# onofreiandrea/quantum_simulations

Hardware: AMD Instinct MI355X
Metric: gate-applications/sec (random 1q+CX circuit, complex128 statevector) (higher is better)
Workload: dtype f64

## Files before the change

include/qsim_hip.h:

```cpp
#ifndef QSIM_HIP_H
#define QSIM_HIP_H

#include <stdint.h>

#ifdef __cplusplus
extern "C" {
#endif

#define QSIM_OK            0
#define QSIM_ERR_INVALID  (-1)
#define QSIM_ERR_NONLOCAL (-2)
#define QSIM_ERR_HIP      (-3)
#define QSIM_ERR_NOMEM    (-4)

typedef struct qsim_chunk qsim_chunk;

const char* qsim_last_error(void);
int qsim_version(void);
int qsim_device_count(int* count);

int qsim_create(int device, int n_local_qubits, qsim_chunk** out);
int qsim_create_view(qsim_chunk* parent, uint64_t offset_amps, int n_local_qubits,
                     qsim_chunk** out);
int qsim_wrap(int device, void* device_ptr, int n_local_qubits, void* stream,
              qsim_chunk** out);
int qsim_destroy(qsim_chunk* c);
int qsim_n_local_qubits(const qsim_chunk* c);
void* qsim_device_ptr(const qsim_chunk* c);

int qsim_init_zero(qsim_chunk* c, int set_amp0);
int qsim_init_random(qsim_chunk* c, uint64_t seed);
int qsim_upload(qsim_chunk* c, const double* re_im, uint64_t offset_amps, uint64_t count);
int qsim_download(qsim_chunk* c, double* re_im, uint64_t offset_amps, uint64_t count);
int qsim_download_c64(qsim_chunk* c, float* re_im, uint64_t offset_amps, uint64_t count);
int qsim_upload_c64(qsim_chunk* c, const float* re_im, uint64_t offset_amps, uint64_t count);
int qsim_copy(qsim_chunk* dst, const qsim_chunk* src);
int qsim_copy_variant(qsim_chunk* dst, const qsim_chunk* src, int variant);

int qsim_apply_1q(qsim_chunk* c, int qubit, const double U[8]);
int qsim_apply_2q(qsim_chunk* c, int qa, int qb, const double U[32]);
int qsim_apply_fused_k(qsim_chunk* c, int k, const int32_t* qubits, const double* M);
int qsim_apply_ops(qsim_chunk* c, int n_ops, const int32_t* nq, const int32_t* qubits,
                   const double* mats);
int qsim_apply_ops_unfused(qsim_chunk* c, int n_ops, const int32_t* nq, const int32_t* qubits,
                           const double* mats);
int qsim_last_pass_count(const qsim_chunk* c);
int qsim_plan_cache_clear(void);
int qsim_apply_ops_tiled(qsim_chunk* c, int n_ops, const int32_t* nq, const int32_t* qubits, const double* mats,
                         int n_tiles, const uint64_t* tile_masks);
int qsim_apply_ops_placed(qsim_chunk* c, int n_ops, const int32_t* nq, const int32_t* qubits, const double* mats,
                          int n_tiles, const uint64_t* tile_masks, const int32_t* earliest_pass);

typedef struct qsim_cycle qsim_cycle;
typedef struct {
  int32_t n_ops; const int32_t* nq; const int32_t* qubits; const double* mats;
  int32_t n_tiles; const uint64_t* tile_masks;
  const int32_t* earliest_pass;
} qsim_cycle_list;
int qsim_cycle_create(int n_local_qubits, const qsim_cycle_list* head, const qsim_cycle_list* steady, const qsim_cycle_list* tail,
                      int32_t* n_passes, qsim_cycle** out);
int qsim_cycle_destroy(qsim_cycle* cycle);
int qsim_apply_cycle(qsim_chunk* c, const qsim_cycle* cycle);

typedef struct {
  uint32_t struct_size;
  const qsim_chunk* src; int32_t src_m; int32_t src_bits[3];
  qsim_chunk* dst; int32_t dst_m; int32_t dst_bits[3];
  qsim_chunk* dst_own; int32_t own_pattern;
  int32_t dst_parts;
  int32_t src_parts;
  int32_t n_tiles;
  const uint64_t* tile_masks;
} qsim_ops_io;
int qsim_apply_ops_io(qsim_chunk* c, int n_ops, const int32_t* nq, const int32_t* qubits,
                      const double* mats, const qsim_ops_io* io, int* n_passes);
int qsim_apply_ops_io_own_slab(const qsim_chunk* c, int32_t* in_chunk);
int qsim_apply_ops_io_load(qsim_chunk* c, int part);
int qsim_apply_ops_io_source_parts(const qsim_chunk* c, int32_t* n_parts, uint64_t* piece_amps, int32_t* n_launches);
int qsim_apply_ops_io_parts(const qsim_chunk* c, int32_t* n_parts, uint64_t* piece_amps, int32_t* n_launches);
int qsim_apply_ops_io_part(qsim_chunk* c, int part);
int qsim_split_piece_count(int n_local_qubits, int m, int dst_parts);
int qsim_tiles_per_workgroup(int n_local_qubits, int tile_bits, int n_fixed_bits);
#define QSIM_PASS_IMAGE_BYTES 4096
int qsim_plan_ops(int n_local_qubits, int n_ops, const int32_t* nq, const int32_t* qubits, const double* mats,
                  void* out, uint64_t out_capacity_bytes, int32_t* n_passes);
int qsim_plan_ops_tiled(int n_local_qubits, int n_ops, const int32_t* nq, const int32_t* qubits, const double* mats,
                        int n_tiles, const uint64_t* tile_masks, void* out, uint64_t out_capacity_bytes, int32_t* n_passes);

int qsim_plan_peek_pass(int n_local_qubits, int n_total_qubits, int n_ops, const int32_t* nq, const int32_t* qubits,
                        const double* mats, const uint8_t* done, uint64_t avoid_mask, uint64_t hint_mask, uint64_t* tile_mask,
                        uint64_t* need_mask, int32_t* n_members, int32_t* members);

int qsim_plan_search(int n_local_qubits, int n_ops, const int32_t* nq, const int32_t* qubits, const double* mats, int beam,
                     uint64_t* out_masks, int out_capacity, int32_t* n_passes);

#define QSIM_PLAN_HISTOGRAM_BINS 64
#define QSIM_TRIPLES_UNBOUNDED 1
#define QSIM_TRIPLES_NEED_BITS 2
int qsim_plan_search_triples(int n_local_qubits, int n_ops, const int32_t* nq, const int32_t* qubits, const double* mats,
                             int n_triples, const int32_t* triples, int beam, int n_threads, int flags, int32_t* best_passes,
                             int32_t* n_found, int32_t* found_index, int32_t* found_triples, uint64_t* found_masks,
                             uint64_t mask_capacity, int32_t* histogram);
int qsim_plan_search_cycle(int n_local_qubits, int n_ops, const int32_t* nq, const int32_t* qubits, const double* mats,
                           int n_triples, const int32_t* triples, const int32_t* plain_passes, int beam, int n_threads,
                           int32_t* n_found, int32_t* found_index, int32_t* found_triples, int32_t* found_passes,
                           uint8_t* found_tail, uint64_t* found_masks, uint64_t mask_capacity);

int qsim_rewrite_ops(int n_qubits, int n_ops, const int32_t* nq, const int32_t* qubits, const double* mats, int32_t* out_nq,
                     int32_t* out_qubits, double* out_mats, int out_capacity, int32_t* n_out, int32_t* need_tile);

int qsim_lower_pass_images(void* images, int n_images, int32_t* n_rewritten);

enum { QSIM_ENGINE_COST_FIXED_US = 0, QSIM_ENGINE_COST_GROUP, QSIM_ENGINE_COST_DENSE1, QSIM_ENGINE_COST_REAL1,
       QSIM_ENGINE_COST_HAD1, QSIM_ENGINE_COST_SWAP1, QSIM_ENGINE_COST_ASWAP1, QSIM_ENGINE_COST_ANTI1, QSIM_ENGINE_COST_PHASE,
       QSIM_ENGINE_COST_PHASE_NEG, QSIM_ENGINE_COST_PHASE_I, QSIM_ENGINE_COST_DIAGR, QSIM_ENGINE_COST_DENSE2,
       QSIM_ENGINE_COST_PRED_LANE, QSIM_ENGINE_COST_PRED_OUTER, QSIM_ENGINE_COST_REG_CTRL, QSIM_ENGINE_COST_DIRECT_END,
       QSIM_ENGINE_COST_FIT_QUBITS, QSIM_ENGINE_COST_UNIT1, QSIM_ENGINE_COST_COUNT };
int qsim_plan_balance(int n_local_qubits, int n_ops, const int32_t* nq, const int32_t* qubits, const double* mats,
                      int n_tiles, const uint64_t* tile_masks, const double* pass_memory_us, const double* engine_costs,
                      int n_engine_costs, int32_t* earliest_pass, double* engine_us_before, double* engine_us_after);
int qsim_plan_ops_placed(int n_local_qubits, int n_ops, const int32_t* nq, const int32_t* qubits, const double* mats,
                         int n_tiles, const uint64_t* tile_masks, const int32_t* earliest_pass, void* out,
                         uint64_t out_capacity_bytes, int32_t* n_passes);
int qsim_rewrite_ops_priced(int n_qubits, int n_ops, const int32_t* nq, const int32_t* qubits, const double* mats,
                            int32_t* out_nq, int32_t* out_qubits, double* out_mats, int out_capacity, int32_t* n_out,
                            int32_t* need_tile, const double* engine_costs, int n_engine_costs);

int qsim_plan_count_layouts(int n_local_qubits, int n_ops, const int32_t* nq, const int32_t* qubits, const double* mats,
                            int n_layouts, const int32_t* layouts, int32_t* n_passes, int n_threads);

int qsim_choose_layout(int n_local_qubits, int n_tiles, const uint64_t* tile_masks, int top_bit, const double* bit_cost,
                       const double* pair_cost, const double* triple_cost , uint64_t seed,
                       int sweeps, int32_t* out_l2p, double* cost_identity, double* cost_chosen);

int qsim_apply_1q_pair(qsim_chunk* c0, qsim_chunk* c1, const double U[8]);
int qsim_apply_2q_pair_qa_local(qsim_chunk* c0, qsim_chunk* c1, int qa, const double U[32]);
int qsim_apply_2q_pair_qb_local(qsim_chunk* c0, qsim_chunk* c1, int qb, const double U[32]);
int qsim_apply_2q_quad(qsim_chunk* c00, qsim_chunk* c01, qsim_chunk* c10, qsim_chunk* c11,
                       const double U[32]);

int qsim_pack_half(const qsim_chunk* src, int bit, int value, qsim_chunk* buf);
int qsim_unpack_half(qsim_chunk* dst, int bit, int value, const qsim_chunk* buf);
int qsim_pack_bits(const qsim_chunk* src, int m, const int32_t* bits, int pattern,
                   qsim_chunk* buf, uint64_t buf_offset_amps);
int qsim_unpack_bits(qsim_chunk* dst, int m, const int32_t* bits, int pattern,
                     const qsim_chunk* buf, uint64_t buf_offset_amps);
int qsim_pack_all(const qsim_chunk* src, int m, const int32_t* bits, qsim_chunk* buf, int skip_pattern,
                  int piece, int n_pieces);
int qsim_unpack_all(qsim_chunk* dst, int m, const int32_t* bits, const qsim_chunk* buf, int skip_pattern,
                    int piece, int n_pieces);

int qsim_swap_global_local(qsim_chunk* const* chunks, int n_chunks, const int32_t* global_bits,
                           const int32_t* local_bits, int m);

#define QSIM_COMM_ID_BYTES 128
typedef struct qsim_comm qsim_comm;
int qsim_comm_get_unique_id(uint8_t id[QSIM_COMM_ID_BYTES]);
int qsim_comm_init(int device, int rank, int world, const uint8_t id[QSIM_COMM_ID_BYTES], qsim_comm** out);
int qsim_comm_destroy(qsim_comm* comm);
int qsim_comm_rank(const qsim_comm* comm);
int qsim_comm_world(const qsim_comm* comm);
int qsim_comm_exchange(qsim_comm* comm, int n_peers, const int32_t* peers, const qsim_chunk* send,
                       const uint64_t* send_off, qsim_chunk* recv, const uint64_t* recv_off, uint64_t count_amps);
int qsim_comm_exchange_bg(qsim_comm* comm, int n_peers, const int32_t* peers, const qsim_chunk* send,
                          const uint64_t* send_off, qsim_chunk* recv, const uint64_t* recv_off, uint64_t count_amps,
                          uint32_t* ticket);
int qsim_comm_join(qsim_comm* comm, qsim_chunk* c);
int qsim_comm_wait(qsim_comm* comm, qsim_chunk* c, uint32_t ticket);
int qsim_comm_relayout(qsim_comm* comm, qsim_chunk* state, qsim_chunk* buf0, qsim_chunk* buf1, int m,
                       const int32_t* local_bits, const int32_t* global_bits, int n_pieces);
int qsim_comm_relayout_plan(int rank, int world, int n_local_qubits, int m, const int32_t* local_bits,
                            const int32_t* global_bits, int n_pieces, int32_t* out_n_pieces, int32_t* out_n_peers,
                            int32_t* out_own_pattern, int32_t* out_peers, uint64_t* out_slab_offsets,
                            uint64_t* out_piece_amps);
int qsim_comm_relayout_loopback(qsim_comm* comm, qsim_chunk* state, qsim_chunk* buf0, qsim_chunk* buf1, int m,
                                const int32_t* local_bits, const int32_t* global_bits, int n_pieces, int as_rank,
                                int as_world);
int qsim_apply_1q_pair_remote(qsim_comm* comm, qsim_chunk* shard, qsim_chunk* buf, int partner_rank, int my_side,
                              const double U[8]);
int qsim_apply_2q_pair_qa_local_remote(qsim_comm* comm, qsim_chunk* shard, qsim_chunk* buf, int partner_rank,
                                       int my_side, int qa, const double U[32]);
int qsim_apply_2q_pair_qb_local_remote(qsim_comm* comm, qsim_chunk* shard, qsim_chunk* buf, int partner_rank,
                                       int my_side, int qb, const double U[32]);

int qsim_apply_2q_quad_remote(qsim_comm* comm, qsim_chunk* shard, qsim_chunk* buf, const int32_t ranks[4], int my_index,
                              const double U[32]);
typedef struct { int32_t n_ops; const int32_t* nq; const int32_t* qubits; const double* mats; } qsim_op_list;
int qsim_comm_relayout_fused(qsim_comm* comm, qsim_chunk* shard, qsim_chunk* send, qsim_chunk* recv,
                             const qsim_op_list* before, const qsim_op_list* after, int m, const int32_t* local_bits,
                             const int32_t* global_bits, int n_pieces, int as_rank, int as_world, int* n_passes);

int qsim_count_nonzero(qsim_chunk* c, double eps, uint64_t* count);
int qsim_export_nonzero(qsim_chunk* c, double eps, uint64_t capacity, uint64_t* out_idx, double* out_re_im,
                        uint64_t* n_rows);
int qsim_sync(qsim_chunk* c);
int qsim_norm2(qsim_chunk* c, double* out);
int qsim_probabilities(qsim_chunk* c, int r, const int32_t* qubits, double* out);
int qsim_reduced_density_matrix(qsim_chunk* c, int r, const int32_t* qubits, double* out);
int qsim_reduced_density_matrix_wide(qsim_chunk* c, int r, const int32_t* qubits, double* out);
int qsim_expectation_pauli(qsim_chunk* c, int n_terms, const uint64_t* x_masks, const uint64_t* z_masks, double* out,
                           int* n_passes);
int qsim_plan_expectation(int n_local_qubits, int n_terms, const uint64_t* x_masks, int32_t* pass_of_term,
                          uint64_t* tile_masks, int* n_passes);
int qsim_apply_pauli_rotations(qsim_chunk* c, int n, const uint64_t* x_masks, const uint64_t* z_masks,
                               const double* thetas, int* n_passes);
int qsim_apply_diagonal_phase(qsim_chunk* c, int n_terms, const uint64_t* z_masks, const double* coeffs, double gamma);
int qsim_diagonal_moments(qsim_chunk* c, int n_terms, const uint64_t* z_masks, const double* coeffs, double out[3]);
int qsim_apply_diagonal_sum(qsim_chunk* dst, const qsim_chunk* src, int n_terms, const uint64_t* z_masks, const double* coeffs,
                            int accumulate);
int qsim_overlap_diagonal(qsim_chunk* ket, const qsim_chunk* bra, int n_terms, const uint64_t* z_masks, const double* coeffs,
                          double out[4]);
int qsim_expectation_z_terms(qsim_chunk* c, int n_terms, const uint64_t* z_masks, double* out, int* n_passes);
int qsim_plan_pauli_rotations(int n_local_qubits, int n, const uint64_t* x_masks, int32_t* pass_of,
                              uint64_t* tile_masks, int* n_passes);
int qsim_apply_pauli_sum(qsim_chunk* dst, const qsim_chunk* src, int n_terms, const uint64_t* x_masks,
                         const uint64_t* z_masks, const double* coeffs, int* n_passes);
int qsim_overlap_pauli(qsim_chunk* ket, const qsim_chunk* bra, int n_terms, const uint64_t* x_masks,
                       const uint64_t* z_masks, double* out_re_im, int* n_passes);
int qsim_lincomb(qsim_chunk* dst, const double dst_coeff[2], int n_src, const qsim_chunk* const* srcs,
                 const double* coeffs_re_im, int n_bras, const qsim_chunk* const* bras, double* dots_re_im,
                 double* norm2);
int qsim_sample(qsim_chunk* c, uint64_t n_shots, const double* randnums, uint64_t* out_indices, double* total, int* n_passes);
int qsim_sample_locate(uint64_t n_blocks, const double* block_cdf, uint64_t n_shots, const double* randnums,
                       uint64_t* out_block, double* out_local);
int qsim_sample_block_bits(void);
int qsim_max_abs_err_closed_form(qsim_chunk* c, int kind, int n_total_qubits,
                                 uint64_t base_index, double* out);
int qsim_max_abs_err_closed_form_perm(qsim_chunk* c, int kind, int n_total_qubits,
                                      uint64_t base_index, const int32_t* log_to_phys,
                                      double* out);
int qsim_fingerprint(qsim_chunk* c, int n_total_qubits, uint64_t base_index, const int32_t* log_to_phys, uint64_t seed,
                     uint64_t sel_mask, uint64_t sel_value, double out[2]);
int qsim_time_begin(qsim_chunk* c);
int qsim_time_end(qsim_chunk* c, float* elapsed_ms);


typedef struct {
  char kernel[48];
  uint64_t launches;
  double total_ms;
  double algorithmic_bytes;
  double hbm_bytes;
  uint64_t streaming_launches;
} qsim_profile_entry;
int qsim_profile_begin(qsim_chunk* c);
int qsim_profile_end(qsim_chunk* c, int max_entries, int* n_entries, qsim_profile_entry* out);

#ifdef __cplusplus
}
#endif
#endif
```

quantum_simulations_amd/_lib.py:

```python
from __future__ import annotations

import ctypes as C
import os
from pathlib import Path

LIB_NAME = "libqsim_hip.so"
LIB_PATH = Path(os.environ.get("QSIM_LIBRARY") or (Path(__file__).resolve().parent / LIB_NAME))

QSIM_OK = 0
QSIM_ERR_INVALID = -1
QSIM_ERR_NONLOCAL = -2
QSIM_ERR_HIP = -3
QSIM_ERR_NOMEM = -4


class QsimLibraryMissing(RuntimeError):
    pass


class QsimHipError(RuntimeError):
    pass


_P = C.c_void_p
_D = C.POINTER(C.c_double)
_I32 = C.POINTER(C.c_int32)

SIGNATURES = {
    "qsim_last_error": (C.c_char_p, []),
    "qsim_version": (C.c_int, []),
    "qsim_device_count": (C.c_int, [C.POINTER(C.c_int)]),
    "qsim_create": (C.c_int, [C.c_int, C.c_int, C.POINTER(_P)]),
    "qsim_create_view": (C.c_int, [_P, C.c_uint64, C.c_int, C.POINTER(_P)]),
    "qsim_wrap": (C.c_int, [C.c_int, _P, C.c_int, _P, C.POINTER(_P)]),
    "qsim_destroy": (C.c_int, [_P]),
    "qsim_n_local_qubits": (C.c_int, [_P]),
    "qsim_device_ptr": (_P, [_P]),
    "qsim_init_zero": (C.c_int, [_P, C.c_int]),
    "qsim_init_random": (C.c_int, [_P, C.c_uint64]),
    "qsim_upload": (C.c_int, [_P, _P, C.c_uint64, C.c_uint64]),
    "qsim_download": (C.c_int, [_P, _P, C.c_uint64, C.c_uint64]),
    "qsim_download_c64": (C.c_int, [_P, _P, C.c_uint64, C.c_uint64]),
    "qsim_upload_c64": (C.c_int, [_P, _P, C.c_uint64, C.c_uint64]),
    "qsim_copy": (C.c_int, [_P, _P]),
    "qsim_copy_variant": (C.c_int, [_P, _P, C.c_int]),
    "qsim_apply_1q": (C.c_int, [_P, C.c_int, _P]),
    "qsim_apply_2q": (C.c_int, [_P, C.c_int, C.c_int, _P]),
    "qsim_apply_fused_k": (C.c_int, [_P, C.c_int, _P, _P]),
    "qsim_apply_ops": (C.c_int, [_P, C.c_int, _P, _P, _P]),
    "qsim_apply_ops_unfused": (C.c_int, [_P, C.c_int, _P, _P, _P]),
    "qsim_plan_ops": (C.c_int, [C.c_int, C.c_int, _P, _P, _P, _P, C.c_uint64, _P]),
    "qsim_plan_ops_tiled": (C.c_int, [C.c_int, C.c_int, _P, _P, _P, C.c_int, _P, _P, C.c_uint64, _P]),
    "qsim_lower_pass_images": (C.c_int, [_P, C.c_int, C.POINTER(C.c_int32)]),
    "qsim_plan_search": (C.c_int, [C.c_int, C.c_int, _P, _P, _P, C.c_int, _P, C.c_int, _P]),
    "qsim_plan_search_triples": (C.c_int, [C.c_int, C.c_int, _P, _P, _P, C.c_int, _P, C.c_int, C.c_int, C.c_int, _P, _P, _P, _P, _P,
                                           C.c_uint64, _P]),
    "qsim_plan_search_cycle": (C.c_int, [C.c_int, C.c_int, _P, _P, _P, C.c_int, _P, _P, C.c_int, C.c_int, _P, _P, _P, _P, _P, _P,
                                         C.c_uint64]),
    "qsim_cycle_create": (C.c_int, [C.c_int, _P, _P, _P, _P, C.POINTER(_P)]),
    "qsim_cycle_destroy": (C.c_int, [_P]),
    "qsim_apply_cycle": (C.c_int, [_P, _P]),
    "qsim_rewrite_ops": (C.c_int, [C.c_int, C.c_int, _P, _P, _P, _P, _P, _P, C.c_int, _P, _P]),
    "qsim_rewrite_ops_priced": (C.c_int, [C.c_int, C.c_int, _P, _P, _P, _P, _P, _P, C.c_int, _P, _P, _P, C.c_int]),
    "qsim_apply_ops_tiled": (C.c_int, [_P, C.c_int, _P, _P, _P, C.c_int, _P]),
    "qsim_apply_ops_placed": (C.c_int, [_P, C.c_int, _P, _P, _P, C.c_int, _P, _P]),
    "qsim_plan_ops_placed": (C.c_int, [C.c_int, C.c_int, _P, _P, _P, C.c_int, _P, _P, _P, C.c_uint64, _P]),
    "qsim_plan_balance": (C.c_int, [C.c_int, C.c_int, _P, _P, _P, C.c_int, _P, _P, _P, C.c_int, _P, _P, _P]),
    "qsim_choose_layout": (C.c_int, [C.c_int, C.c_int, _P, C.c_int, _P, _P, _P, C.c_uint64, C.c_int, _P, C.POINTER(C.c_double), C.POINTER(C.c_double)]),
    "qsim_plan_count_layouts": (C.c_int, [C.c_int, C.c_int, _P, _P, _P, C.c_int, _P, _P, C.c_int]),
    "qsim_plan_peek_pass": (C.c_int, [C.c_int, C.c_int, C.c_int, _P, _P, _P, _P, C.c_uint64, C.c_uint64, C.POINTER(C.c_uint64),
                                      C.POINTER(C.c_uint64), C.POINTER(C.c_int32), _P]),
    "qsim_last_pass_count": (C.c_int, [_P]),
    "qsim_plan_cache_clear": (C.c_int, []),
    "qsim_apply_ops_io": (C.c_int, [_P, C.c_int, _P, _P, _P, _P, C.POINTER(C.c_int)]),
    "qsim_apply_ops_io_part": (C.c_int, [_P, C.c_int]),
    "qsim_apply_ops_io_load": (C.c_int, [_P, C.c_int]),
    "qsim_apply_ops_io_source_parts": (C.c_int, [_P, _P, _P, _P]),
    "qsim_apply_ops_io_parts": (C.c_int, [_P, _P, _P, _P]),
    "qsim_apply_ops_io_own_slab": (C.c_int, [_P, _P]),
    "qsim_split_piece_count": (C.c_int, [C.c_int, C.c_int, C.c_int]),
    "qsim_tiles_per_workgroup": (C.c_int, [C.c_int, C.c_int, C.c_int]),
    "qsim_apply_1q_pair": (C.c_int, [_P, _P, _P]),
    "qsim_apply_2q_pair_qa_local": (C.c_int, [_P, _P, C.c_int, _P]),
    "qsim_apply_2q_pair_qb_local": (C.c_int, [_P, _P, C.c_int, _P]),
    "qsim_apply_2q_quad": (C.c_int, [_P, _P, _P, _P, _P]),
    "qsim_pack_half": (C.c_int, [_P, C.c_int, C.c_int, _P]),
    "qsim_unpack_half": (C.c_int, [_P, C.c_int, C.c_int, _P]),
    "qsim_pack_bits": (C.c_int, [_P, C.c_int, _P, C.c_int, _P, C.c_uint64]),
    "qsim_unpack_bits": (C.c_int, [_P, C.c_int, _P, C.c_int, _P, C.c_uint64]),
    "qsim_pack_all": (C.c_int, [_P, C.c_int, _P, _P, C.c_int, C.c_int, C.c_int]),
    "qsim_unpack_all": (C.c_int, [_P, C.c_int, _P, _P, C.c_int, C.c_int, C.c_int]),
    "qsim_swap_global_local": (C.c_int, [_P, C.c_int, _P, _P, C.c_int]),
    "qsim_comm_get_unique_id": (C.c_int, [_P]),
    "qsim_comm_init": (C.c_int, [C.c_int, C.c_int, C.c_int, _P, C.POINTER(_P)]),
    "qsim_comm_destroy": (C.c_int, [_P]),
    "qsim_comm_rank": (C.c_int, [_P]),
    "qsim_comm_world": (C.c_int, [_P]),
    "qsim_comm_exchange": (C.c_int, [_P, C.c_int, _P, _P, _P, _P, _P, C.c_uint64]),
    "qsim_comm_exchange_bg": (C.c_int, [_P, C.c_int, _P, _P, _P, _P, _P, C.c_uint64, C.POINTER(C.c_uint32)]),
    "qsim_comm_wait": (C.c_int, [_P, _P, C.c_uint32]),
    "qsim_comm_join": (C.c_int, [_P, _P]),
    "qsim_comm_relayout": (C.c_int, [_P, _P, _P, _P, C.c_int, _P, _P, C.c_int]),
    "qsim_comm_relayout_plan": (C.c_int, [C.c_int, C.c_int, C.c_int, C.c_int, _P, _P, C.c_int, _P, _P, _P, _P, _P, _P]),
    "qsim_comm_relayout_loopback": (C.c_int, [_P, _P, _P, _P, C.c_int, _P, _P, C.c_int, C.c_int, C.c_int]),
    "qsim_apply_1q_pair_remote": (C.c_int, [_P, _P, _P, C.c_int, C.c_int, _P]),
    "qsim_apply_2q_pair_qa_local_remote": (C.c_int, [_P, _P, _P, C.c_int, C.c_int, C.c_int, _P]),
    "qsim_apply_2q_pair_qb_local_remote": (C.c_int, [_P, _P, _P, C.c_int, C.c_int, C.c_int, _P]),
    "qsim_apply_2q_quad_remote": (C.c_int, [_P, _P, _P, _P, C.c_int, _P]),
    "qsim_comm_relayout_fused": (C.c_int, [_P, _P, _P, _P, _P, _P, C.c_int, _P, _P, C.c_int, C.c_int, C.c_int, C.POINTER(C.c_int)]),
    "qsim_count_nonzero": (C.c_int, [_P, C.c_double, C.POINTER(C.c_uint64)]),
    "qsim_export_nonzero": (C.c_int, [_P, C.c_double, C.c_uint64, _P, _P, C.POINTER(C.c_uint64)]),
    "qsim_sync": (C.c_int, [_P]),
    "qsim_norm2": (C.c_int, [_P, C.POINTER(C.c_double)]),
    "qsim_probabilities": (C.c_int, [_P, C.c_int, _P, _P]),
    "qsim_reduced_density_matrix": (C.c_int, [_P, C.c_int, _P, _P]),
    "qsim_reduced_density_matrix_wide": (C.c_int, [_P, C.c_int, _P, _P]),
    "qsim_expectation_pauli": (C.c_int, [_P, C.c_int, _P, _P, _P, C.POINTER(C.c_int)]),
    "qsim_plan_expectation": (C.c_int, [C.c_int, C.c_int, _P, _P, _P, C.POINTER(C.c_int)]),
    "qsim_apply_pauli_rotations": (C.c_int, [_P, C.c_int, _P, _P, _P, C.POINTER(C.c_int)]),
    "qsim_plan_pauli_rotations": (C.c_int, [C.c_int, C.c_int, _P, _P, _P, C.POINTER(C.c_int)]),
    "qsim_apply_diagonal_phase": (C.c_int, [_P, C.c_int, _P, _P, C.c_double]),
    "qsim_diagonal_moments": (C.c_int, [_P, C.c_int, _P, _P, _P]),
    "qsim_apply_diagonal_sum": (C.c_int, [_P, _P, C.c_int, _P, _P, C.c_int]),
    "qsim_overlap_diagonal": (C.c_int, [_P, _P, C.c_int, _P, _P, _P]),
    "qsim_expectation_z_terms": (C.c_int, [_P, C.c_int, _P, _P, C.POINTER(C.c_int)]),
    "qsim_apply_pauli_sum": (C.c_int, [_P, _P, C.c_int, _P, _P, _P, C.POINTER(C.c_int)]),
    "qsim_overlap_pauli": (C.c_int, [_P, _P, C.c_int, _P, _P, _P, C.POINTER(C.c_int)]),
    "qsim_lincomb": (C.c_int, [_P, _P, C.c_int, _P, _P, C.c_int, _P, _P, _P]),
    "qsim_sample": (C.c_int, [_P, C.c_uint64, _P, _P, C.POINTER(C.c_double), C.POINTER(C.c_int)]),
    "qsim_sample_locate": (C.c_int, [C.c_uint64, _P, C.c_uint64, _P, _P, _P]),
    "qsim_sample_block_bits": (C.c_int, []),
    "qsim_max_abs_err_closed_form": (C.c_int, [_P, C.c_int, C.c_int, C.c_uint64,
                                               C.POINTER(C.c_double)]),
    "qsim_max_abs_err_closed_form_perm": (C.c_int, [_P, C.c_int, C.c_int, C.c_uint64, _P,
                                                    C.POINTER(C.c_double)]),
    "qsim_fingerprint": (C.c_int, [_P, C.c_int, C.c_uint64, _P, C.c_uint64, C.c_uint64, C.c_uint64, _P]),
    "qsim_time_begin": (C.c_int, [_P]),
    "qsim_time_end": (C.c_int, [_P, C.POINTER(C.c_float)]),
    "qsim_profile_begin": (C.c_int, [_P]),
    "qsim_profile_end": (C.c_int, [_P, C.c_int, C.POINTER(C.c_int), _P]),
}


class OpsIo(C.Structure):
    _fields_ = [("struct_size", C.c_uint32),
                ("src", C.c_void_p), ("src_m", C.c_int32), ("src_bits", C.c_int32 * 3),
                ("dst", C.c_void_p), ("dst_m", C.c_int32), ("dst_bits", C.c_int32 * 3),
                ("dst_own", C.c_void_p), ("own_pattern", C.c_int32), ("dst_parts", C.c_int32), ("src_parts", C.c_int32),
                ("n_tiles", C.c_int32), ("tile_masks", C.c_void_p)]

    def __init__(self, *args, **kw):
        super().__init__(*args, **kw)
        self.struct_size = C.sizeof(OpsIo)


class OpList(C.Structure):
    _fields_ = [("n_ops", C.c_int32), ("nq", C.c_void_p), ("qubits", C.c_void_p), ("mats", C.c_void_p)]


class CycleList(C.Structure):
    _fields_ = [("n_ops", C.c_int32), ("nq", C.c_void_p), ("qubits", C.c_void_p), ("mats", C.c_void_p),
                ("n_tiles", C.c_int32), ("tile_masks", C.c_void_p), ("earliest_pass", C.c_void_p)]


class ProfileEntry(C.Structure):
    _fields_ = [("kernel", C.c_char * 48), ("launches", C.c_uint64),
                ("total_ms", C.c_double), ("algorithmic_bytes", C.c_double),
                ("hbm_bytes", C.c_double), ("streaming_launches", C.c_uint64)]

_lib = None


def source_hash() -> str:
    import hashlib
    h = hashlib.sha256()
    csrc = Path(__file__).resolve().parent / "csrc"
    for path in sorted(list(csrc.glob("*.h")) + list(csrc.glob("*.hip")) + list(csrc.glob("*.py")) + [csrc / "Makefile"]):
        h.update(path.name.encode())
        h.update(path.read_bytes())
    return h.hexdigest()[:16]


def load() -> C.CDLL:
    global _lib
    if _lib is not None:
        return _lib
    if not LIB_PATH.exists():
        raise QsimLibraryMissing(
            f"{LIB_PATH} not found: the HIP extension is not built. Run "
            "`python -c 'import __graft_entry__ as g; g.build()'` (needs hipcc). "
            "This engine has no CPU fallback.")
    lib = C.CDLL(str(LIB_PATH))
    for name, (restype, argtypes) in SIGNATURES.items():
        fn = getattr(lib, name)
        fn.restype = restype
        fn.argtypes = argtypes
    _lib = lib
    return lib


def ptr(a):
    return None if a is None else a.ctypes.data_as(C.c_void_p)


def check(rc: int) -> None:
    if rc == QSIM_OK:
        return
    msg = (load().qsim_last_error() or b"").decode("utf-8", "replace")
    if rc == QSIM_ERR_NONLOCAL:
        raise NotImplementedError(msg)
    if rc == QSIM_ERR_INVALID:
        raise ValueError(msg)
    if rc == QSIM_ERR_NOMEM:
        raise MemoryError(msg)
    raise QsimHipError(msg)
```

quantum_simulations_amd/csrc/abi_gates.h:

```cpp

enum QubitReport { kQubitOfChunk, kQubitOfPlan, kQubitOfState };

static int check_op_list(int n_ops, const int32_t* nq, const int32_t* qubits, const double* mats, int qubit_limit, QubitReport how) {
  if (n_ops < 0 || (n_ops && (!nq || !qubits || !mats))) return fail(QSIM_ERR_INVALID, "bad op list");
  for (int i = 0; i < n_ops; ++i) {
    if (nq[i] != 1 && nq[i] != 2) return fail(QSIM_ERR_INVALID, "op %d: arity %d", i, nq[i]);
    for (int j = 0; j < nq[i]; ++j) {
      const int q = qubits[2 * i + j];
      if (q >= 0 && q < qubit_limit) continue;
      if (how == kQubitOfState) return fail(QSIM_ERR_INVALID, "op %d: qubit %d out of range", i, q);
      if (how == kQubitOfChunk && q < 0) return fail(QSIM_ERR_INVALID, "qubit %d is negative", q);
      return fail(QSIM_ERR_NONLOCAL, "qubit %d >= log2(chunk_size)=%d: non-local gate requires layout/collect step", q, qubit_limit);
    }
    if (nq[i] == 2 && qubits[2 * i] == qubits[2 * i + 1]) return fail(QSIM_ERR_INVALID, "op %d: repeated qubit", i);
  }
  return QSIM_OK;
}

static void classify_ops(int n_ops, const int32_t* nq, const int32_t* qubits, const double* mats, std::vector<FusedOp>* ops,
                         std::vector<int32_t>* origin = nullptr) {
  ops->reserve((size_t)n_ops);
  for (int i = 0; i < n_ops; ++i) {
    FusedOp o;
    if (!classify_op(nq[i], qubits + 2 * i, mats + 32 * (size_t)i, &o)) continue;
    ops->push_back(o);
    if (origin) origin->push_back(i);
  }
}

static int validate_ops(qsim_chunk* c, int n_ops, const int32_t* nq, const int32_t* qubits, const double* mats) {
  int rc = check_chunk(c, "qsim_apply_ops");
  if (rc) return rc;
  return check_op_list(n_ops, nq, qubits, mats, c->k, kQubitOfChunk);
}

extern "C" {
int qsim_apply_1q(qsim_chunk* c, int qubit, const double U[8]) {
  int rc = check_chunk(c, "qsim_apply_1q");
  if (rc || (rc = check_local_qubit(c, qubit))) return rc;
  if (!U) return fail(QSIM_ERR_INVALID, "U is null");
  HIP_TRY(hipSetDevice(c->device));
  Group g = {{c, nullptr, nullptr, nullptr}, 1, c->k};
  return gate_1q(g, qubit, U, c->stream);
}

int qsim_apply_2q(qsim_chunk* c, int qa, int qb, const double U[32]) {
  int rc = check_chunk(c, "qsim_apply_2q");
  if (rc || (rc = check_local_qubit(c, qa)) || (rc = check_local_qubit(c, qb))) return rc;
  if (qa == qb) return fail(QSIM_ERR_INVALID, "apply_2q needs two distinct qubits, got %d twice", qa);
  if (!U) return fail(QSIM_ERR_INVALID, "U is null");
  HIP_TRY(hipSetDevice(c->device));
  Group g = {{c, nullptr, nullptr, nullptr}, 1, c->k};
  return gate_2q(g, qa, qb, U, c->stream);
}

int qsim_apply_ops_unfused(qsim_chunk* c, int n_ops, const int32_t* nq, const int32_t* qubits, const double* mats) {
  int rc = validate_ops(c, n_ops, nq, qubits, mats);
  if (rc) return rc;
  for (int i = 0; i < n_ops; ++i) {
    rc = nq[i] == 1 ? qsim_apply_1q(c, qubits[2 * i], mats + 32 * (size_t)i)
                    : qsim_apply_2q(c, qubits[2 * i], qubits[2 * i + 1], mats + 32 * (size_t)i);
    if (rc) return rc;
  }
  return QSIM_OK;
}

static int apply_ops_fused(qsim_chunk* c, int n_ops, const int32_t* nq, const int32_t* qubits, const double* mats,
                           int n_tiles, const uint64_t* tile_masks, const char* what, const int32_t* earliest_pass = nullptr) {
  int rc = validate_ops(c, n_ops, nq, qubits, mats);
  if (rc) return rc;
  if (n_tiles < 0 || (n_tiles && !tile_masks)) return fail(QSIM_ERR_INVALID, "%s: bad tile list", what);
  if ((rc = require_no_parts(c, what))) return rc;
  if (n_ops < 2 || c->k < kTileMinChunk || c->k > kTileMaxQubits) {
    c->last_passes = n_ops;
    return qsim_apply_ops_unfused(c, n_ops, nq, qubits, mats);
  }
  HIP_TRY(hipSetDevice(c->device));
  std::vector<FusedOp> ops;
  std::vector<int32_t> origin, placed;
  classify_ops(n_ops, nq, qubits, mats, &ops, &origin);
  int passes = 0;
  TileHint hint = {tile_masks, n_tiles};
  if (earliest_pass && n_tiles) {
    for (int32_t i : origin) placed.push_back(earliest_pass[i]);
    hint.earliest = placed.data();
  }
  rc = run_fused(c, ops, RawOps{n_ops, nq, qubits, mats}, n_tiles ? &hint : nullptr, nullptr, &passes,
                 [&](TileArgs& a, int T, double alg_bytes, bool) { return dispatch_planned(c, a, T, alg_bytes); });
  c->last_passes = passes;
  return rc;
}

int qsim_apply_ops(qsim_chunk* c, int n_ops, const int32_t* nq, const int32_t* qubits, const double* mats) {
  return apply_ops_fused(c, n_ops, nq, qubits, mats, 0, nullptr, "qsim_apply_ops");
}
int qsim_apply_ops_tiled(qsim_chunk* c, int n_ops, const int32_t* nq, const int32_t* qubits, const double* mats,
                         int n_tiles, const uint64_t* tile_masks) {
  return apply_ops_fused(c, n_ops, nq, qubits, mats, n_tiles, tile_masks, "qsim_apply_ops_tiled");
}
int qsim_apply_ops_placed(qsim_chunk* c, int n_ops, const int32_t* nq, const int32_t* qubits, const double* mats,
                          int n_tiles, const uint64_t* tile_masks, const int32_t* earliest_pass) {
  return apply_ops_fused(c, n_ops, nq, qubits, mats, n_tiles, tile_masks, "qsim_apply_ops_placed", earliest_pass);
}

}

struct qsim_cycle {
  int k;
  u64 id;
  PassList head, steady, tail;
};
static std::atomic<u64> g_cycle_ids{0};

static int cycle_passes(int k, const qsim_cycle_list* l, const char* part, PassList* out) {
  if (!l || l->n_ops < 1 || l->n_tiles < 0 || (l->n_tiles && !l->tile_masks))
    return fail(QSIM_ERR_INVALID, "qsim_cycle_create: bad %s list", part);
  int rc = check_op_list(l->n_ops, l->nq, l->qubits, l->mats, k, kQubitOfPlan);
  if (rc) return rc;
  std::vector<FusedOp> ops;
  std::vector<int32_t> origin, placed;
  classify_ops(l->n_ops, l->nq, l->qubits, l->mats, &ops, &origin);
  if (ops.empty()) return fail(QSIM_ERR_INVALID, "qsim_cycle_create: the %s list holds identities only", part);
  TileHint hint = {l->tile_masks, l->n_tiles};
  if (l->earliest_pass && l->n_tiles) {
    for (int32_t i : origin) placed.push_back(l->earliest_pass[i]);
    hint.earliest = placed.data();
  }
  auto made = std::make_shared<std::vector<CachedPass>>();
  int passes = 0;
  rc = plan_fused(k, ops, &passes, [&](TileArgs& a, int T, double alg_bytes, bool, bool) {
    lower_unit_real(&a);
    made->push_back(CachedPass{a, T, alg_bytes});
    return (int)QSIM_OK;
  }, l->n_tiles ? &hint : nullptr);
  *out = made;
  return rc;
}

extern "C" {
int qsim_cycle_create(int n_local_qubits, const qsim_cycle_list* head, const qsim_cycle_list* steady, const qsim_cycle_list* tail,
                      int32_t* n_passes, qsim_cycle** out) {
  if (!out) return fail(QSIM_ERR_INVALID, "qsim_cycle_create: out is null");
  if (n_local_qubits < kTileMinChunk || n_local_qubits > kTileMaxQubits)
    return fail(QSIM_ERR_INVALID, "qsim_cycle_create: fused passes need %d..%d local qubits", kTileMinChunk, kTileMaxQubits);
  std::unique_ptr<qsim_cycle> cy(new qsim_cycle());
  cy->k = n_local_qubits;
  cy->id = ++g_cycle_ids;
  int rc = cycle_passes(n_local_qubits, head, "head", &cy->head);
  if (rc || (rc = cycle_passes(n_local_qubits, steady, "steady", &cy->steady)) || (rc = cycle_passes(n_local_qubits, tail, "tail", &cy->tail)))
    return rc;
  if (n_passes) { n_passes[0] = (int32_t)cy->head->size(); n_passes[1] = (int32_t)cy->steady->size(); n_passes[2] = (int32_t)cy->tail->size(); }
  *out = cy.release();
  return QSIM_OK;
}

int qsim_cycle_destroy(qsim_cycle* cycle) {
  delete cycle;
  return QSIM_OK;
}

int qsim_apply_cycle(qsim_chunk* c, const qsim_cycle* cycle) {
  int rc = check_chunk_unsettled(c, "qsim_apply_cycle");
  if (rc) return rc;
  if (!cycle) return fail(QSIM_ERR_INVALID, "qsim_apply_cycle: null cycle");
  if (cycle->k != c->k) return fail(QSIM_ERR_INVALID, "qsim_apply_cycle: a cycle for %d qubits on a chunk of %d", cycle->k, c->k);
  if (!c->owns_memory || c->parent)
    return fail(QSIM_ERR_INVALID, "qsim_apply_cycle: the chunk must own its memory (views and wrapped pointers cannot defer a tail)");
  if ((rc = require_no_parts(c, "qsim_apply_cycle"))) return rc;
  const bool steady = c->deferred && c->deferred->passes && c->deferred->id == cycle->id;
  if (!steady && (rc = settle(c))) return rc;
  if (!c->deferred) c->deferred = new DeferredTail();
  c->deferred->passes.reset();
  const std::vector<CachedPass>& run = steady ? *cycle->steady : *cycle->head;
  if ((rc = launch_passes(c, run))) return rc;
  c->deferred->id = cycle->id;
  c->deferred->passes = cycle->tail;
  c->last_passes = (int)run.size();
  return QSIM_OK;
}

int qsim_apply_fused_k(qsim_chunk* c, int k, const int32_t* qubits, const double* M) {
  int rc = check_chunk(c, "qsim_apply_fused_k");
  if (rc) return rc;
  if (!qubits || !M) return fail(QSIM_ERR_INVALID, "qsim_apply_fused_k: null argument");
  if (k < 1 || k > 6) return fail(QSIM_ERR_INVALID, "qsim_apply_fused_k: 1 <= k <= 6 qubits expected, got %d", k);
  if ((rc = require_no_parts(c, "qsim_apply_fused_k"))) return rc;
  for (int i = 0; i < k; ++i) {
    if ((rc = check_local_qubit(c, qubits[i]))) return rc;
    for (int j = 0; j < i; ++j) if (qubits[j] == qubits[i]) return fail(QSIM_ERR_INVALID, "qsim_apply_fused_k: repeated qubit %d", qubits[i]);
  }
  if (k == 1) return qsim_apply_1q(c, qubits[0], M);
  if (k == 2) return qsim_apply_2q(c, qubits[1], qubits[0], M);
  return apply_dense_block(c, k, qubits, M);
}

int qsim_last_pass_count(const qsim_chunk* c) { return c ? c->last_passes : -1; }

int qsim_apply_1q_pair(qsim_chunk* c0, qsim_chunk* c1, const double U[8]) {
  qsim_chunk* cs[2] = {c0, c1};
  int rc = check_group(cs, 2, "qsim_apply_1q_pair");
  if (rc) return rc;
  if (!U) return fail(QSIM_ERR_INVALID, "U is null");
  HIP_TRY(hipSetDevice(c0->device));
  Group g = {{c0, c1, nullptr, nullptr}, 2, c0->k};
  return gate_1q(g, c0->k, U, c0->stream);
}

static int apply_2q_pair(qsim_chunk* c0, qsim_chunk* c1, int q_local, bool qa_is_local, const double U[32], const char* what) {
  qsim_chunk* cs[2] = {c0, c1};
  int rc = check_group(cs, 2, what);
  if (rc || (rc = check_local_qubit(c0, q_local))) return rc;
  if (!U) return fail(QSIM_ERR_INVALID, "U is null");
  HIP_TRY(hipSetDevice(c0->device));
  Group g = {{c0, c1, nullptr, nullptr}, 2, c0->k};
  return qa_is_local ? gate_2q(g, q_local, c0->k, U, c0->stream) : gate_2q(g, c0->k, q_local, U, c0->stream);
}
int qsim_apply_2q_pair_qa_local(qsim_chunk* c0, qsim_chunk* c1, int qa, const double U[32]) {
  return apply_2q_pair(c0, c1, qa, true, U, "qsim_apply_2q_pair_qa_local");
}
int qsim_apply_2q_pair_qb_local(qsim_chunk* c0, qsim_chunk* c1, int qb, const double U[32]) {
  return apply_2q_pair(c0, c1, qb, false, U, "qsim_apply_2q_pair_qb_local");
}

int qsim_apply_2q_quad(qsim_chunk* c00, qsim_chunk* c01, qsim_chunk* c10, qsim_chunk* c11, const double U[32]) {
  qsim_chunk* cs[4] = {c00, c01, c10, c11};
  int rc = check_group(cs, 4, "qsim_apply_2q_quad");
  if (rc) return rc;
  if (!U) return fail(QSIM_ERR_INVALID, "U is null");
  HIP_TRY(hipSetDevice(c00->device));
  Group g = {{c00, c01, c10, c11}, 4, c00->k};
  return gate_2q(g, c00->k + 1, c00->k, U, c00->stream);
}
}
```

quantum_simulations_amd/csrc/abi_plan.h:

```cpp
extern "C" {
int qsim_plan_cache_clear(void) {
  std::lock_guard<std::mutex> lock(g_plan_cache_mu);
  g_plan_cache.clear();
  return QSIM_OK;
}

static_assert(sizeof(TileArgs) == QSIM_PASS_IMAGE_BYTES, "pass image = the kernel-argument block of k_tile");

}
static int plan_ops_images(const char* what, int n_local_qubits, int n_ops, const int32_t* nq, const int32_t* qubits,
                           const double* mats, int n_tiles, const uint64_t* tile_masks, const int32_t* earliest_pass, void* out,
                           uint64_t out_capacity_bytes, int32_t* n_passes) {
  if (n_tiles < 0 || (n_tiles && !tile_masks)) return fail(QSIM_ERR_INVALID, "%s: bad tile list", what);
  if (!n_passes) return fail(QSIM_ERR_INVALID, "%s: n_passes is null", what);
  if (n_local_qubits < kTileMinChunk || n_local_qubits > kTileMaxQubits)
    return fail(QSIM_ERR_INVALID, "%s: fused passes need %d..%d local qubits", what, kTileMinChunk, kTileMaxQubits);
  int rc = check_op_list(n_ops, nq, qubits, mats, n_local_qubits, kQubitOfPlan);
  if (rc) return rc;
  std::vector<FusedOp> ops;
  std::vector<int32_t> origin, placed;
  classify_ops(n_ops, nq, qubits, mats, &ops, &origin);
  int passes = 0;
  char* dst = (char*)out;
  uint64_t used = 0;
  TileHint hint = {tile_masks, n_tiles};
  if (earliest_pass && n_tiles) {
    for (int32_t i : origin) placed.push_back(earliest_pass[i]);
    hint.earliest = placed.data();
  }
  rc = plan_fused(n_local_qubits, ops, &passes, [&](TileArgs& a, int T, double, bool, bool) {
    if (dst) {
      if (used + sizeof(TileArgs) > out_capacity_bytes) return fail(QSIM_ERR_INVALID, "%s: output buffer too small", what);
      std::memcpy(dst + used, &a, sizeof a);
    }
    used += sizeof(TileArgs);
    return (int)QSIM_OK;
  }, n_tiles ? &hint : nullptr);
  *n_passes = passes;
  return rc;
}
extern "C" {
int qsim_plan_ops(int n_local_qubits, int n_ops, const int32_t* nq, const int32_t* qubits, const double* mats,
                  void* out, uint64_t out_capacity_bytes, int32_t* n_passes) {
  return plan_ops_images("qsim_plan_ops", n_local_qubits, n_ops, nq, qubits, mats, 0, nullptr, nullptr, out, out_capacity_bytes, n_passes);
}
int qsim_plan_ops_tiled(int n_local_qubits, int n_ops, const int32_t* nq, const int32_t* qubits, const double* mats,
                        int n_tiles, const uint64_t* tile_masks, void* out, uint64_t out_capacity_bytes, int32_t* n_passes) {
  return plan_ops_images("qsim_plan_ops_tiled", n_local_qubits, n_ops, nq, qubits, mats, n_tiles, tile_masks, nullptr, out,
                         out_capacity_bytes, n_passes);
}
int qsim_plan_ops_placed(int n_local_qubits, int n_ops, const int32_t* nq, const int32_t* qubits, const double* mats,
                         int n_tiles, const uint64_t* tile_masks, const int32_t* earliest_pass, void* out,
                         uint64_t out_capacity_bytes, int32_t* n_passes) {
  return plan_ops_images("qsim_plan_ops_placed", n_local_qubits, n_ops, nq, qubits, mats, n_tiles, tile_masks, earliest_pass, out,
                         out_capacity_bytes, n_passes);
}

int qsim_lower_pass_images(void* images, int n_images, int32_t* n_rewritten) {
  if (n_images < 0 || (n_images && !images)) return fail(QSIM_ERR_INVALID, "qsim_lower_pass_images: bad arguments");
  int total = 0;
  for (int i = 0; i < n_images; ++i) {
    TileArgs a;
    std::memcpy(&a, (char*)images + (size_t)i * sizeof a, sizeof a);
    total += lower_unit_real(&a);
    std::memcpy((char*)images + (size_t)i * sizeof a, &a, sizeof a);
  }
  if (n_rewritten) *n_rewritten = total;
  return QSIM_OK;
}

int qsim_plan_search(int n_local_qubits, int n_ops, const int32_t* nq, const int32_t* qubits, const double* mats, int beam,
                     uint64_t* out_masks, int out_capacity, int32_t* n_passes) {
  if (!n_passes || out_capacity < 0) return fail(QSIM_ERR_INVALID, "qsim_plan_search: bad arguments");
  if (n_local_qubits < kTileMinChunk || n_local_qubits > kTileMaxQubits)
    return fail(QSIM_ERR_INVALID, "qsim_plan_search: fused passes need %d..%d local qubits", kTileMinChunk, kTileMaxQubits);
  int rc = check_op_list(n_ops, nq, qubits, mats, n_local_qubits, kQubitOfPlan);
  if (rc) return rc;
#ifdef QSIM_PROBES
  if (beam <= 0) if (const char* e = getenv("QSIM_PLAN_BEAM")) beam = atoi(e);
#endif
  ListSearch ts;
  ts.beam = beam;
  ts.bounded = false;
  rc = plan_search_triples(n_local_qubits, n_ops, nq, qubits, mats, {LineTriple{{0, 1, 2}}}, &ts);
  if (rc) return rc;
  const std::vector<u64>& masks = ts.masks[0];
  *n_passes = ts.best;
  if (out_masks) {
    if ((int)masks.size() > out_capacity) return fail(QSIM_ERR_INVALID, "qsim_plan_search: output buffer too small");
    for (size_t p = 0; p < masks.size(); ++p) out_masks[p] = masks[p];
  }
  return QSIM_OK;
}

int qsim_plan_search_triples(int n_local_qubits, int n_ops, const int32_t* nq, const int32_t* qubits, const double* mats,
                             int n_triples, const int32_t* triples, int beam, int n_threads, int flags, int32_t* best_passes,
                             int32_t* n_found, int32_t* found_index, int32_t* found_triples, uint64_t* found_masks,
                             uint64_t mask_capacity, int32_t* histogram) {
  if (!best_passes || !n_found || !found_index || !found_triples || n_triples < 0 || (n_triples && !triples) || (mask_capacity && !found_masks))
    return fail(QSIM_ERR_INVALID, "qsim_plan_search_triples: bad arguments");
  if (n_local_qubits < kTileMinChunk || n_local_qubits > kTileMaxQubits)
    return fail(QSIM_ERR_INVALID, "qsim_plan_search_triples: fused passes need %d..%d local qubits", kTileMinChunk, kTileMaxQubits);
  int rc = check_op_list(n_ops, nq, qubits, mats, n_local_qubits, kQubitOfPlan);
  if (rc) return rc;
  std::vector<LineTriple> list;
  for (int t = 0; t < n_triples; ++t) {
    const int32_t* q = triples + 3 * (size_t)t;
    for (int b = 0; b < 3; ++b)
      if (q[b] < 0 || q[b] >= n_local_qubits || (b && q[b] == q[0]) || (b == 2 && q[2] == q[1]))
        return fail(QSIM_ERR_INVALID, "qsim_plan_search_triples: triple %d is not three qubits of the %d", t, n_local_qubits);
    list.push_back(LineTriple{{q[0], q[1], q[2]}});
  }
  if (!n_triples)
    for (int a = 0; a < n_local_qubits; ++a)
      for (int b = a + 1; b < n_local_qubits; ++b)
        for (int c = b + 1; c < n_local_qubits; ++c) list.push_back(LineTriple{{a, b, c}});
  ListSearch ts;
  ts.beam = beam;
  ts.n_threads = n_threads;
  ts.bounded = !(flags & QSIM_TRIPLES_UNBOUNDED);
  ts.need_bits = (flags & QSIM_TRIPLES_NEED_BITS) != 0;
  rc = plan_search_triples(n_local_qubits, n_ops, nq, qubits, mats, list, &ts);
  if (rc) return rc;
  std::vector<int32_t> found;
  for (size_t t = 0; t < list.size(); ++t) if (ts.passes[t] == ts.best) found.push_back((int32_t)t);
  std::stable_sort(found.begin(), found.end(), [&](int32_t x, int32_t y) {
    return std::lexicographical_compare(list[(size_t)x].q, list[(size_t)x].q + 3, list[(size_t)y].q, list[(size_t)y].q + 3);
  });
  *best_passes = ts.best;
  *n_found = (int32_t)found.size();
  if (histogram) {
    for (int b = 0; b < QSIM_PLAN_HISTOGRAM_BINS; ++b) histogram[b] = 0;
    for (int32_t p : ts.passes) ++histogram[p < 0 ? QSIM_PLAN_HISTOGRAM_BINS - 1 : std::min((int)p, QSIM_PLAN_HISTOGRAM_BINS - 2)];
  }
  if ((uint64_t)found.size() * (uint64_t)ts.best > mask_capacity)
    return fail(QSIM_ERR_INVALID, "qsim_plan_search_triples: output buffer too small (%d triples of %d masks)", (int)found.size(), ts.best);
  for (size_t f = 0; f < found.size(); ++f) {
    const size_t t = (size_t)found[f];
    found_index[f] = found[f];
    for (int b = 0; b < 3; ++b) found_triples[3 * f + b] = list[t].q[b];
    for (int p = 0; p < ts.best; ++p) found_masks[f * (size_t)ts.best + p] = ts.masks[t][(size_t)p];
  }
  return QSIM_OK;
}

int qsim_plan_search_cycle(int n_local_qubits, int n_ops, const int32_t* nq, const int32_t* qubits, const double* mats,
                           int n_triples, const int32_t* triples, const int32_t* plain_passes, int beam, int n_threads,
                           int32_t* n_found, int32_t* found_index, int32_t* found_triples, int32_t* found_passes,
                           uint8_t* found_tail, uint64_t* found_masks, uint64_t mask_capacity) {
  if (!n_found || !found_index || !found_triples || !found_passes || !found_tail || n_triples < 1 || !triples || (mask_capacity && !found_masks))
    return fail(QSIM_ERR_INVALID, "qsim_plan_search_cycle: bad arguments");
  if (n_local_qubits < kTileMinChunk || n_local_qubits > kTileMaxQubits)
    return fail(QSIM_ERR_INVALID, "qsim_plan_search_cycle: fused passes need %d..%d local qubits", kTileMinChunk, kTileMaxQubits);
  int rc = check_op_list(n_ops, nq, qubits, mats, n_local_qubits, kQubitOfPlan);
  if (rc) return rc;
  std::vector<LineTriple> list;
  for (int t = 0; t < n_triples; ++t) {
    const int32_t* q = triples + 3 * (size_t)t;
    for (int b = 0; b < 3; ++b)
      if (q[b] < 0 || q[b] >= n_local_qubits || (b && q[b] == q[0]) || (b == 2 && q[2] == q[1]))
        return fail(QSIM_ERR_INVALID, "qsim_plan_search_cycle: triple %d is not three qubits of the %d", t, n_local_qubits);
    list.push_back(LineTriple{{q[0], q[1], q[2]}});
  }
  std::vector<CyclePlan> cycles;
  if ((rc = plan_search_cycle(n_local_qubits, n_ops, nq, qubits, mats, list, plain_passes, beam, n_threads, &cycles))) return rc;
  int fewest = 1 << 30;
  for (const CyclePlan& c : cycles) if (c.found) fewest = std::min(fewest, (int)c.passes[1]);
  int found = 0;
  uint64_t used = 0;
  for (const CyclePlan& c : cycles) if (c.found && c.passes[1] == fewest) { ++found; used += c.masks[0].size() + c.masks[1].size() + c.masks[2].size(); }
  *n_found = found;
  if (used > mask_capacity) return fail(QSIM_ERR_INVALID, "qsim_plan_search_cycle: output buffer too small (%llu masks)", (u64)used);
  size_t f = 0;
  for (size_t t = 0; t < cycles.size(); ++t) {
    const CyclePlan& c = cycles[t];
    if (!c.found || c.passes[1] != fewest) continue;
    found_index[f] = (int32_t)t;
    for (int b = 0; b < 3; ++b) found_triples[3 * f + b] = list[t].q[b];
    found_passes[4 * f] = c.plain;
    for (int w = 0; w < 3; ++w) {
      found_passes[4 * f + 1 + w] = c.passes[w];
      for (u64 m : c.masks[w]) *found_masks++ = m;
    }
    std::memcpy(found_tail + f * (size_t)n_ops, c.tail.data(), (size_t)n_ops);
    ++f;
  }
  return QSIM_OK;
}

int qsim_plan_balance(int n_local_qubits, int n_ops, const int32_t* nq, const int32_t* qubits, const double* mats,
                      int n_tiles, const uint64_t* tile_masks, const double* pass_memory_us, const double* engine_costs,
                      int n_engine_costs, int32_t* earliest_pass, double* engine_us_before, double* engine_us_after) {
  if (n_tiles < 1 || !tile_masks || !pass_memory_us) return fail(QSIM_ERR_INVALID, "qsim_plan_balance: bad arguments");
  if (n_local_qubits < kTileMinChunk || n_local_qubits > kTileMaxQubits)
    return fail(QSIM_ERR_INVALID, "qsim_plan_balance: fused passes need %d..%d local qubits", kTileMinChunk, kTileMaxQubits);
  EngineCosts ec;
  if (!engine_costs_from(engine_costs, n_engine_costs, &ec))
    return fail(QSIM_ERR_INVALID, "qsim_plan_balance: the cost table needs %d entries", (int)QSIM_ENGINE_COST_COUNT);
  int rc = check_op_list(n_ops, nq, qubits, mats, n_local_qubits, kQubitOfPlan);
  if (rc) return rc;
  std::vector<FusedOp> ops;
  std::vector<int32_t> origin;
  classify_ops(n_ops, nq, qubits, mats, &ops, &origin);
  const std::vector<u64> masks(tile_masks, tile_masks + n_tiles);
  std::vector<int32_t> placed;
  std::vector<double> before, after;
  rc = plan_balance(n_local_qubits, ops, masks, pass_memory_us, ec, earliest_pass != nullptr, &placed, &before, &after);
  if (rc) return rc;
  for (int i = 0; earliest_pass && i < n_ops; ++i) earliest_pass[i] = 0;
  for (size_t j = 0; earliest_pass && j < origin.size(); ++j) earliest_pass[origin[j]] = placed[j];
  for (int p = 0; p < n_tiles; ++p) {
    if (engine_us_before) engine_us_before[p] = before[(size_t)p];
    if (engine_us_after) engine_us_after[p] = after[(size_t)p];
  }
  return QSIM_OK;
}

int qsim_rewrite_ops(int n_qubits, int n_ops, const int32_t* nq, const int32_t* qubits, const double* mats, int32_t* out_nq,
                     int32_t* out_qubits, double* out_mats, int out_capacity, int32_t* n_out, int32_t* need_tile) {
  return qsim_rewrite_ops_priced(n_qubits, n_ops, nq, qubits, mats, out_nq, out_qubits, out_mats, out_capacity, n_out, need_tile, nullptr, 0);
}

int qsim_rewrite_ops_priced(int n_qubits, int n_ops, const int32_t* nq, const int32_t* qubits, const double* mats,
                            int32_t* out_nq, int32_t* out_qubits, double* out_mats, int out_capacity, int32_t* n_out,
                            int32_t* need_tile, const double* engine_costs, int n_engine_costs) {
  if (!n_out || out_capacity < 0 || (out_capacity && (!out_nq || !out_qubits || !out_mats)))
    return fail(QSIM_ERR_INVALID, "qsim_rewrite_ops: bad arguments");
  if (n_qubits < 1 || n_qubits > 63) return fail(QSIM_ERR_INVALID, "qsim_rewrite_ops: bad qubit count %d", n_qubits);
  int rc = check_op_list(n_ops, nq, qubits, mats, n_qubits, kQubitOfState);
  if (rc) return rc;
  std::vector<RwOp> ops;
  int need_in = 0, need_out = 0;
  EngineCosts ec;
  const bool priced = engine_costs_from(engine_costs, n_engine_costs, &ec);
  if (engine_costs && !priced) return fail(QSIM_ERR_INVALID, "qsim_rewrite_ops_priced: the cost table has %d entries, not %d", n_engine_costs, (int)QSIM_ENGINE_COST_COUNT);
  rewrite_op_list(n_qubits, n_ops, nq, qubits, mats, &ops, &need_in, priced ? &ec : nullptr);
  *n_out = (int32_t)ops.size();
  if (ops.size() > (size_t)out_capacity) return fail(QSIM_ERR_INVALID, "qsim_rewrite_ops: output buffer too small (%d ops)", (int)ops.size());
  for (size_t i = 0; i < ops.size(); ++i) {
    out_nq[i] = ops[i].nq;
    out_qubits[2 * i] = ops[i].q[0];
    out_qubits[2 * i + 1] = ops[i].nq == 2 ? ops[i].q[1] : 0;
    std::memcpy(out_mats + 32 * i, ops[i].U, sizeof ops[i].U);
    need_out += rw_needs_tile(ops[i]);
  }
  if (need_tile) { need_tile[0] = need_in; need_tile[1] = need_out; }
  return QSIM_OK;
}

int qsim_plan_peek_pass(int n_local_qubits, int n_total_qubits, int n_ops, const int32_t* nq, const int32_t* qubits,
                        const double* mats, const uint8_t* done, uint64_t avoid_mask, uint64_t hint_mask, uint64_t* tile_mask,
                        uint64_t* need_mask, int32_t* n_members, int32_t* members) {
  if (!done || !tile_mask || !n_members || !members) return fail(QSIM_ERR_INVALID, "qsim_plan_peek_pass: null argument");
  if (n_local_qubits < kTileMinChunk || n_local_qubits > kTileMaxQubits)
    return fail(QSIM_ERR_INVALID, "qsim_plan_peek_pass: fused passes need %d..%d local qubits", kTileMinChunk, kTileMaxQubits);
  if (n_total_qubits < n_local_qubits || n_total_qubits > 63) return fail(QSIM_ERR_INVALID, "qsim_plan_peek_pass: bad total qubit count %d", n_total_qubits);
  int rc = check_op_list(n_ops, nq, qubits, mats, n_total_qubits, kQubitOfState);
  if (rc) return rc;
  std::vector<FusedOp> ops;
  std::vector<int32_t> origin;
  classify_ops(n_ops, nq, qubits, mats, &ops, &origin);
  std::vector<uint8_t> done_ops;
  for (int32_t i : origin) done_ops.push_back(done[i]);
  std::vector<size_t> held;
  PeekPlan peek;
  peek.n_total = n_total_qubits;
  peek.done = done_ops.data();
  peek.avoid = avoid_mask;
  peek.tile_mask = peek.need_mask = 0;
  peek.members = &held;
  int passes = 0;
  const TileHint hint = {&hint_mask, 1};
  rc = plan_fused(n_local_qubits, ops, &passes, [](TileArgs&, int, double, bool, bool) { return (int)QSIM_OK; },
                  hint_mask ? &hint : nullptr, &peek);
  if (rc) return rc;
  *tile_mask = peek.tile_mask;
  if (need_mask) *need_mask = peek.need_mask;
  *n_members = (int32_t)held.size();
  for (size_t j = 0; j < held.size(); ++j) members[j] = origin[held[j]];
  return QSIM_OK;
}

int qsim_plan_count_layouts(int n_local_qubits, int n_ops, const int32_t* nq, const int32_t* qubits, const double* mats,
                            int n_layouts, const int32_t* layouts, int32_t* n_passes, int n_threads) {
  if (!n_passes || n_layouts < 0 || (n_layouts && !layouts)) return fail(QSIM_ERR_INVALID, "qsim_plan_count_layouts: bad arguments");
  if (n_local_qubits < kTileMinChunk || n_local_qubits > kTileMaxQubits)
    return fail(QSIM_ERR_INVALID, "qsim_plan_count_layouts: fused passes need %d..%d local qubits", kTileMinChunk, kTileMaxQubits);
  const int bad_ops = check_op_list(n_ops, nq, qubits, mats, n_local_qubits, kQubitOfPlan);
  if (bad_ops) return bad_ops;
  for (int l = 0; l < n_layouts; ++l) {
    u64 seen = 0;
    for (int q = 0; q < n_local_qubits; ++q) {
      const int b = layouts[(size_t)l * n_local_qubits + q];
      if (b < 0 || b >= n_local_qubits || ((seen >> b) & 1)) return fail(QSIM_ERR_INVALID, "qsim_plan_count_layouts: layout %d is not a permutation", l);
      seen |= 1ull << b;
    }
  }
  (void)tuning();
  std::atomic<int> next{0}, bad{0};
  auto work = [&]() {
    std::vector<FusedOp> ops;
    for (;;) {
      const int l = next.fetch_add(1);
      if (l >= n_layouts) return;
      const int32_t* lay = layouts + (size_t)l * n_local_qubits;
      ops.clear();
      for (int i = 0; i < n_ops; ++i) {
        const int32_t q[2] = {lay[qubits[2 * i]], nq[i] == 2 ? lay[qubits[2 * i + 1]] : -1};
        FusedOp o;
        if (classify_op(nq[i], q, mats + 32 * (size_t)i, &o)) ops.push_back(o);
      }
      int passes = 0;
      const int rc = plan_fused(n_local_qubits, ops, &passes, [](TileArgs&, int, double, bool, bool) { return (int)QSIM_OK; });
      if (rc) bad.store(1);
      n_passes[l] = rc ? -1 : passes;
    }
  };
  const int nt = std::max(1, std::min(n_threads > 0 ? n_threads : 1, std::min(n_layouts, 64)));
  std::vector<std::thread> pool;
  for (int t = 1; t < nt; ++t) pool.emplace_back(work);
  work();
  for (std::thread& t : pool) t.join();
  if (bad.load()) return fail(QSIM_ERR_INVALID, "qsim_plan_count_layouts: a layout could not be planned");
  return QSIM_OK;
}

int qsim_choose_layout(int n_local_qubits, int n_tiles, const uint64_t* tile_masks, int top_bit, const double* bit_cost,
                       const double* pair_cost, const double* triple_cost, uint64_t seed, int sweeps, int32_t* out_l2p,
                       double* cost_identity, double* cost_chosen) {
  const int n = n_local_qubits, low = kTileLow;
  if (n < low + 2 || n > 62 || n_tiles < 0 || (n_tiles && !tile_masks) || !bit_cost || !pair_cost || !out_l2p || top_bit < low || top_bit > 62 || sweeps < 1)
    return fail(QSIM_ERR_INVALID, "qsim_choose_layout: bad arguments");
  const int nb = top_bit - low + 1;
  std::vector<std::vector<int>> tiles((size_t)n_tiles);
  std::vector<std::vector<int>> member((size_t)n);
  for (int t = 0; t < n_tiles; ++t)
    for (int q = low; q < n; ++q)
      if ((tile_masks[t] >> q) & 1) { tiles[(size_t)t].push_back(q); member[(size_t)q].push_back(t); }
  std::vector<double> sym((size_t)nb * nb, 0.0);
  for (int a = 0; a < nb; ++a)
    for (int b = a + 1; b < nb; ++b) sym[(size_t)a * nb + b] = sym[(size_t)b * nb + a] = pair_cost[(size_t)a * nb + b];
  std::vector<int> l2p((size_t)n);
  for (int q = 0; q < n; ++q) l2p[(size_t)q] = q;
  auto cost_of = [&](int t) {
    int idx[64], m = 0;
    for (int q : tiles[(size_t)t]) idx[m++] = std::min(l2p[(size_t)q], top_bit) - low;
    double c = 0;
    for (int i = 0; i < m; ++i) {
      c += bit_cost[idx[i]];
      for (int j = i + 1; j < m; ++j) c += sym[(size_t)idx[i] * nb + idx[j]];
    }
    if (triple_cost) {
      std::sort(idx, idx + m);
      for (int i = 0; i < m; ++i)
        for (int j = i + 1; j < m; ++j) {
          if (idx[j] == idx[i]) continue;
          const double* row = triple_cost + ((size_t)idx[i] * nb + idx[j]) * nb;
          for (int l = j + 1; l < m; ++l) if (idx[l] != idx[j]) c += row[idx[l]];
        }
    }
    return c;
  };
  std::vector<double> costs((size_t)n_tiles);
  double cur = 0;
  for (int t = 0; t < n_tiles; ++t) cur += (costs[(size_t)t] = cost_of(t));
  const double identity = cur;
  double best = cur;
// ... 46 lines not shown
```

quantum_simulations_amd/csrc/tile_groups.h:

```cpp

template <class Fn>
static void for_each_triple(unsigned mask, Fn&& fn) {
  for (unsigned a = mask; a; a &= a - 1)
    for (unsigned b = a & (a - 1); b; b &= b - 1)
      for (unsigned c = b & (b - 1); c; c &= c - 1) fn((a & -a) | (b & -b) | (c & -c));
}

struct PhaseRuns {
  struct Acc { uint16_t blk; u64 outer; double2 phi[3]; unsigned touched; };
  std::vector<Acc> open;

  static int run_bytes(unsigned touched) { const int n = __builtin_popcount(touched); return desc_bytes(n == 1 ? 2 : (n == 2 ? 6 : 14)); }
  int reserve() const {
    int bytes = 0;
    for (const Acc& acc : open) bytes += run_bytes(acc.touched);
    return bytes;
  }
  void add(uint16_t blk, u64 outer, int r, double2 phase) {
    size_t i = 0;
    while (i < open.size() && !(open[i].blk == blk && open[i].outer == outer)) ++i;
    if (i == open.size()) {
      Acc acc;
      acc.blk = blk; acc.outer = outer; acc.touched = 0;
      for (int e = 0; e < 3; ++e) acc.phi[e] = make_double2(1.0, 0.0);
// ... 229 lines not shown
        bool touched_later = false;
        for (size_t q = p + 1; q < ng && !touched_later; ++q) touched_later = !gone[q] && (op_qmask(op_at(q)) & tbit);
        if (cv.kind == TG_SWAP1 && tuning().tile_sink_swaps && !touched_later) continue;
        for (size_t q = p; q-- > 0;) {
          if (gone[q] || !(op_qmask(op_at(q)) & tbit)) continue;
          if (is_plain_1q(op_at(q)) && !paired[q]) { partner = (long)q; u_first = true; }
          break;
        }
      }
      if (partner < 0) continue;
      const FusedOp& u = op_at((size_t)partner);
      Half& half = first_half[(size_t)partner];
      half.op = cv;
      if (u_first) mul2x2(cv.m, u.m, half.op.m); else mul2x2(u.m, cv.m, half.op.m);
      set_1q_kind(&half.op);
      half.stands_for = p;
      paired[(size_t)partner] = 1;
      gone[p] = 1;
    }
    for (size_t q = 0; q < ng; ++q) {
      if (gone[q]) continue;
      const FusedOp& u = op_at(q);
      if (!paired[q]) { seq.push_back(Item{u, grp[q], 0}); continue; }
      const FusedOp& a = first_half[q].op;
      FusedOp b = u;
      b.control = a.control;
      b.control_zero = true;
      b.nq = 2;
      b.qubits[1] = a.control;
      seq.push_back(Item{a, grp[first_half[q].stands_for], desc_bytes(op_shape(b).nd)});
      seq.push_back(Item{b, grp[q], 0});
    }
    return seq;
  }

  TileDesc describe(const FusedOp& o, const OpShape& shape, u64 touched_later, unsigned* reg_mask) {
    TileDesc d;
    std::memset(&d, 0, sizeof d);
    int ctrl_reg = -1;
    *reg_mask = 0;
    auto require_one = [&](int qubit) {
      const int p = tile_pos(qubit);
      if (p < 0) { d.outer_mask |= 1ull << qubit; return; }
      const int r = reg_pos(p);
      if (r >= 0) { *reg_mask |= 1u << r; ctrl_reg = r; }
      else d.blk_mask |= (uint16_t)(1u << p);
    };
    auto put = [&](int at, double2 v) { d.m[2 * at] = v.x; d.m[2 * at + 1] = v.y; };
    if (o.kind == TG_PHASE) {
      for (int t = 0; t < o.nbits; ++t) require_one(o.bits[t]);
      d.opcode = (uint8_t)(shape.family + *reg_mask);
      if (shape.nd) { put(0, o.m[0]); d.nd = 2; }
    } else if (o.kind == TG_DENSE2) {
      d.opcode = (uint8_t)(OPC_DENSE2 + 3 * reg_pos(tile_pos(o.target[0])) + reg_pos(tile_pos(o.target[1])));
      for (int e = 0; e < 16; ++e) put(e, o.m[e]);
      d.nd = 32;
    } else {
      const int J = reg_pos(tile_pos(o.target[0]));
      if (o.control >= 0 && o.control_zero) { d.outer_mask |= 1ull << o.control; d.outer_zero = true; }
      else if (o.control >= 0) require_one(o.control);
      d.opcode = (uint8_t)(shape.family + opc_1q_variant(J, ctrl_reg));
      if (shape.family == OPC_SWAP1 && tuning().tile_sink_swaps &&
          !(touched_later & (1ull << o.target[0])) && !(ctrl_reg >= 0 && (touched_later & (1ull << o.control))))
        d.opcode = (uint8_t)(OPC_ASWAP1 + opc_1q_variant(J, ctrl_reg));
      if (shape.family == OPC_HAD1) {
        pass_scale *= o.m[0].x;
      } else if (shape.family == OPC_REAL1) {
        d.m[0] = o.m[0].x; d.m[1] = o.m[1].x; d.m[2] = o.m[2].x; d.m[3] = o.m[3].x; d.nd = 4;
      } else if (shape.family == OPC_ANTI1) {
        put(0, o.m[1]); put(1, o.m[2]); d.nd = 4;
      } else if (shape.family == OPC_DENSE1) {
        for (int e = 0; e < 4; ++e) put(e, o.m[e]);
        d.nd = 8;
      }
    }
    return d;
  }

  bool write_group(const std::vector<size_t>& grp, unsigned claimed) {
    std::vector<int> S;
    for (unsigned m = claimed; m; m &= m - 1) S.push_back(__builtin_ctz(m));
    for (int b = T - 1; (int)S.size() < kGroupBits && b >= 0; --b)
      if (std::find(S.begin(), S.end(), b) == S.end()) S.push_back(b);
    std::sort(S.begin(), S.end());
    TileGroup tg;
    for (int j = 0; j < 3; ++j) tg.s[j] = regs[j] = S[j];
    tg.qmask = 0;
    used += kGroupRecordBytes;
    PhaseRuns runs;
    const std::vector<Item> seq = mux_pairs(grp);
    std::vector<u64> later(seq.size() + 1, 0);
    for (size_t i = seq.size(); i-- > 0;) later[i] = later[i + 1] | op_qmask(seq[i].op);
    bool cut = false;
    size_t gi = 0;
    for (const Item& item : seq) {
      const u64 touched_later = later[++gi];
      const FusedOp& o = item.op;
      const OpShape shape = op_shape(o);
      {
        const bool mergeable = merge_on && o.kind == TG_PHASE;
        if (used + runs.reserve() + (mergeable ? desc_bytes(14) : desc_bytes(shape.nd)) + item.with_next > kTileRecordBudget) { cut = true; break; }
      }
      done[item.mi] = 1;
      (*emitted)[item.mi] = 1;
      --left;
      tg.qmask |= op_qmask(o);
      unsigned reg_mask = 0;
      const TileDesc d = describe(o, shape, touched_later, &reg_mask);
      if (o.kind == TG_PHASE && merge_on && __builtin_popcount(reg_mask) == 1) {
        runs.add(d.blk_mask, d.outer_mask, __builtin_ctz(reg_mask), o.m[0]);
        continue;
      }
      if (o.kind != TG_PHASE) {
        unsigned tmask = 0;
        for (int t = 0; t < o.ntargets; ++t) tmask |= 1u << reg_pos(tile_pos(o.target[t]));
        for (size_t i = runs.open.size(); i-- > 0;) if (runs.open[i].touched & tmask) used += runs.flush(i, &tg.gates);
      }
      used += desc_bytes(d);
      tg.gates.push_back(d);
    }
    while (!runs.open.empty()) used += runs.flush(0, &tg.gates);
    if (!tg.gates.empty()) out->push_back(tg);
    else used -= kGroupRecordBytes;
    return cut;
  }

  void move_last_forward() {
    if (!(tuning().tile_direct && T == kTileBitsMax && out->size() > 1 && out->back().s[0] < low)) return;
    size_t at = out->size() - 1;
    while (at > 0 && !((*out)[at].qmask & (*out)[at - 1].qmask)) { std::swap((*out)[at], (*out)[at - 1]); --at; }
    if (out->back().s[0] < low)
      while (at + 1 < out->size()) { std::swap((*out)[at], (*out)[at + 1]); ++at; }
  }
  void apply_scale() {
    if (!(pass_scale != 1.0 && !out->empty())) return;
    TileDesc* host = nullptr;
    for (TileGroup& g : *out)
      for (TileDesc& d : g.gates) {
        if (factor_host_doubles(d.opcode) && !d.blk_mask && !d.outer_mask && !host) host = &d;
      }
    if (host) {
      for (int e = 0; e < host->nd; ++e) host->m[e] *= pass_scale;
    } else {
      TileDesc d;
      std::memset(&d, 0, sizeof d);
      d.opcode = OPC_SCALE;
      d.m[0] = pass_scale;
      d.nd = 1;
      out->back().gates.push_back(d);
    }
  }
};

static int lower_unit_real(TileArgs* a) {
  if (!tuning().tile_unit || !tuning().tile_special) return 0;
  unsigned char* const base = reinterpret_cast<unsigned char*>(a);
  auto get32 = [&](int at) { uint32_t v; std::memcpy(&v, base + at, 4); return v; };
  auto put32 = [&](int at, uint32_t v) { std::memcpy(base + at, &v, 4); };
  std::vector<int> unit;
  int host = -1, host_next = 0;
  for (int off = kTileStreamOff;;) {
    const int entry = (int)(get32(off) / 4), next = (int)get32(off + 4);
    if (entry == OPC_END || entry == OPC_END_DIRECT) break;
    if (next <= off || next + kEndRecordBytes > kTileArgBytes) return 0;
    if (factor_host_doubles(entry)) {
      double m[4];
      for (int e = 0; e < 4; ++e) std::memcpy(&m[e], base + record_double_at(off, next, 4, e), 8);
      if (entry >= OPC_REAL1 && entry < OPC_REAL1 + 3 && unit_real_of(m)) unit.push_back(off);
      else if (host < 0) { host = off; host_next = next; }
    }
    off = next;
  }
  if (host < 0) {
    if (unit.size() < 2) return 0;
    host = unit.back();
    host_next = (int)get32(host + 4);
    unit.pop_back();
  }
  double factor = 1.0;
  for (int off : unit) {
    double m[4];
    const int next = (int)get32(off + 4);
    for (int e = 0; e < 4; ++e) std::memcpy(&m[e], base + record_double_at(off, next, 4, e), 8);
    UnitReal u;
    unit_real_of(m, &u);
    factor *= u.s;
    const uint32_t J = get32(off) / 4 - OPC_REAL1;
    const uint32_t entry = OPC_UNIT1 + 4 * J + 2 * (u.form_a ? 1u : 0u) + (u.neg ? 1u : 0u);
    put32(off, 4 * entry);
    put32(off + 12, (4 * entry) << 16);
    const double out[4] = {u.p, u.q, u.s, 0.0};
    for (int e = 0; e < 4; ++e) std::memcpy(base + record_double_at(off, next, 4, e), &out[e], 8);
  }
  if (unit.empty()) return 0;
  const int host_nd = factor_host_doubles((int)(get32(host) / 4));
  for (int e = 0; e < host_nd; ++e) {
    double v;
    unsigned char* at = base + record_double_at(host, host_next, host_nd, e);
    std::memcpy(&v, at, 8);
    v *= factor;
    std::memcpy(at, &v, 8);
  }
  return (int)unit.size();
}
```

quantum_simulations_amd/csrc/tile_launch.h:

```cpp
static int tile_order_for(const TileArgs&, int) {
#ifdef QSIM_PROBES
  if (tuning().tile_order >= 0) return tuning().tile_order;
#endif
  return 0;
}

static uint8_t slab_position(const TileSlab& t, int b) {
  for (int j = 0; j < 3; ++j) if (t.bit[j] == b) return (uint8_t)(t.top + j);
  for (int i = 0; i < 4; ++i) if ((t.field[i] >> b) & 1) return (uint8_t)(b - i);
  return (uint8_t)b;
}

static void probe_out_of_place(TileArgs* args, const qsim_chunk* c) {
#ifdef QSIM_PROBES
  if (getenv("QSIM_DEBUG_OUT_OF_PLACE")) {
    static double2* other = nullptr;
    static size_t other_bytes = 0;
    const size_t need = sizeof(double2) << c->k;
    if (other_bytes < need) { if (other) (void)hipFree(other); (void)hipMalloc((void**)&other, need); other_bytes = need; }
    args->amp_out = other;
  }
#endif
}
static void probe_stamps_arm(TileArgs* args, u64 ntiles, hipStream_t stream) {
// ... 53 lines not shown
  } else {
  const int per_wg = tiles_per_workgroup(c->k, T, a.nfix);
  if (per_wg < 0) return per_wg;
  const u64 ntiles = 1ull << (c->k - T - a.nfix);
  TileArgs args = a;
  args.ntiles = (uint32_t)ntiles;
  args.order = (uint8_t)((a.order & ~kTileOrderMask) | (tile_order_for(a, T) & kTileOrderMask));
  args.nbits = (uint8_t)c->k;
  if (!args.amp_out) args.amp_out = args.amp;
  for (int i = 0; i < T - kTileLow; ++i) {
    if (args.perm & kTilePermIn) args.lay_in[i] = slab_position(args.slab_in, args.lay_in[i]);
    if (args.perm & kTilePermOut) args.lay_out[i] = slab_position(args.slab_out, args.lay_out[i]);
  }
  probe_out_of_place(&args, c);
  probe_stamps_arm(&args, ntiles, stream);
  bool wide = false;
  for (int i = 0; i < kTileThreadBits - kTileLow && i < T - kTileLow; ++i) wide = wide || args.lay_in[i] >= 28 || args.lay_out[i] >= 28;
  bool nt = c->span_bytes > tuning().mall_bytes;
  if (tuning().force_nt >= 0) nt = tuning().force_nt != 0;
  constexpr int TPW = QSIM_TILES_PER_WG;
  const bool two = per_wg > 1;
  const unsigned grid = (unsigned)(two ? ntiles / TPW : ntiles);
  const bool part = T == kTileBitsMax && args.nfix != 0;
  {
    ProfileScope prof(kClsTile, alg_bytes, stream, nt, 32.0 * (double)(ntiles << T));
    if constexpr (T == kTileBitsMax) {
      if (part && two) launch_k_tile<T, TPW, true>(nt, wide, grid, stream, args);
      else if (part) launch_k_tile<T, 1, true>(nt, wide, grid, stream, args);
    }
    if (!part && two) launch_k_tile<T, TPW, false>(nt, wide, grid, stream, args);
    else if (!part) launch_k_tile<T, 1, false>(nt, wide, grid, stream, args);
  }
  HIP_TRY(hipGetLastError());
  if (!part) probe_stamps_dump(args, a.nrec, ntiles, stream);
  return QSIM_OK;
  }
}

static int launch_tile_any(const TileArgs& a, int T, const qsim_chunk* c, hipStream_t stream, double alg_bytes) {
  switch (T) {
    case 8: return launch_tile<8>(a, c, stream, alg_bytes);
    case 9: return launch_tile<9>(a, c, stream, alg_bytes);
    case 10: return launch_tile<10>(a, c, stream, alg_bytes);
    case 11: return launch_tile<11>(a, c, stream, alg_bytes);
    case 12: return launch_tile<12>(a, c, stream, alg_bytes);
  }
  return fail(QSIM_ERR_INVALID, "internal: tile size %d", T);
}

struct SlabLayout {
  int m = 0;
  int bits[3] = {0, 0, 0};
};
static void slab_descriptor(int k, const SlabLayout& L, TileSlab* t) {
  int sorted[3] = {64, 64, 64};
  for (int j = 0; j < L.m; ++j) sorted[j] = L.bits[j];
  std::sort(sorted, sorted + L.m);
  auto below = [](int b) -> u64 { return b >= 64 ? ~0ull : ((1ull << b) - 1); };
  t->field[0] = below(sorted[0]);
  for (int i = 1; i < 4; ++i) {
    const int lo = sorted[i - 1], hi = i < 3 ? sorted[i] : 64;
    t->field[i] = lo >= 64 ? 0 : (below(hi) & ~below(lo + 1));
  }
  for (int j = 0; j < 3; ++j) t->bit[j] = (uint8_t)(j < L.m ? L.bits[j] : 63);
  t->top = (uint8_t)(k - L.m);
  std::memset(t->pad, 0, sizeof t->pad);
}
struct FusedIo {
  const qsim_chunk* src = nullptr;
  SlabLayout in;
  qsim_chunk* dst = nullptr;
  SlabLayout out;
  qsim_chunk* dst_own = nullptr;
  int own_pattern = -1;
  bool parts = false;
  bool fused_in = false, fused_out = false;
  bool own_in_chunk = false;
};

static void prepare_planned(qsim_chunk* c, TileArgs& a, int T, bool first, bool last, FusedIo* io) {
  a.amp = c->amp;
  a.amp_out = c->amp;
  a.amp_out_own = nullptr;
  a.perm = 0;
  if (io && first && io->src) {
    a.amp = io->src->amp;
    a.perm |= kTilePermIn;
    slab_descriptor(c->k, io->in, &a.slab_in);
    io->fused_in = true;
  }
  if (io && last && io->dst) {
    bool clash = false;
    for (int j = 0; j < T - kTileLow; ++j)
      for (int i = 0; i < io->out.m; ++i) clash = clash || a.h[j] == io->out.bits[i];
    if (!clash || io->own_pattern < 0) {
      a.amp_out = io->dst->amp;
      a.perm |= kTilePermOut;
      slab_descriptor(c->k, io->out, &a.slab_out);
      if (io->own_pattern >= 0) {
        a.perm |= kTileOwnOut;
        a.amp_out_own = io->dst_own->amp;
        if (first && io->src && io->dst_own->amp == io->src->amp) {
          a.amp_out_own = c->amp;
          io->own_in_chunk = true;
        }
        a.own_mask = a.own_value = 0;
        for (int i = 0; i < io->out.m; ++i) {
          a.own_mask |= 1ull << io->out.bits[i];
          if ((io->own_pattern >> i) & 1) a.own_value |= 1ull << io->out.bits[i];
        }
      }
      io->fused_out = true;
    }
  }
}

static bool stays_for_parts(const FusedIo& io, int T, bool last) {
  return last && io.dst && io.parts && io.fused_out && T == kTileBitsMax;
}

static int dispatch_planned(qsim_chunk* c, TileArgs& a, int T, double alg_bytes) {
  if (tuning().debug_stats < 2) return launch_tile_any(a, T, c, c->stream, alg_bytes);
  hipEvent_t e0, e1;
  (void)hipEventCreate(&e0); (void)hipEventCreate(&e1);
  (void)hipEventRecord(e0, c->stream);
  const int rc = launch_tile_any(a, T, c, c->stream, alg_bytes);
  (void)hipEventRecord(e1, c->stream);
  (void)hipEventSynchronize(e1);
  float ms = 0;
  (void)hipEventElapsedTime(&ms, e0, e1);
  std::fprintf(stderr, "[qsim] timed pass: %.3f ms, %d records, high bits", ms, a.nrec);
  for (int j = 0; j < T - kTileLow; ++j) std::fprintf(stderr, " %d", a.h[j]);
  std::fprintf(stderr, "\n");
  (void)hipEventDestroy(e0); (void)hipEventDestroy(e1);
  return rc;
}

struct CachedPass { TileArgs a; int T; double alg_bytes; };
struct CachedPlan {
  int k = 0;
  u64 hash = 0;
  std::vector<unsigned char> key;
  std::vector<CachedPass> passes;
};
constexpr size_t kPlanCacheEntries = 8;
constexpr size_t kPlanCacheMaxKeyBytes = 4u << 20;
static std::list<CachedPlan> g_plan_cache;
static std::mutex g_plan_cache_mu;

struct RawOps { int n; const int32_t* nq; const int32_t* qubits; const double* mats; };

template <class Sink>
static int run_fused(qsim_chunk* c, const std::vector<FusedOp>& ops, const RawOps& raw, const TileHint* hint, FusedIo* io,
                     int* n_passes, Sink&& sink) {
  std::vector<unsigned char> key;
  u64 hash = 0;
  const size_t n_ops = (size_t)raw.n;
  const size_t hint_bytes = hint ? sizeof(uint64_t) * (size_t)hint->n : 0;
  const size_t placed_bytes = hint && hint->earliest ? sizeof(int32_t) * ops.size() : 0;
  const int32_t hint_tag[2] = {hint ? hint->n : -1, placed_bytes != 0};
  const size_t key_bytes = n_ops * (sizeof(int32_t) * 3 + sizeof(double) * 32) + sizeof hint_tag + hint_bytes + placed_bytes;
  const bool cacheable = raw.nq && raw.qubits && raw.mats && raw.n > 0 && key_bytes <= kPlanCacheMaxKeyBytes && tuning().debug_stats == 0 &&
                         tuning().debug_skip_gates == 0;
  if (cacheable) {
    key.resize(key_bytes);
    unsigned char* w = key.data();
    std::memcpy(w, raw.nq, sizeof(int32_t) * n_ops); w += sizeof(int32_t) * n_ops;
    std::memcpy(w, raw.qubits, sizeof(int32_t) * 2 * n_ops); w += sizeof(int32_t) * 2 * n_ops;
    std::memcpy(w, raw.mats, sizeof(double) * 32 * n_ops); w += sizeof(double) * 32 * n_ops;
    std::memcpy(w, hint_tag, sizeof hint_tag); w += sizeof hint_tag;
    if (hint_bytes) std::memcpy(w, hint->masks, hint_bytes);
    if (placed_bytes) std::memcpy(w + hint_bytes, hint->earliest, placed_bytes);
    hash = fnv1a(key.data(), key.size(), 1469598103934665603ull ^ (u64)c->k);
    std::vector<CachedPass> hit;
    {
      std::lock_guard<std::mutex> lock(g_plan_cache_mu);
      for (auto it = g_plan_cache.begin(); it != g_plan_cache.end(); ++it)
        if (it->hash == hash && it->k == c->k && it->key == key) {
          g_plan_cache.splice(g_plan_cache.begin(), g_plan_cache, it);
          hit = g_plan_cache.front().passes;
          break;
        }
    }
    if (!hit.empty()) {
      for (size_t p = 0; p < hit.size(); ++p) {
        const bool last = p + 1 == hit.size();
        prepare_planned(c, hit[p].a, hit[p].T, p == 0, last, io);
        const int rc = sink(hit[p].a, hit[p].T, hit[p].alg_bytes, last);
        if (rc) return rc;
      }
      *n_passes = (int)hit.size();
      return QSIM_OK;
    }
  }
  std::vector<CachedPass> made;
  const int rc = plan_fused(c->k, ops, n_passes, [&](TileArgs& a, int T, double alg_bytes, bool first, bool last) {
    lower_unit_real(&a);
    if (cacheable) made.push_back(CachedPass{a, T, alg_bytes});
    prepare_planned(c, a, T, first, last, io);
    return sink(a, T, alg_bytes, last);
  }, hint);
  if (rc == QSIM_OK && cacheable && !made.empty()) {
    std::lock_guard<std::mutex> lock(g_plan_cache_mu);
    g_plan_cache.emplace_front();
    CachedPlan& e = g_plan_cache.front();
    e.k = c->k; e.hash = hash; e.key.swap(key); e.passes.swap(made);
    while (g_plan_cache.size() > kPlanCacheEntries) g_plan_cache.pop_back();
  }
  return rc;
}
```

quantum_simulations_amd/csrc/tile_planner.h:

```cpp
constexpr int kTileMinChunk = kTileThreadBits > 8 ? kTileThreadBits : 8;

struct TileHint { const uint64_t* masks; int n; const int32_t* earliest = nullptr; };
struct PeekPlan {
  int n_total;
  const uint8_t* done;
  uint64_t avoid;
  uint64_t tile_mask;
  uint64_t need_mask;
  std::vector<size_t>* members;
};

struct PassBuilder {
  const Tuning& tune;
  const std::vector<FusedOp>& ops;
  const int k, T, low, cap;
  const size_t n_ops;
  std::vector<char> done;
  std::vector<u64> qm, need;
  std::vector<u64> tm;
  std::vector<u64> xm;
  u64 all_qubits, rank_bits;
  bool lookahead;
  const int32_t* earliest = nullptr;
  int pass_no = 0;
// ... 26 lines not shown
    lookahead = tune.plan_lookahead >= 0 ? tune.plan_lookahead != 0 : k >= 24;
    remaining = n_ops;
    scan_window = tune.plan_scan_window;
    tie_break = tune.plan_conflict_cost < 0;
    jit_state = 0x9E3779B97F4A7C15ull * (u64)(tune.plan_jitter + 1);
    for (int b = low; b < low + tune.plan_force_low && b < k && __builtin_popcountll(forced_static) < cap; ++b) forced_static |= 1ull << b;
    anchor = tune.plan_anchor;
  }

  struct Blocked {
    const PassBuilder& pb;
    u64 bt = 0, bd = 0, bx = 0;
    bool admits(size_t i) const { return !(pb.qm[i] & bt) && !(pb.tm[i] & bd) && !((pb.qm[i] & ~pb.xm[i]) & bx); }
    bool add(size_t i) {
      bt |= pb.tm[i] & ~pb.xm[i];
      bx |= pb.xm[i];
      bd |= pb.qm[i] & ~pb.tm[i];
      return bt == pb.all_qubits;
    }
  };

  void begin_pass() {
    while (first < n_ops && done[first]) ++first;
    scan_window = remaining > 4 * (size_t)tune.plan_scan_window ? std::max(1, tune.plan_scan_window * 2 / 3) : tune.plan_scan_window;
  }

  int holds(u64 tile_mask, std::vector<size_t>* out) const {
    Blocked blocked{*this};
    int count = 0, seen = 0;
    for (size_t i = first; i < n_ops && count < tune.max_gates_per_pass; ++i) {
      if (done[i]) continue;
      if (++seen > scan_window) break;
      if (!blocked.admits(i) || (need[i] & ~tile_mask) || (earliest && earliest[i] > pass_no)) {
        if (blocked.add(i)) break;
        continue;
      }
      ++count;
      if (out) out->push_back(i);
    }
    return count;
  }
  static int conflicts(u64 mask) {
    int c = 0;
    for (int b = 13; b <= 16; ++b) c += 2 * (int)(((mask >> b) & (mask >> (b + 7)) & 1));
    for (int b = 18; b <= 19; ++b) c += (int)(((mask >> b) & (mask >> (b + 8)) & 1));
    return c;
  }
  int penalty(u64 mask) const { return tune.plan_conflict_cost > 0 ? tune.plan_conflict_cost * conflicts(mask) / 2 : 0; }
  unsigned jitter() { jit_state ^= jit_state << 13; jit_state ^= jit_state >> 7; jit_state ^= jit_state << 17; return (unsigned)(jit_state >> 33); }
  int keyed(int count, u64 mask) {
    if (tune.plan_jitter > 0) return (count - (int)(jitter() % 8 == 0) - (int)(jitter() % 16 == 0)) * 64 + (int)(jitter() % 64);
    return tie_break ? count * 64 - conflicts(mask) : count;
  }
  static u64 mask_of(const std::vector<int>& bits, size_t n) { u64 m = 0; for (size_t i = 0; i < n && i < bits.size(); ++i) m |= 1ull << bits[i]; return m; }

  bool grow_memo_on = false;
  std::vector<std::pair<u64, u64>> grow_memo;
  u64 grow(u64 mask) {
    const bool memo = grow_memo_on && tune.plan_jitter <= 0;
    const size_t known = grow_memo.size();
    std::vector<u64> path;
    while (__builtin_popcountll(mask) < cap) {
      if (memo) {
        size_t at = 0;
        while (at < known && grow_memo[at].first != mask) ++at;
        if (at < known) { mask = grow_memo[at].second; break; }
        path.push_back(mask);
      }
      int pick = -1, pick_count = -(1 << 20);
      for (int b = low; b < k; ++b) {
        if ((mask >> b) & 1) continue;
        const int c = keyed(holds(mask | (1ull << b), nullptr) - penalty(mask | (1ull << b)), mask | (1ull << b));
        if (c > pick_count) { pick_count = c; pick = b; }
      }
      if (pick < 0) break;
      mask |= 1ull << pick;
    }
    for (u64 through : path) grow_memo.push_back({through, mask});
    return mask;
  }

  u64 first_come(u64 forced, std::vector<int>* claimed) const {
    const int n_forced = __builtin_popcountll(forced);
    Blocked blocked{*this};
    u64 mask = forced;
    int count = 0, seen = 0;
    for (size_t i = first; i < n_ops && count < tune.max_gates_per_pass; ++i) {
      if (done[i]) continue;
      if (++seen > scan_window) break;
      bool ok = blocked.admits(i);
      const u64 extra = need[i] & ~mask;
      if (ok && (n_forced + (int)claimed->size() + __builtin_popcountll(extra) > cap || (extra & rank_bits))) ok = false;
      if (!ok) { if (blocked.add(i)) break; continue; }
      for (u64 e = extra; e; e &= e - 1) claimed->push_back(__builtin_ctzll(e));
      mask |= extra;
      ++count;
    }
    return mask;
  }

  void candidates(std::vector<u64>* out, size_t max_seed, size_t seed_step, u64 prev, bool always = false) {
    u64 forced = forced_static;
    if (anchor > 0 && prev) {
      for (int picked = 0; picked < anchor && picked < cap; ++picked) {
        int pick = -1, pick_count = -(1 << 20);
        for (int b = low; b < k; ++b) {
          if (!((prev >> b) & 1) || ((forced >> b) & 1)) continue;
          const int c = holds(forced | (1ull << b), nullptr);
          if (c > pick_count) { pick_count = c; pick = b; }
        }
        if (pick < 0) break;
        forced |= 1ull << pick;
      }
    }
    std::vector<int> claimed;
    first_come(forced, &claimed);
    out->clear();
    out->push_back(forced | mask_of(claimed, claimed.size()));
    if (!((lookahead || always) && k - low > cap) || holds(out->front(), nullptr) >= kSaturated) return;
    for (size_t seed = 0; seed <= max_seed && seed <= claimed.size(); seed += seed_step)
      out->push_back(grow(forced | mask_of(claimed, seed)));
  }

  std::vector<int> filled(std::vector<int> high) const {
    for (int b = low; (int)high.size() < cap && b < k; ++b)
      if (std::find(high.begin(), high.end(), b) == high.end()) high.push_back(b);
    std::sort(high.begin(), high.end());
    return high;
  }
  std::vector<int> bits_of(u64 mask) const {
    std::vector<int> high;
    for (int b = low; b < k; ++b) if ((mask >> b) & 1) high.push_back(b);
    return high;
  }

  void emit(const std::vector<size_t>& members, const std::vector<int>& high, std::vector<TileGroup>* groups, std::vector<char>* emitted) const {
    emitted->assign(members.size(), 0);
    GroupEmitter::emit(ops, members, high, T, groups, emitted);
    if (lookahead && tune.tile_direct && tune.tile_last_search && T == kTileBitsMax) {
      auto trips = [&](const std::vector<TileGroup>& g) {
        return g.empty() ? 1 << 20 : (int)g.size() + (g.front().s[0] < kTileLow) + (g.back().s[0] < kTileLow);
      };
      auto count = [](const std::vector<char>& e) { size_t c = 0; for (char x : e) c += x != 0; return c; };
      std::vector<char> emitted2(members.size(), 0);
      std::vector<TileGroup> groups2;
      GroupEmitter::emit(ops, members, high, T, &groups2, &emitted2, true);
      if (count(emitted2) > count(*emitted) || (count(emitted2) == count(*emitted) && trips(groups2) < trips(*groups))) {
        groups->swap(groups2);
        emitted->swap(emitted2);
      }
    }
  }

  u64 choose_tile(const TileHint* hint, int pass, u64 prev_mask, bool depth2) {
    if (hint && pass < hint->n) {
      const u64 m = hint->masks[pass] & all_qubits & ~((1ull << low) - 1);
      if (m && __builtin_popcountll(m) <= cap && holds(m, nullptr) > 0) return m;
    }
    candidates(&cands, 6, 2, prev_mask);
    u64 best_mask = cands[0];
    int best_score = -(1 << 20);
    for (size_t ci = 0; ci < cands.size(); ++ci) {
      trial.clear();
      int score = std::min(holds(cands[ci], &trial), kSaturated) - penalty(cands[ci]);
      if (depth2 && cands.size() > 1 && trial.size() < remaining) {
        const size_t first_saved = first;
        for (size_t i : trial) done[i] = 1;
        while (first < n_ops && done[first]) ++first;
        candidates(&cands2, 4, 4, cands[ci]);
        int next_best = 0;
        for (u64 m2 : cands2) next_best = std::max(next_best, std::min(holds(m2, nullptr), kSaturated) - penalty(m2));
        for (size_t i : trial) done[i] = 0;
        first = first_saved;
        score += next_best;
      } else if (depth2 && trial.size() >= remaining) {
        score += 2 * kSaturated;
      }
      score = keyed(score, cands[ci]);
      if (score > best_score) { best_score = score; best_mask = cands[ci]; }
    }
    return best_mask;
  }

  u64 keep_needed(const std::vector<size_t>& members, u64 avoid, std::vector<int>* high) const {
    u64 needed = 0;
    for (size_t i : members) needed |= need[i];
    std::vector<int> kept;
    for (int b : *high) if ((needed >> b) & 1) kept.push_back(b);
    for (int b = low; (int)kept.size() < cap && b < k; ++b)
      if (!((avoid >> b) & 1) && std::find(kept.begin(), kept.end(), b) == kept.end()) kept.push_back(b);
    *high = kept;
    return needed;
  }
  double account(const std::vector<size_t>& members, const std::vector<char>& emitted, size_t* n_emitted) {
    double alg_bytes = 0;
    *n_emitted = 0;
    for (size_t mi = 0; mi < members.size(); ++mi)
      if (emitted[mi]) {
        const FusedOp& o = ops[members[mi]];
        const int halvings = o.kind == TG_PHASE ? o.nbits : (o.control >= 0 ? 1 : o.halvings);
        alg_bytes += 32.0 * (double)((1ull << k) >> halvings) + 32.0 * (double)(1ull << k) * o.absorbed;
        done[members[mi]] = 1; --remaining; ++*n_emitted;
      }
    return alg_bytes;
  }
};

#ifdef QSIM_PROBES
static std::vector<int> probe_int_list(const char* name) {
  std::vector<int> bits;
  if (const char* e = getenv(name))
    for (const char* p = e; *p;) { bits.push_back(atoi(p)); while (*p && *p != ',') ++p; if (*p) ++p; }
  return bits;
}
#endif
static void probe_tile_bits(int k, int low, int cap, std::vector<int>* high_io) {
#ifdef QSIM_PROBES
  std::vector<int>& high = *high_io;
  const int mode = tuning().debug_skip_gates;
  if (mode == 2) for (int j = 0; j < cap; ++j) high[j] = low + j;
  if (mode == 3) for (int j = 0; j < cap; ++j) high[j] = k - cap + j;
  if (mode == 4) {
    const std::vector<int> bits = probe_int_list("QSIM_DEBUG_TILE_BITS");
    if ((int)bits.size() == cap) { high = bits; std::sort(high.begin(), high.end()); }
  }
#endif
}
static void probe_strip_gates(std::vector<TileGroup>* groups) {
#ifdef QSIM_PROBES
  if (tuning().debug_skip_gates) {
    groups->resize(1);
    (*groups)[0].gates.clear();
  }
#endif
}
static void probe_remap_tile(int T, int cap, TileArgs* a) {
#ifdef QSIM_PROBES
  std::vector<int> bits = probe_int_list("QSIM_DEBUG_REMAP_TILE");
  if ((int)bits.size() == cap && T == kTileBitsMax) {
    std::sort(bits.begin(), bits.end());
    uint8_t map[64];
    for (int b = 0; b < 64; ++b) map[b] = (uint8_t)b;
    for (int j = 0; j < cap; ++j) map[a->h[j]] = (uint8_t)bits[(size_t)j];
    for (int j = 0; j < cap; ++j) { a->lay_in[j] = map[a->lay_in[j]]; a->lay_out[j] = map[a->lay_out[j]]; }
    for (int j = 0; j < cap; ++j) a->h[j] = (uint8_t)bits[(size_t)j];
  }
#endif
}

template <class Sink>
static int plan_fused(int k, const std::vector<FusedOp>& ops_in, int* n_passes, Sink&& sink, const TileHint* hint = nullptr,
                      PeekPlan* peek = nullptr) {
  const Tuning& tune = tuning();
  const std::vector<FusedOp> ops = planned_ops(ops_in);
  PassBuilder pb(k, ops, peek ? peek->n_total : k);
  const int T = pb.T;
  *n_passes = 0;
  if (peek) {
    pb.remaining = 0;
    for (size_t i = 0; i < pb.n_ops; ++i) { pb.done[i] = peek->done[i] != 0; pb.remaining += !pb.done[i]; }
    peek->tile_mask = peek->need_mask = 0;
    peek->members->clear();
  }
  const bool depth2 = tune.plan_lookahead >= 0 ? tune.plan_lookahead >= 2 : k >= 26;
  u64 prev_mask = 0;
  while (pb.remaining) {
    pb.begin_pass();
    pb.pass_no = *n_passes;
    pb.earliest = (hint && hint->earliest && *n_passes < hint->n && !tune.tile_commute_fuse) ? hint->earliest : nullptr;
    u64 best_mask = pb.choose_tile(hint, *n_passes, prev_mask, depth2);
    std::vector<size_t> members;
    pb.holds(best_mask, &members);
    if (members.empty() && pb.earliest) {
      pb.earliest = nullptr;
      best_mask = pb.choose_tile(hint, *n_passes, prev_mask, depth2);
      pb.holds(best_mask, &members);
    }
    std::vector<int> high = pb.bits_of(best_mask);
    if (peek) {
      if (members.empty()) { *n_passes = 0; return QSIM_OK; }
      peek->need_mask = pb.keep_needed(members, peek->avoid, &high);
    }
    if (members.empty()) return fail(QSIM_ERR_INVALID, "internal: fused planner made no progress");
    high = pb.filled(high);
    prev_mask = PassBuilder::mask_of(high, high.size());
    probe_tile_bits(k, pb.low, pb.cap, &high);
    TileArgs a;
    std::memset(&a, 0, sizeof a);
    a.T = T;
    for (size_t j = 0; j < high.size(); ++j) a.h[j] = (uint8_t)high[j];
    std::vector<char> emitted;
    std::vector<TileGroup> groups;
    pb.emit(members, high, &groups, &emitted);
    size_t n_emitted = 0;
    const double alg_bytes = pb.account(members, emitted, &n_emitted);
    if (!n_emitted) return fail(QSIM_ERR_INVALID, "internal: fused planner emitted nothing");
    if (peek) {
      for (int b : high) peek->tile_mask |= 1ull << b;
      for (size_t mi = 0; mi < members.size(); ++mi) if (emitted[mi]) peek->members->push_back(members[mi]);
      *n_passes = 1;
      return QSIM_OK;
    }
    probe_strip_gates(&groups);
    int rc = serialize_pass(groups, &a);
    if (rc) return rc;
    probe_remap_tile(T, pb.cap, &a);
    if (tune.debug_stats) {
      size_t descs = 0;
      for (const TileGroup& g : groups) descs += g.gates.size();
      std::fprintf(stderr, "[qsim] pass %d: %zu gates, %zu groups, %zu descriptors\n", *n_passes, n_emitted, groups.size(), descs);
    }
    rc = sink(a, T, alg_bytes, *n_passes == 0, pb.remaining == 0);
    if (rc) return rc;
    ++*n_passes;
  }
  return QSIM_OK;
}
```

quantum_simulations_amd/csrc/tile_search.h:

```cpp
struct SearchNode { int parent; u64 mask; };
struct SearchState {
  std::vector<char> done;
  size_t remaining;
  int parent;
  u64 mask;
  long rank;
  int conflicts;
  u64 hash;
};

constexpr int kSearchBeamDefault = 8;
constexpr size_t kSearchPairSeeds = 10;
constexpr int kSearchBeamMax = 4096;

struct SearchBound {
  const std::atomic<int>* best;
  bool need_bits;
  bool cut;
};

static int planned_tiles(int k, const std::vector<FusedOp>& ops, const TileHint* hint, std::vector<u64>* masks, int* n_passes) {
  masks->clear();
  return plan_fused(k, ops, n_passes, [&](TileArgs& a, int T, double, bool, bool) {
    u64 m = 0;
// ... 182 lines not shown
      for (int seen = best.load(); passes < seen && !best.compare_exchange_weak(seen, passes);) {}
    }
  };
  const int nt = (int)std::max<size_t>(1, std::min<size_t>((size_t)std::max(1, ts->n_threads), std::min<size_t>(n, 64)));
  std::vector<std::thread> pool;
  for (int t = 1; t < nt; ++t) pool.emplace_back(work);
  work();
  for (std::thread& t : pool) t.join();
  if (bad.load()) return fail(QSIM_ERR_INVALID, "internal: an op list of a pass search could not be planned");
  ts->best = best.load();
  for (size_t t = 0; t < n && ts->bounded; ++t)
    if (ts->passes[t] != ts->best) {
      ts->masks[t].clear();
      ts->passes[t] = -1;
    }
  return QSIM_OK;
}

static void triple_ops(int k, const LineTriple& t, int n_ops, const int32_t* nq, const int32_t* qubits, const double* mats,
                       std::vector<FusedOp>* ops, std::vector<int32_t>* origin = nullptr) {
  std::vector<int32_t> lay((size_t)k);
  triple_layout(k, t, lay.data());
  for (int i = 0; i < n_ops; ++i) {
    const int32_t q[2] = {lay[qubits[2 * i]], nq[i] == 2 ? lay[qubits[2 * i + 1]] : -1};
    FusedOp o;
    if (!classify_op(nq[i], q, mats + 32 * (size_t)i, &o)) continue;
    ops->push_back(o);
    if (origin) origin->push_back(i);
  }
}

static int plan_search_triples(int k, int n_ops, const int32_t* nq, const int32_t* qubits, const double* mats,
                               const std::vector<LineTriple>& triples, ListSearch* ts) {
  const bool bounded = ts->bounded;
  const int rc = plan_search_lists(k, triples.size(), [&](size_t t, std::vector<FusedOp>* ops) {
    triple_ops(k, triples[t], n_ops, nq, qubits, mats, ops);
  }, ts);
  for (size_t t = 0; t < triples.size() && !rc && !bounded; ++t) if (ts->passes[t] != ts->best) ts->masks[t].clear();
  return rc;
}

struct CyclePlan {
  bool found = false;
  int32_t plain = 0;
  int32_t passes[3] = {0, 0, 0};
  std::vector<uint8_t> tail;
  std::vector<u64> masks[3];
};

static bool replay_pass_of(int k, const std::vector<FusedOp>& ops, const std::vector<u64>& masks, std::vector<int32_t>* pass_of) {
  pass_of->assign(ops.size(), -1);
  PassBuilder pb(k, ops, k);
  std::vector<size_t> members;
  std::vector<char> emitted;
  std::vector<TileGroup> groups;
  for (size_t p = 0; p < masks.size() && pb.remaining; ++p) {
    pb.begin_pass();
    pb.pass_no = (int)p;
    members.clear();
    pb.holds(masks[p], &members);
    if (members.empty()) return false;
    pb.emit(members, pb.filled(pb.bits_of(masks[p])), &groups, &emitted);
    for (size_t mi = 0; mi < members.size(); ++mi) if (emitted[mi]) (*pass_of)[members[mi]] = (int32_t)p;
    size_t n_emitted = 0;
    pb.account(members, emitted, &n_emitted);
    if (!n_emitted) return false;
  }
  return pb.remaining == 0;
}

static int plan_search_cycle(int k, int n_ops, const int32_t* nq, const int32_t* qubits, const double* mats,
                             const std::vector<LineTriple>& triples, const int32_t* plain_passes, int beam, int n_threads,
                             std::vector<CyclePlan>* out) {
  const size_t n = triples.size();
  out->assign(n, CyclePlan());
  std::vector<std::vector<FusedOp>> L(n);
  std::vector<std::vector<int32_t>> origin(n);
  for (size_t t = 0; t < n; ++t) triple_ops(k, triples[t], n_ops, nq, qubits, mats, &L[t], &origin[t]);
  ListSearch ls;
  ls.beam = beam;
  ls.n_threads = n_threads;
  int rc = plan_search_lists(k, n, [&](size_t t, std::vector<FusedOp>* ops) {
    *ops = L[t];
    ops->insert(ops->end(), L[t].begin(), L[t].end());
  }, &ls);
  if (rc) return rc;
  std::vector<size_t> cyc;
  std::vector<std::vector<FusedOp>> part[3];
  std::vector<int32_t> pass_of;
  for (size_t t = 0; t < n; ++t) {
    if (ls.passes[t] < 0) continue;
    std::vector<FusedOp> twice = L[t];
    twice.insert(twice.end(), L[t].begin(), L[t].end());
    const std::vector<FusedOp> planned = planned_ops(twice);
    const size_t m = L[t].size();
    if (planned.size() != twice.size() || !replay_pass_of(k, planned, ls.masks[t], &pass_of)) continue;
    int32_t cut = 1 << 30;
    for (size_t i = m; i < 2 * m; ++i) cut = std::min(cut, pass_of[i]);
    std::vector<FusedOp> A, B;
    CyclePlan& c = (*out)[t];
    c.tail.assign((size_t)n_ops, 0);
    for (size_t i = 0; i < m; ++i) {
      (pass_of[i] < cut ? A : B).push_back(L[t][i]);
      c.tail[(size_t)origin[t][i]] = pass_of[i] >= cut;
    }
    if (A.empty() || B.empty()) continue;
    std::vector<FusedOp> BA = B;
    BA.insert(BA.end(), A.begin(), A.end());
    cyc.push_back(t);
    part[0].push_back(A); part[1].push_back(BA); part[2].push_back(B);
  }
  if (cyc.empty()) return QSIM_OK;
  ListSearch steady;
  steady.beam = beam;
  steady.n_threads = n_threads;
  rc = plan_search_lists(k, cyc.size(), [&](size_t j, std::vector<FusedOp>* ops) { *ops = part[1][j]; }, &steady);
  if (rc) return rc;
  std::vector<size_t> kept;
  for (size_t j = 0; j < cyc.size(); ++j) if (steady.passes[j] == steady.best) kept.push_back(j);
  ListSearch ends;
  ends.beam = beam;
  ends.n_threads = n_threads;
  ends.bounded = false;
  const size_t per = plain_passes ? 2 : 3;
  rc = plan_search_lists(k, per * kept.size(), [&](size_t j, std::vector<FusedOp>* ops) {
    const size_t which = j % per, at = kept[j / per];
    *ops = which == 0 ? part[0][at] : which == 1 ? part[2][at] : L[cyc[at]];
  }, &ends);
  if (rc) return rc;
  for (size_t i = 0; i < kept.size(); ++i) {
    const size_t t = cyc[kept[i]];
    CyclePlan& c = (*out)[t];
    c.plain = plain_passes ? plain_passes[t] : ends.passes[per * i + 2];
    c.passes[0] = ends.passes[per * i];
    c.passes[1] = steady.passes[kept[i]];
    c.passes[2] = ends.passes[per * i + 1];
    c.masks[0] = ends.masks[per * i];
    c.masks[1] = steady.masks[kept[i]];
    c.masks[2] = ends.masks[per * i + 1];
    bool ok = c.passes[1] < c.plain;
    for (int w = 0; w < 3 && ok; ++w) {
      std::vector<u64> replay;
      int replay_passes = 0;
      const std::vector<uint64_t> named(c.masks[w].begin(), c.masks[w].end());
      const TileHint hint = {named.data(), (int)named.size()};
      if ((rc = planned_tiles(k, part[w][kept[i]], &hint, &replay, &replay_passes))) return rc;
      ok = replay_passes == c.passes[w] && (int)named.size() == c.passes[w];
    }
    c.found = ok;
  }
  return QSIM_OK;
}

static int plan_balance(int k, const std::vector<FusedOp>& ops_in, const std::vector<u64>& masks, const double* mem_us,
                        const EngineCosts& ec, bool place, std::vector<int32_t>* earliest, std::vector<double>* eng_before,
                        std::vector<double>* eng_after) {
  const std::vector<FusedOp> ops = planned_ops(ops_in);
  const size_t n_pass = masks.size(), n_ops = ops.size();
  earliest->assign(ops_in.size(), 0);
  eng_before->assign(n_pass, 0.0);
  eng_after->assign(n_pass, 0.0);
  if (n_ops != ops_in.size() || !n_pass) return QSIM_OK;
  std::vector<size_t> members;
  std::vector<char> emitted;
  std::vector<TileGroup> groups;
  std::vector<int32_t> pass_of(n_ops, -1);
  PassBuilder rules(k, ops, k);
  auto replay = [&](const int32_t* place, std::vector<double>* eng) {
    PassBuilder pb(k, ops, k);
    for (size_t p = 0; p < n_pass && pb.remaining; ++p) {
      pb.begin_pass();
      pb.pass_no = (int)p;
      pb.earliest = place;
      members.clear();
      pb.holds(masks[p], &members);
      if (members.empty()) return false;
      pb.emit(members, pb.filled(pb.bits_of(masks[p])), &groups, &emitted);
      (*eng)[p] = ec.of_pass(groups, k);
      for (size_t mi = 0; mi < members.size(); ++mi) if (emitted[mi]) pass_of[members[mi]] = (int32_t)p;
      size_t n_emitted = 0;
      pb.account(members, emitted, &n_emitted);
      if (!n_emitted) return false;
    }
    return pb.remaining == 0;
  };
  if (!replay(nullptr, eng_before)) return QSIM_OK;
  *eng_after = *eng_before;
  if (!place) return QSIM_OK;
  const double scale = std::ldexp(1.0, k - (int)ec.v[QSIM_ENGINE_COST_FIT_QUBITS]);
  std::vector<double> slack(n_pass);
  for (size_t p = 0; p < n_pass; ++p) slack[p] = mem_us[p] - (*eng_before)[p];
  std::vector<int32_t> window(n_ops, -1);
  for (size_t i = 0; i < n_ops; ++i) {
    if (ops[i].ntargets) continue;
    window[i] = (int32_t)n_pass - 1;
    for (size_t j = i + 1; j < n_ops; ++j)
      if (rules.tm[j] & rules.qm[i]) window[i] = std::min(window[i], pass_of[j]);
  }
  std::vector<int32_t> placed(n_ops, 0);
  bool any = false;
  for (size_t p = 0; p + 1 < n_pass; ++p)
    for (size_t i = n_ops; i-- > 0 && slack[p] < 0;) {
      if (pass_of[i] != (int32_t)p || window[i] <= (int32_t)p) continue;
      const double us = ec.of_family(priced_family(ops[i])) * scale;
      size_t to = p;
      for (size_t q = p + 1; q <= (size_t)window[i]; ++q) if (to == p || slack[q] > slack[to]) to = q;
      if (slack[to] < us) continue;
      placed[i] = (int32_t)to;
      slack[to] -= us;
      slack[p] += us;
      any = true;
    }
  if (!any) return QSIM_OK;
  std::vector<double> check(n_pass, 0.0);
  if (!replay(placed.data(), &check)) return QSIM_OK;
  double before = 0, after = 0;
  for (size_t p = 0; p < n_pass; ++p) { before += std::max(mem_us[p], (*eng_before)[p]); after += std::max(mem_us[p], check[p]); }
  if (!(after < before)) return QSIM_OK;
  *earliest = placed;
  *eng_after = check;
  return QSIM_OK;
}
```

quantum_simulations_amd/kernel/device.py:

```python
from __future__ import annotations

import ctypes as C

import numpy as np

from quantum_simulations_amd import _lib


def _mat_ptr(U: np.ndarray, dim: int):
    m = np.ascontiguousarray(U, dtype=np.complex128)
    if m.shape != (dim, dim):
        raise ValueError(f"expected a {dim}x{dim} matrix, got shape {m.shape}")
    return m, _lib.ptr(m)


Z_TERMS_PER_CALL = 16384

_TERM_ARRAYS = {"x": (np.uint64, "x masks"), "z": (np.uint64, "z masks"), "coeffs": (np.float64, "coefficients"), "angles": (np.float64, "angles")}


def _term_arrays(call: str, **arrays) -> list:
    out = [np.ascontiguousarray(a, dtype=_TERM_ARRAYS[kind][0]).reshape(-1) for kind, a in arrays.items()]
    if len({a.size for a in out}) > 1:
        raise ValueError(f"{call}: " + ", ".join(f"{a.size} {_TERM_ARRAYS[kind][1]}" for kind, a in zip(arrays, out)))
    return out


def pack_ops(ops) -> tuple[np.ndarray, np.ndarray, np.ndarray]:
    n = len(ops)
    nq = np.zeros(n, dtype=np.int32)
    qs = np.zeros(2 * n, dtype=np.int32)
    mats = np.zeros((n, 16), dtype=np.complex128)
    for i, (qubits, U) in enumerate(ops):
        nq[i] = len(qubits)
        qs[2 * i: 2 * i + len(qubits)] = qubits
        flat = np.asarray(U, dtype=np.complex128).reshape(-1)
        if flat.size != (4 if len(qubits) == 1 else 16):
            raise ValueError(f"op {i}: matrix size {flat.size} does not fit {len(qubits)} qubit(s)")
        mats[i, : flat.size] = flat
    return nq, qs, mats


def as_packed(ops) -> tuple[np.ndarray, np.ndarray, np.ndarray]:
    if isinstance(ops, tuple) and len(ops) == 3 and isinstance(ops[0], np.ndarray):
        return ops
    return pack_ops(ops)


class DeviceChunk:

    def __init__(self, handle: int, k: int, device: int, keep=None):
        self._h = C.c_void_p(handle)
        self.k = k
        self.device = device
        self._keep = keep

    @classmethod
    def empty(cls, k: int, device: int = 0) -> "DeviceChunk":
        lib = _lib.load()
        h = C.c_void_p()
        _lib.check(lib.qsim_create(device, k, C.byref(h)))
        return cls(h.value, k, device)

    @classmethod
    def zero_state(cls, k: int, device: int = 0, set_amp0: bool = True) -> "DeviceChunk":
        c = cls.empty(k, device)
        c.init_zero(set_amp0)
        return c

    @classmethod
    def from_numpy(cls, arr: np.ndarray, device: int = 0) -> "DeviceChunk":
        n = arr.shape[0]
        if arr.ndim != 1 or n < 1 or n & (n - 1):
            raise ValueError("chunk must be a 1-D array with a power-of-two length")
        c = cls.empty(n.bit_length() - 1, device)
        c.upload(arr)
        return c

    @classmethod
    def wrap_pointer(cls, ptr: int, k: int, device: int, stream: int = 0, keep=None) -> "DeviceChunk":
        lib = _lib.load()
        h = C.c_void_p()
        _lib.check(lib.qsim_wrap(device, C.c_void_p(ptr), k, C.c_void_p(stream), C.byref(h)))
        return cls(h.value, k, device, keep=keep)

    def view(self, offset_amps: int, k: int) -> "DeviceChunk":
        lib = _lib.load()
        h = C.c_void_p()
        _lib.check(lib.qsim_create_view(self._h, offset_amps, k, C.byref(h)))
        return DeviceChunk(h.value, k, self.device, keep=self)

    def close(self) -> None:
        if self._h is not None and self._h.value:
            _lib.load().qsim_destroy(self._h)
            self._h = C.c_void_p()

    def __del__(self):
        try:
            self.close()
        except Exception:
            pass

    def __len__(self) -> int:
        return 1 << self.k

    @property
    def device_ptr(self) -> int:
        return _lib.load().qsim_device_ptr(self._h) or 0

    def init_zero(self, set_amp0: bool = True) -> None:
        _lib.check(_lib.load().qsim_init_zero(self._h, 1 if set_amp0 else 0))

    def init_random(self, seed: int) -> None:
        _lib.check(_lib.load().qsim_init_random(self._h, seed))

    def upload(self, arr: np.ndarray, offset: int = 0) -> None:
        host = np.ascontiguousarray(arr, dtype=np.complex128)
        _lib.check(_lib.load().qsim_upload(self._h, _lib.ptr(host), offset, host.size))

    def download(self, offset: int = 0, count: int | None = None) -> np.ndarray:
        count = len(self) - offset if count is None else count
        out = np.empty(count, dtype=np.complex128)
        _lib.check(_lib.load().qsim_download(self._h, _lib.ptr(out), offset, count))
        return out

    def download_c64(self, offset: int = 0, count: int | None = None) -> np.ndarray:
        count = len(self) - offset if count is None else count
        out = np.empty(count, dtype=np.complex64)
        _lib.check(_lib.load().qsim_download_c64(self._h, _lib.ptr(out), int(offset), int(count)))
        return out

    def upload_c64(self, arr: np.ndarray, offset: int = 0) -> None:
        a = np.ascontiguousarray(arr, dtype=np.complex64)
        _lib.check(_lib.load().qsim_upload_c64(self._h, _lib.ptr(a), int(offset), int(a.size)))

    def copy_from(self, other: "DeviceChunk", variant: int = 0) -> None:
        if variant:
            _lib.check(_lib.load().qsim_copy_variant(self._h, other._h, int(variant)))
        else:
            _lib.check(_lib.load().qsim_copy(self._h, other._h))

    def apply_1q(self, qubit: int, U: np.ndarray) -> None:
        m, p = _mat_ptr(U, 2)
        _lib.check(_lib.load().qsim_apply_1q(self._h, int(qubit), p))

    def apply_2q(self, qa: int, qb: int, U: np.ndarray) -> None:
        m, p = _mat_ptr(U, 4)
        _lib.check(_lib.load().qsim_apply_2q(self._h, int(qa), int(qb), p))

    def apply_fused_k(self, qubits, M: np.ndarray) -> None:
        q = np.asarray(qubits, dtype=np.int32)
        m = np.ascontiguousarray(M, dtype=np.complex128)
        if m.shape != (1 << len(q), 1 << len(q)):
            raise ValueError(f"a {len(q)}-qubit block needs a {1 << len(q)} x {1 << len(q)} matrix, got {m.shape}")
        _lib.check(_lib.load().qsim_apply_fused_k(self._h, len(q), _lib.ptr(q), _lib.ptr(m)))

    def apply_ops_tiled(self, ops, tile_masks) -> int:
        nq, qs, mats = as_packed(ops)
        tm = np.ascontiguousarray(tile_masks, dtype=np.uint64)
        lib = _lib.load()
        _lib.check(lib.qsim_apply_ops_tiled(self._h, len(nq), _lib.ptr(nq), _lib.ptr(qs), _lib.ptr(mats), len(tm), _lib.ptr(tm)))
        return lib.qsim_last_pass_count(self._h)

    def apply_ops_placed(self, ops, tile_masks, earliest) -> int:
        nq, qs, mats = as_packed(ops)
        tm = np.ascontiguousarray(tile_masks, dtype=np.uint64)
        place = np.ascontiguousarray(earliest, dtype=np.int32)
        if len(place) != len(nq):
            raise ValueError("one earliest pass per op expected")
        lib = _lib.load()
        _lib.check(lib.qsim_apply_ops_placed(self._h, len(nq), _lib.ptr(nq), _lib.ptr(qs), _lib.ptr(mats), len(tm), _lib.ptr(tm),
                                             _lib.ptr(place)))
        return lib.qsim_last_pass_count(self._h)

    def apply_cycle(self, cycle: "Cycle") -> int:
        lib = _lib.load()
        _lib.check(lib.qsim_apply_cycle(self._h, cycle._h))
        return lib.qsim_last_pass_count(self._h)

    def apply_ops(self, ops, fused: bool = True) -> int:
        if not len(ops):
            return 0
        nq, qs, mats = as_packed(ops)
        lib = _lib.load()
        fn = lib.qsim_apply_ops if fused else lib.qsim_apply_ops_unfused
        _lib.check(fn(self._h, len(nq), _lib.ptr(nq), _lib.ptr(qs), _lib.ptr(mats)))
        return lib.qsim_last_pass_count(self._h) if fused else len(nq)

    def apply_pauli_rotations(self, x_masks, z_masks, thetas) -> int:
        x, z, th = _term_arrays("apply_pauli_rotations", x=x_masks, z=z_masks, angles=thetas)
        passes = C.c_int(0)
        _lib.check(_lib.load().qsim_apply_pauli_rotations(self._h, int(x.size), _lib.ptr(x), _lib.ptr(z), _lib.ptr(th), C.byref(passes)))
        self.last_rotation_passes = passes.value
        return passes.value

    def apply_diagonal_phase(self, z_masks, coeffs, gamma) -> None:
        z, co = _term_arrays("apply_diagonal_phase", z=z_masks, coeffs=coeffs)
        _lib.check(_lib.load().qsim_apply_diagonal_phase(self._h, int(z.size), _lib.ptr(z), _lib.ptr(co), float(gamma)))

    def diagonal_moments(self, z_masks, coeffs) -> tuple:
        z, co = _term_arrays("diagonal_moments", z=z_masks, coeffs=coeffs)
        out = np.empty(3, dtype=np.float64)
        _lib.check(_lib.load().qsim_diagonal_moments(self._h, int(z.size), _lib.ptr(z), _lib.ptr(co), _lib.ptr(out)))
        return float(out[0]), float(out[1]), float(out[2])

    def apply_diagonal_sum(self, src: "DeviceChunk", z_masks, coeffs, accumulate: bool = False) -> None:
        z, co = _term_arrays("apply_diagonal_sum", z=z_masks, coeffs=coeffs)
        _lib.check(_lib.load().qsim_apply_diagonal_sum(self._h, src._h, int(z.size), _lib.ptr(z), _lib.ptr(co), 1 if accumulate else 0))

    def overlap_diagonal(self, bra: "DeviceChunk", z_masks, coeffs) -> tuple:
        z, co = _term_arrays("overlap_diagonal", z=z_masks, coeffs=coeffs)
        out = np.empty(4, dtype=np.float64)
        _lib.check(_lib.load().qsim_overlap_diagonal(self._h, bra._h, int(z.size), _lib.ptr(z), _lib.ptr(co), _lib.ptr(out)))
        return complex(out[0], out[1]), complex(out[2], out[3])

    def expectation_z_terms(self, z_masks) -> np.ndarray:
        (z,) = _term_arrays("expectation_z_terms", z=z_masks)
        out = np.empty(z.size, dtype=np.float64)
        self.last_z_terms_passes = 0
        for first in range(0, max(z.size, 1), Z_TERMS_PER_CALL):
            part, res = z[first:first + Z_TERMS_PER_CALL], out[first:first + Z_TERMS_PER_CALL]
            passes = C.c_int(0)
            _lib.check(_lib.load().qsim_expectation_z_terms(self._h, int(part.size), _lib.ptr(part), _lib.ptr(res), C.byref(passes)))
            self.last_z_terms_passes += passes.value
        return out

    def apply_pauli_sum(self, src: "DeviceChunk", x_masks, z_masks, coeffs) -> int:
        x, z, co = _term_arrays("apply_pauli_sum", x=x_masks, z=z_masks, coeffs=coeffs)
        passes = C.c_int(0)
        _lib.check(_lib.load().qsim_apply_pauli_sum(self._h, src._h, int(x.size), _lib.ptr(x), _lib.ptr(z), _lib.ptr(co), C.byref(passes)))
        self.last_pauli_sum_passes = passes.value
        return passes.value

    def overlap_pauli(self, bra: "DeviceChunk", x_masks, z_masks) -> np.ndarray:
        x, z = _term_arrays("overlap_pauli", x=x_masks, z=z_masks)
        out = np.empty(x.size, dtype=np.complex128)
        passes = C.c_int(0)
        _lib.check(_lib.load().qsim_overlap_pauli(self._h, bra._h, int(x.size), _lib.ptr(x), _lib.ptr(z), _lib.ptr(out), C.byref(passes)))
        self.last_overlap_passes = passes.value
        return out

    def overlap(self, bra: "DeviceChunk") -> complex:
        return complex(self.overlap_pauli(bra, [0], [0])[0])

    def lincomb(self, dst_coeff, srcs=(), coeffs=(), bras=(), want_norm2: bool = False) -> tuple:
        srcs, bras = list(srcs), list(bras)
        co = np.ascontiguousarray(coeffs, dtype=np.complex128).reshape(-1)
        if co.size != len(srcs):
            raise ValueError(f"lincomb: {len(srcs)} sources, {co.size} coefficients")
        dc = np.array([complex(dst_coeff)], dtype=np.complex128)
        src_h = (C.c_void_p * max(len(srcs), 1))(*[s._h.value for s in srcs])
        bra_h = (C.c_void_p * max(len(bras), 1))(*[b._h.value for b in bras])
        dots = np.empty(len(bras), dtype=np.complex128)
        norm2 = C.c_double(0.0)
        _lib.check(_lib.load().qsim_lincomb(self._h, _lib.ptr(dc), len(srcs), src_h, _lib.ptr(co), len(bras), bra_h, _lib.ptr(dots),
                                            C.byref(norm2) if want_norm2 else None))
        return dots, (norm2.value if want_norm2 else None)

    def dot(self, bra: "DeviceChunk") -> complex:
        return complex(self.lincomb(1.0, bras=[bra])[0][0])

    def apply_ops_io(self, ops, src=None, dst=None, parts: int = 0, src_parts: int = 0, tiles=None) -> int:
        nq, qs, mats = as_packed(ops)
        io = _lib.OpsIo()
        keep = []
        if tiles is not None and len(tiles):
            tm = np.ascontiguousarray(tiles, dtype=np.uint64)
            io.n_tiles, io.tile_masks = len(tm), tm.ctypes.data
            keep.append(tm)
        if src is not None:
            chunk, bits = src
            io.src, io.src_m = chunk._h, len(bits)
            for i, b in enumerate(bits):
                io.src_bits[i] = int(b)
            keep.append(chunk)
        io.own_pattern = -1
        if dst is not None:
            chunk, bits, own_chunk, own_pattern = dst
            io.dst, io.dst_m = chunk._h, len(bits)
            for i, b in enumerate(bits):
                io.dst_bits[i] = int(b)
            if own_chunk is not None and own_pattern >= 0:
                io.dst_own, io.own_pattern = own_chunk._h, int(own_pattern)
            keep += [chunk, own_chunk]
        io.dst_parts = int(parts) if dst is not None else 0
        io.src_parts = int(src_parts) if src is not None else 0
        passes = C.c_int()
        _lib.check(_lib.load().qsim_apply_ops_io(self._h, len(nq), _lib.ptr(nq), _lib.ptr(qs), _lib.ptr(mats), C.byref(io), C.byref(passes)))
        return passes.value

    def own_slab_in_chunk(self) -> bool:
        flag = C.c_int32()
        _lib.check(_lib.load().qsim_apply_ops_io_own_slab(self._h, C.byref(flag)))
        return bool(flag.value)

    def pending_parts(self) -> list:
        n_parts, amps_, launches = C.c_int32(), C.c_uint64(), C.c_int32()
        _lib.check(_lib.load().qsim_apply_ops_io_parts(self._h, C.byref(n_parts), C.byref(amps_), C.byref(launches)))
        self.last_split_launches = launches.value
        return [(j * int(amps_.value), int(amps_.value)) for j in range(n_parts.value)]

    def store_part(self, part: int) -> None:
        _lib.check(_lib.load().qsim_apply_ops_io_part(self._h, int(part)))

    def source_parts(self) -> tuple:
        n_parts, amps_, launches = C.c_int32(), C.c_uint64(), C.c_int32()
        _lib.check(_lib.load().qsim_apply_ops_io_source_parts(self._h, C.byref(n_parts), C.byref(amps_), C.byref(launches)))
        return n_parts.value, int(amps_.value), launches.value

    def load_part(self, part: int) -> None:
        _lib.check(_lib.load().qsim_apply_ops_io_load(self._h, int(part)))

    def sync(self) -> None:
        _lib.check(_lib.load().qsim_sync(self._h))

    def count_nonzero(self, eps: float = 1e-15) -> int:
        n = C.c_uint64()
        _lib.check(_lib.load().qsim_count_nonzero(self._h, float(eps), C.byref(n)))
        return int(n.value)

    def export_nonzero(self, eps: float = 1e-15, capacity: int | None = None):
        if capacity is None:
            capacity = self.count_nonzero(eps)
        idx = np.empty(capacity, dtype=np.uint64)
        amp = np.empty(capacity, dtype=np.complex128)
        n = C.c_uint64()
        _lib.check(_lib.load().qsim_export_nonzero(self._h, float(eps), int(capacity), _lib.ptr(idx), _lib.ptr(amp), C.byref(n)))
        if n.value > capacity:
            return None
        return idx[:n.value], amp[:n.value]

    def norm2(self) -> float:
        out = C.c_double()
        _lib.check(_lib.load().qsim_norm2(self._h, C.byref(out)))
        return out.value

    def probabilities(self, qubits) -> np.ndarray:
        q = np.ascontiguousarray(qubits, dtype=np.int32).reshape(-1)
        if not 1 <= len(q) <= 8:
            raise ValueError(f"probabilities: 1 to 8 qubits expected, got {len(q)}")
        out = np.empty(1 << len(q), dtype=np.float64)
        _lib.check(_lib.load().qsim_probabilities(self._h, len(q), _lib.ptr(q), _lib.ptr(out)))
        return out

    def reduced_density_matrix(self, qubits) -> np.ndarray:
        return self._density_call("reduced_density_matrix", 1, 6, "", qubits)

    def reduced_density_matrix_wide(self, qubits) -> np.ndarray:
        return self._density_call("reduced_density_matrix_wide", 7, 12, " (reduced_density_matrix serves 1 to 6)", qubits)

    def _density_call(self, name: str, lo: int, hi: int, hint: str, qubits) -> np.ndarray:
        q = np.ascontiguousarray(qubits, dtype=np.int32).reshape(-1)
        if not lo <= len(q) <= hi:
            raise ValueError(f"{name}: {lo} to {hi} qubits expected, got {len(q)}{hint}")
        out = np.empty((1 << len(q), 1 << len(q)), dtype=np.complex128)
        _lib.check(getattr(_lib.load(), "qsim_" + name)(self._h, len(q), _lib.ptr(q), _lib.ptr(out)))
        return out

    def expectation_pauli(self, x_masks, z_masks) -> np.ndarray:
        x, z = _term_arrays("expectation_pauli", x=x_masks, z=z_masks)
        out = np.empty(x.size, dtype=np.float64)
        passes = C.c_int(0)
        _lib.check(_lib.load().qsim_expectation_pauli(self._h, int(x.size), _lib.ptr(x), _lib.ptr(z), _lib.ptr(out), C.byref(passes)))
        self.last_expectation_passes = passes.value
        return out

    def expectation(self, obs, l2p=None) -> float:
        from quantum_simulations_amd.observable import as_pauli_sum
        obs = as_pauli_sum(obs, self.k if l2p is None else len(l2p))
        x, z = obs.masks(l2p)
        return obs.value(self.expectation_pauli(x, z))

    def sample(self, randnums) -> np.ndarray:
        r = np.ascontiguousarray(randnums, dtype=np.float64).reshape(-1)
        out = np.empty(r.size, dtype=np.uint64)
        total, passes = C.c_double(0.0), C.c_int(0)
        _lib.check(_lib.load().qsim_sample(self._h, int(r.size), _lib.ptr(r), _lib.ptr(out), C.byref(total), C.byref(passes)))
        self.last_sample_total, self.last_sample_passes = total.value, passes.value
        return out

    def max_abs_err_closed_form(self, kind: str, n_total: int, base_index: int = 0,
                                log_to_phys=None) -> float:
        out = C.c_double()
        code = {"ghz": 0, "ghz_qft": 1}[kind]
        perm = None if log_to_phys is None else np.asarray(log_to_phys, dtype=np.int32)
        _lib.check(_lib.load().qsim_max_abs_err_closed_form_perm(self._h, code, n_total, base_index, _lib.ptr(perm), C.byref(out)))
        return out.value

    def fingerprint(self, n_total: int, base_index: int = 0, log_to_phys=None, seed: int = 0,
                    sel_mask: int = 0, sel_value: int = 0) -> complex:
        out = (C.c_double * 2)()
        perm = None if log_to_phys is None else np.asarray(log_to_phys, dtype=np.int32)
        _lib.check(_lib.load().qsim_fingerprint(self._h, n_total, base_index, _lib.ptr(perm), seed, sel_mask, sel_value, out))
        return complex(out[0], out[1])

    def time_begin(self) -> None:
        _lib.check(_lib.load().qsim_time_begin(self._h))

    def time_end(self) -> float:
        ms = C.c_float()
        _lib.check(_lib.load().qsim_time_end(self._h, C.byref(ms)))
        return ms.value

    def profile_begin(self) -> None:
        _lib.check(_lib.load().qsim_profile_begin(self._h))

    def profile_end(self) -> list[dict]:
        entries = (_lib.ProfileEntry * 32)()
        n = C.c_int()
        _lib.check(_lib.load().qsim_profile_end(self._h, 32, C.byref(n), C.cast(entries, C.c_void_p)))
        out = []
        for e in entries[: min(n.value, 32)]:
            out.append({"kernel": e.kernel.decode(), "launches": int(e.launches),
                        "total_ms": float(e.total_ms), "algorithmic_bytes": float(e.algorithmic_bytes),
                        "hbm_bytes": float(e.hbm_bytes), "streaming_launches": int(e.streaming_launches)})
        return out

    def pack_half(self, bit: int, value: int, buf: "DeviceChunk") -> None:
        _lib.check(_lib.load().qsim_pack_half(self._h, bit, value, buf._h))

    def unpack_half(self, bit: int, value: int, buf: "DeviceChunk") -> None:
        _lib.check(_lib.load().qsim_unpack_half(self._h, bit, value, buf._h))

    def pack_bits(self, bits, pattern: int, buf: "DeviceChunk", buf_offset: int = 0) -> None:
        b = np.asarray(bits, dtype=np.int32)
        _lib.check(_lib.load().qsim_pack_bits(self._h, len(b), _lib.ptr(b), int(pattern), buf._h, int(buf_offset)))

    def unpack_bits(self, bits, pattern: int, buf: "DeviceChunk", buf_offset: int = 0) -> None:
        b = np.asarray(bits, dtype=np.int32)
        _lib.check(_lib.load().qsim_unpack_bits(self._h, len(b), _lib.ptr(b), int(pattern), buf._h, int(buf_offset)))

    def pack_all(self, bits, buf: "DeviceChunk", skip_pattern: int = -1, piece: int = 0, n_pieces: int = 1) -> None:
        b = np.asarray(bits, dtype=np.int32)
        _lib.check(_lib.load().qsim_pack_all(self._h, len(b), _lib.ptr(b), buf._h, int(skip_pattern),
                                             int(piece), int(n_pieces)))

    def unpack_all(self, bits, buf: "DeviceChunk", skip_pattern: int = -1, piece: int = 0, n_pieces: int = 1) -> None:
        b = np.asarray(bits, dtype=np.int32)
        _lib.check(_lib.load().qsim_unpack_all(self._h, len(b), _lib.ptr(b), buf._h, int(skip_pattern),
                                               int(piece), int(n_pieces)))


class Cycle:

    def __init__(self, k: int, head, steady, tail):
        keep, lists = [], []
        for ops, masks, earliest in (head, steady, tail):
            nq, qs, mats = as_packed(ops)
            tm = np.ascontiguousarray(masks if masks is not None else [], dtype=np.uint64)
            place = None if earliest is None else np.ascontiguousarray(earliest, dtype=np.int32)
            if place is not None and len(place) != len(nq):
                raise ValueError("one earliest pass per op expected")
            keep.append((nq, qs, mats, tm, place))
            lists.append(_lib.CycleList(len(nq), _lib.ptr(nq).value, _lib.ptr(qs).value, _lib.ptr(mats).value, len(tm),
                                        _lib.ptr(tm).value if len(tm) else None, None if place is None else _lib.ptr(place).value))
        counts = np.zeros(3, dtype=np.int32)
        self._h = C.c_void_p()
        _lib.check(_lib.load().qsim_cycle_create(int(k), C.byref(lists[0]), C.byref(lists[1]), C.byref(lists[2]), _lib.ptr(counts),
                                                 C.byref(self._h)))
        self.k = k
        self.passes = tuple(int(x) for x in counts)

    def close(self) -> None:
        if self._h is not None and self._h.value:
            _lib.load().qsim_cycle_destroy(self._h)
            self._h = C.c_void_p()

    def __del__(self):
        try:
            self.close()
        except Exception:
            pass


def split_piece_count(k: int, m: int, parts: int) -> int:
    return int(_lib.load().qsim_split_piece_count(int(k), int(m), int(parts)))


def plan_expectation(k: int, x_masks) -> tuple[np.ndarray, np.ndarray]:
    x = np.ascontiguousarray(x_masks, dtype=np.uint64).reshape(-1)
    pass_of = np.empty(x.size, dtype=np.int32)
    tiles = np.empty(max(x.size, 1), dtype=np.uint64)
    n = C.c_int(0)
    _lib.check(_lib.load().qsim_plan_expectation(int(k), int(x.size), _lib.ptr(x), _lib.ptr(pass_of), _lib.ptr(tiles), C.byref(n)))
    return pass_of, tiles[: n.value].copy()


def sample_block_bits() -> int:
    return int(_lib.load().qsim_sample_block_bits())


def sample_locate(block_cdf, randnums) -> tuple[np.ndarray, np.ndarray]:
    cdf = np.ascontiguousarray(block_cdf, dtype=np.float64).reshape(-1)
    r = np.ascontiguousarray(randnums, dtype=np.float64).reshape(-1)
    block = np.empty(r.size, dtype=np.uint64)
    local = np.empty(r.size, dtype=np.float64)
    _lib.check(_lib.load().qsim_sample_locate(int(cdf.size), _lib.ptr(cdf), int(r.size), _lib.ptr(r), _lib.ptr(block), _lib.ptr(local)))
    return block, local


def device_count() -> int:
    n = C.c_int()
    _lib.check(_lib.load().qsim_device_count(C.byref(n)))
    return n.value


def relayout_plan(rank: int, world: int, k: int, local_bits, global_bits, n_pieces: int = 4) -> dict:
    lb, gb = np.asarray(local_bits, dtype=np.int32), np.asarray(global_bits, dtype=np.int32)
    n_p, n_peers, own = C.c_int32(), C.c_int32(), C.c_int32()
    peers, offs, part = np.zeros(7, dtype=np.int32), np.zeros(7, dtype=np.uint64), C.c_uint64()
    _lib.check(_lib.load().qsim_comm_relayout_plan(int(rank), int(world), int(k), len(lb), _lib.ptr(lb), _lib.ptr(gb), int(n_pieces),
                                                   C.byref(n_p), C.byref(n_peers), C.byref(own), _lib.ptr(peers), _lib.ptr(offs), C.byref(part)))
    return {"pieces": n_p.value, "own_pattern": own.value, "peers": [int(x) for x in peers[:n_peers.value]],
            "slab_offsets": [int(x) for x in offs[:n_peers.value]], "piece_amps": int(part.value)}


class Comm:

    ID_BYTES = 128

    def __init__(self, device: int, rank: int, world: int, uid: bytes):
        if len(uid) != self.ID_BYTES:
            raise ValueError("the unique id has 128 bytes")
        self._h = C.c_void_p()
        buf = (C.c_uint8 * self.ID_BYTES).from_buffer_copy(uid)
        _lib.check(_lib.load().qsim_comm_init(device, rank, world, C.cast(buf, C.c_void_p), C.byref(self._h)))
        self.rank, self.world = rank, world

    @staticmethod
    def unique_id() -> bytes:
        buf = (C.c_uint8 * Comm.ID_BYTES)()
        _lib.check(_lib.load().qsim_comm_get_unique_id(C.cast(buf, C.c_void_p)))
        return bytes(buf)

    def exchange(self, peers, send: DeviceChunk, send_off, recv: DeviceChunk, recv_off, count: int) -> None:
        p = np.asarray(peers, dtype=np.int32)
        so, ro = np.asarray(send_off, dtype=np.uint64), np.asarray(recv_off, dtype=np.uint64)
        _lib.check(_lib.load().qsim_comm_exchange(self._h, len(p), _lib.ptr(p), send._h, _lib.ptr(so), recv._h, _lib.ptr(ro), int(count)))

    def exchange_bg(self, peers, send: DeviceChunk, send_off, recv: DeviceChunk, recv_off, count: int) -> int:
        p = np.asarray(peers, dtype=np.int32)
        so, ro = np.asarray(send_off, dtype=np.uint64), np.asarray(recv_off, dtype=np.uint64)
        ticket = C.c_uint32()
        _lib.check(_lib.load().qsim_comm_exchange_bg(self._h, len(p), _lib.ptr(p), send._h, _lib.ptr(so), recv._h, _lib.ptr(ro),
                                                     int(count), C.byref(ticket)))
        return ticket.value

    def join(self, chunk: DeviceChunk) -> None:
        _lib.check(_lib.load().qsim_comm_join(self._h, chunk._h))

    def wait(self, chunk: DeviceChunk, ticket: int) -> None:
        _lib.check(_lib.load().qsim_comm_wait(self._h, chunk._h, int(ticket)))

    def relayout(self, state: DeviceChunk, buf0: DeviceChunk, buf1: DeviceChunk, local_bits, global_bits,
                 n_pieces: int = 4) -> None:
        lb, gb = np.asarray(local_bits, dtype=np.int32), np.asarray(global_bits, dtype=np.int32)
        _lib.check(_lib.load().qsim_comm_relayout(self._h, state._h, buf0._h, buf1._h, len(lb), _lib.ptr(lb), _lib.ptr(gb), int(n_pieces)))

    def relayout_loopback(self, state: DeviceChunk, buf0: DeviceChunk, buf1: DeviceChunk, local_bits, global_bits,
                          n_pieces: int, as_rank: int, as_world: int) -> None:
        lb, gb = np.asarray(local_bits, dtype=np.int32), np.asarray(global_bits, dtype=np.int32)
        _lib.check(_lib.load().qsim_comm_relayout_loopback(self._h, state._h, buf0._h, buf1._h, len(lb), _lib.ptr(lb), _lib.ptr(gb),
                                                           int(n_pieces), int(as_rank), int(as_world)))

    def relayout_fused(self, shard: DeviceChunk, send: DeviceChunk, recv: DeviceChunk, before, after, local_bits,
                       global_bits, n_pieces: int = 4, as_rank: int = 0, as_world: int = 0) -> int:
        lb, gb = np.asarray(local_bits, dtype=np.int32), np.asarray(global_bits, dtype=np.int32)
        keep, lists = [], []
        for ops in (before, after):
            ol = _lib.OpList()
            if ops:
                nq, qs, mats = pack_ops(ops)
                keep.append((nq, qs, mats))
                ol.n_ops, ol.nq, ol.qubits, ol.mats = len(nq), nq.ctypes.data, qs.ctypes.data, mats.ctypes.data
            lists.append(ol)
        passes = C.c_int()
        _lib.check(_lib.load().qsim_comm_relayout_fused(self._h, shard._h, send._h, recv._h, C.byref(lists[0]), C.byref(lists[1]),
                                                        len(lb), _lib.ptr(lb), _lib.ptr(gb),
                                                        int(n_pieces), int(as_rank), int(as_world), C.byref(passes)))
        return passes.value

    def apply_2q_quad_remote(self, shard: DeviceChunk, buf: DeviceChunk, ranks, my_index: int, U) -> None:
        m, p = _mat_ptr(U, 4)
        r = np.asarray(ranks, dtype=np.int32)
        _lib.check(_lib.load().qsim_apply_2q_quad_remote(self._h, shard._h, buf._h, _lib.ptr(r), int(my_index), p))

    def apply_1q_pair_remote(self, shard: DeviceChunk, buf: DeviceChunk, partner: int, my_side: int, U) -> None:
        m, p = _mat_ptr(U, 2)
        _lib.check(_lib.load().qsim_apply_1q_pair_remote(self._h, shard._h, buf._h, int(partner), int(my_side), p))

    def apply_2q_pair_qa_local_remote(self, shard, buf, partner: int, my_side: int, qa: int, U) -> None:
        m, p = _mat_ptr(U, 4)
        _lib.check(_lib.load().qsim_apply_2q_pair_qa_local_remote(self._h, shard._h, buf._h, int(partner),
                                                                  int(my_side), int(qa), p))

    def apply_2q_pair_qb_local_remote(self, shard, buf, partner: int, my_side: int, qb: int, U) -> None:
        m, p = _mat_ptr(U, 4)
        _lib.check(_lib.load().qsim_apply_2q_pair_qb_local_remote(self._h, shard._h, buf._h, int(partner),
                                                                  int(my_side), int(qb), p))

    def close(self) -> None:
        if self._h is not None and self._h.value:
            _lib.load().qsim_comm_destroy(self._h)
            self._h = C.c_void_p()

    def __del__(self):
        try:
            self.close()
        except Exception:
            pass
```

quantum_simulations_amd/kernel/planner.py:

```python
from __future__ import annotations

import ctypes as C

import numpy as np

from quantum_simulations_amd import _lib
from quantum_simulations_amd._lib import ptr
from quantum_simulations_amd.kernel.device import as_packed

IMAGE_BYTES = 4096
STREAM_OFF = 192
PASS_IMAGE = np.dtype([("amp", "<u8"), ("nrec", "<i4"), ("T", "<i4"), ("h", "u1", (11,)), ("order", "u1"), ("ntiles", "<u4"),
                       ("lay_in", "u1", (12,)), ("lay_out", "u1", (12,)), ("amp_out", "<u8"),
                       ("amp_out_own", "<u8"), ("own_mask", "<u8"), ("own_value", "<u8"),
                       ("slab_in", "u1", (40,)), ("slab_out", "u1", (40,)), ("nbits", "u1"), ("perm", "u1"), ("reserved", "u1", (22,)),
                       ("stream", "u1", (IMAGE_BYTES - STREAM_OFF,))])
assert PASS_IMAGE.itemsize == IMAGE_BYTES
_FIRST_BUFFER = 64


def tile_bits(image) -> list:
    return [int(b) for b in image["h"][:int(image["T"]) - 3]]


def tile_masks(images) -> np.ndarray:
    return np.array([sum(1 << b for b in tile_bits(img)) for img in images], dtype=np.uint64)


def _plan(n: int, ops, tiles, images, earliest=None) -> tuple:
    nq, qubits, mats = as_packed(ops)
    lib, count = _lib.load(), C.c_int32()
    head = (n, len(nq), ptr(nq), ptr(qubits), ptr(mats))
    tail = (ptr(images), 0 if images is None else images.nbytes, C.byref(count))
    tm = np.ascontiguousarray(tiles if tiles is not None else [], dtype=np.uint64)
    if len(tm) and earliest is not None:
        place = np.ascontiguousarray(earliest, dtype=np.int32)
        if len(place) != len(nq):
            raise ValueError("one earliest pass per op expected")
        return lib.qsim_plan_ops_placed(*head, len(tm), ptr(tm), ptr(place), *tail), count.value
    rc = lib.qsim_plan_ops_tiled(*head, len(tm), ptr(tm), *tail) if len(tm) else lib.qsim_plan_ops(*head, *tail)
    return rc, count.value


def plan_ops(n: int, ops, tiles=None, earliest=None) -> np.ndarray:
    room = _FIRST_BUFFER
    while True:
        images = np.zeros(room, dtype=PASS_IMAGE)
        rc, count = _plan(n, ops, tiles, images, earliest)
        if rc != _lib.QSIM_ERR_INVALID or count < room:
            _lib.check(rc)
            return images[:count]
        room *= 2


def lower_images(images) -> tuple:
    out = np.ascontiguousarray(images, dtype=PASS_IMAGE).copy()
    count = C.c_int32()
    _lib.check(_lib.load().qsim_lower_pass_images(ptr(out), len(out), C.byref(count)))
    return out, count.value


def pass_count(n: int, ops, tiles=None, earliest=None) -> int:
    rc, count = _plan(n, ops, tiles, None, earliest)
    _lib.check(rc)
    return count


def balance(n: int, ops, tiles, pass_memory_us, engine_costs, place: bool = True) -> tuple:
    nq, qubits, mats = as_packed(ops)
    tm = np.ascontiguousarray(tiles, dtype=np.uint64)
    mem = np.ascontiguousarray(pass_memory_us, dtype=np.float64)
    costs = np.ascontiguousarray(engine_costs, dtype=np.float64)
    if len(mem) != len(tm):
        raise ValueError("one memory time per named pass expected")
    earliest = np.zeros(len(nq), dtype=np.int32) if place else None
    before, after = np.zeros(len(tm)), np.zeros(len(tm))
    _lib.check(_lib.load().qsim_plan_balance(n, len(nq), ptr(nq), ptr(qubits), ptr(mats), len(tm), ptr(tm), ptr(mem), ptr(costs),
                                             len(costs), ptr(earliest), ptr(before), ptr(after)))
    return earliest, before, after


def tiles_per_workgroup(n: int, tile_bits: int, fixed_bits: int = 0) -> int:
    rc = int(_lib.load().qsim_tiles_per_workgroup(int(n), int(tile_bits), int(fixed_bits)))
    if rc < 0:
        _lib.check(rc)
    return rc


def search_tiles(n: int, ops, beam: int = 0) -> np.ndarray:
    nq, qubits, mats = as_packed(ops)
    count = C.c_int32()
    out = np.zeros(len(nq), dtype=np.uint64)
    _lib.check(_lib.load().qsim_plan_search(n, len(nq), ptr(nq), ptr(qubits), ptr(mats), beam, ptr(out), len(out), C.byref(count)))
    return out[:count.value].copy()


HISTOGRAM_BINS = 64
TRIPLES_UNBOUNDED, TRIPLES_NEED_BITS = 1, 2
_MASK_ROOM = 1 << 22


def search_triples(n: int, ops, triples=None, beam: int = 0, threads: int = 1, flags: int = 0) -> dict:
    nq, qubits, mats = as_packed(ops)
    tri = None if triples is None else np.ascontiguousarray(triples, dtype=np.int32).reshape(-1, 3)
    if tri is not None and not len(tri):
        raise ValueError("an empty list of triples (None searches them all)")
    m = n * (n - 1) * (n - 2) // 6 if tri is None else len(tri)
    best, count = C.c_int32(), C.c_int32()
    index, found = np.zeros(m, dtype=np.int32), np.zeros((m, 3), dtype=np.int32)
    room = min(_MASK_ROOM, m * max(1, len(nq)))
    masks, hist = np.zeros(room, dtype=np.uint64), np.zeros(HISTOGRAM_BINS, dtype=np.int32)
    _lib.check(_lib.load().qsim_plan_search_triples(n, len(nq), ptr(nq), ptr(qubits), ptr(mats), 0 if tri is None else m, ptr(tri),
                                                    beam, threads, flags, C.byref(best), C.byref(count), ptr(index), ptr(found),
                                                    ptr(masks), room, ptr(hist)))
    k, p = count.value, best.value
    histogram = {int(b): int(c) for b, c in enumerate(hist[:-1]) if c}
    if hist[-1]:
        histogram[None] = int(hist[-1])
    return {"passes": p, "index": index[:k].copy(), "triples": found[:k].copy(), "masks": masks[:k * p].reshape(k, p).copy(),
            "searched": m, "histogram": histogram}


def search_cycle(n: int, ops, triples, plain_passes=None, beam: int = 0, threads: int = 1) -> list:
    nq, qubits, mats = as_packed(ops)
    tri = np.ascontiguousarray(triples, dtype=np.int32).reshape(-1, 3)
    m = len(tri)
    if not m:
        raise ValueError("an empty list of triples")
    plain = None if plain_passes is None else np.ascontiguousarray(plain_passes, dtype=np.int32)
    if plain is not None and len(plain) != m:
        raise ValueError("one plain pass count per triple expected")
    count = C.c_int32()
    index, found, passes = np.zeros(m, dtype=np.int32), np.zeros((m, 3), dtype=np.int32), np.zeros((m, 4), dtype=np.int32)
    tail = np.zeros((m, max(1, len(nq))), dtype=np.uint8)
    room = min(_MASK_ROOM, 3 * m * max(1, len(nq)))
    masks = np.zeros(room, dtype=np.uint64)
    _lib.check(_lib.load().qsim_plan_search_cycle(n, len(nq), ptr(nq), ptr(qubits), ptr(mats), m, ptr(tri), ptr(plain), beam, threads,
                                                  C.byref(count), ptr(index), ptr(found), ptr(passes), ptr(tail), ptr(masks), room))
    out, at = [], 0
    for f in range(count.value):
        cuts = at + np.concatenate([[0], np.cumsum(passes[f, 1:])])
        out.append({"index": int(index[f]), "triple": [int(q) for q in found[f]], "plain": int(passes[f, 0]), "head": int(passes[f, 1]),
                    "steady": int(passes[f, 2]), "tail": int(passes[f, 3]), "is_tail": tail[f, :len(nq)].astype(bool),
                    "masks": [masks[cuts[w]:cuts[w + 1]].copy() for w in range(3)]})
        at = int(cuts[3])
    return out


def rewrite_ops(n: int, ops, stats: dict = None, engine_costs=None) -> list:
    nq, qubits, mats = as_packed(ops)
    room = 2 * len(nq) + n
    out_nq, out_q = np.zeros(room, dtype=np.int32), np.zeros(2 * room, dtype=np.int32)
    out_m = np.zeros((room, 16), dtype=np.complex128)
    count, need = C.c_int32(), np.zeros(2, dtype=np.int32)
    costs = None if engine_costs is None else np.ascontiguousarray(engine_costs, dtype=np.float64)
    _lib.check(_lib.load().qsim_rewrite_ops_priced(n, len(nq), ptr(nq), ptr(qubits), ptr(mats), ptr(out_nq), ptr(out_q), ptr(out_m),
                                                   room, C.byref(count), ptr(need), ptr(costs), 0 if costs is None else len(costs)))
    if stats is not None:
        stats.update(ops_in=len(nq), ops_out=int(count.value), need_tile_in=int(need[0]), need_tile_out=int(need[1]))
    return [([int(out_q[2 * i])], out_m[i, :4].reshape(2, 2).copy()) if out_nq[i] == 1 else
            ([int(out_q[2 * i]), int(out_q[2 * i + 1])], out_m[i].reshape(4, 4).copy()) for i in range(count.value)]


def count_layouts(n: int, ops, layouts, threads: int) -> np.ndarray:
    nq, qubits, mats = as_packed(ops)
    lay = np.ascontiguousarray(layouts, dtype=np.int32)
    out = np.zeros(len(lay), dtype=np.int32)
    _lib.check(_lib.load().qsim_plan_count_layouts(n, len(nq), ptr(nq), ptr(qubits), ptr(mats), len(lay), ptr(lay), ptr(out), threads))
    return out


def peek_pass(k: int, n: int, nq, qubits, mats, done, members, avoid: int = 0, hint: int = 0) -> tuple:
    mask, need, count = C.c_uint64(), C.c_uint64(), C.c_int32()
    _lib.check(_lib.load().qsim_plan_peek_pass(k, n, len(nq), ptr(nq), ptr(qubits), ptr(mats), ptr(done), avoid, hint,
                                               C.byref(mask), C.byref(need), C.byref(count), ptr(members)))
    return int(mask.value), int(need.value), [int(i) for i in members[:count.value]]


def plan_pauli_rotations(n: int, x_masks) -> tuple:
    x = np.ascontiguousarray(x_masks, dtype=np.uint64).reshape(-1)
    pass_of = np.empty(x.size, dtype=np.int32)
    tiles = np.empty(max(x.size, 1), dtype=np.uint64)
    count = C.c_int(0)
    _lib.check(_lib.load().qsim_plan_pauli_rotations(int(n), int(x.size), ptr(x), ptr(pass_of), ptr(tiles), C.byref(count)))
    return pass_of, tiles[:count.value].copy()
```

quantum_simulations_amd/runner/engine.py:

```python
from __future__ import annotations

from contextlib import contextmanager

import numpy as np

from quantum_simulations_amd.circuit.fusion import batch_levels
from quantum_simulations_amd.circuit.io import levelize, validate_circuit_dict
from quantum_simulations_amd.kernel import gates as gate_table, planner
from quantum_simulations_amd.kernel.device import DeviceChunk
from quantum_simulations_amd.runner import measure
from quantum_simulations_amd.runner.layout_search import (_count_passes, choose_plan_layout, layout_swaps,
                                                          pass_memory_us, priced_variant)
from quantum_simulations_amd.state_calls import StateCalls


def gate_ops(cd: dict) -> list:
    return [(g["qubits"], gate_table.gate_matrix(g["gate"], g["params"])) for g in cd["gates"]]


class GpuPlan(list):
    tiles: list
    placed: list | None = None
    l2p: list | None = None
    model_ms: tuple | None = None
    cycle = None


class SingleGpuEngine(StateCalls):

    world = 1
    rank = 0
    LAYOUT_MIN_QUBITS = 26
    LAYOUT_MIN_REPEATS = 8
    LAYOUT_CANDIDATES = 63
    LAYOUT_BEAM = 0
    LAYOUT_FINALISTS = 8
    CYCLES = True
    ENGINE_PRICING = True

    def __init__(self, n_qubits: int, device: int = 0, mode: str = "fused", layout: str = "auto", tune_on_device: bool = False):
        if layout not in ("auto", "search", "identity"):
            raise ValueError("layout must be 'auto', 'search' or 'identity'")
        self.n = n_qubits
        self.mode = mode
        self.layout_mode = layout
        self.tune_on_device = bool(tune_on_device)
        self.state = DeviceChunk.empty(n_qubits, device)
        self.l2p: list | None = None
        self._zero = False
        self._work: DeviceChunk | None = None

    def init_zero_state(self) -> None:
        self.state.init_zero(True)
        self.l2p, self._zero = None, True

    def init_random_state(self, seed: int) -> None:
        self.state.init_random(seed)
        self.l2p, self._zero = None, False

    def norm2(self) -> float:
        return self.state.norm2()

    def state_vector(self) -> np.ndarray:
        psi = self.state.download()
        if self.l2p is None:
            return psi
        from quantum_simulations_amd.circuit.staging import permute_state
        return permute_state(psi, self.l2p)

    @contextmanager
    def _second_chunk(self):
        if self._work is None:
            self._work = self._new_chunk()
        yield self._work

    def _state_written(self) -> None:
        self._zero = False

    def logical_index(self, offset: int, count: int) -> np.ndarray:
        x = offset + np.arange(count, dtype=np.int64)
        if self.l2p is None:
            return x
        y = np.zeros_like(x)
        for q, p in enumerate(self.l2p):
            y |= ((x >> p) & 1) << q
        return y

    def plan(self, circuit_dict: dict, repeats: int = 1) -> GpuPlan:
        cd = validate_circuit_dict(circuit_dict)
        if cd["number_of_qubits"] != self.n:
            raise ValueError(f"circuit has {cd['number_of_qubits']} qubits, engine has {self.n}")
        from quantum_simulations_amd.kernel.device import pack_ops
        if self.mode == "per-gate":
            plan = GpuPlan([pack_ops(gate_ops(cd))])
            plan.tiles = [None]
            return plan
        return self.plan_batches([p["local_ops"] for p in batch_levels(levelize(cd), self.n)], repeats)

    def plan_batches(self, batches, repeats: int = 1) -> GpuPlan:
        from quantum_simulations_amd.kernel.device import pack_ops
        search = self.layout_mode == "search" or (self.layout_mode == "auto" and repeats >= self.LAYOUT_MIN_REPEATS)
        if not search or self.n < self.LAYOUT_MIN_QUBITS:
            plan = GpuPlan([pack_ops(ops) for ops in batches])
            plan.tiles = [None] * len(batches)
            return plan
        import time
        t0 = time.perf_counter()
        tune = self.tune_on_device and self._zero
        plans = self.finalist_plans(batches, self.LAYOUT_FINALISTS if tune else 4, repeats)
        chosen = plans[0]
        if tune and len(plans) > 1:
            timed = self._time_on_device(plans)
            chosen = plans[int(np.argmin(timed))]
            chosen.layout_info["tuned_on_device_ms"] = [round(t, 3) for t in timed]
        chosen.layout_info["seconds"] = round(time.perf_counter() - t0, 3)
        return chosen

    def finalist_plans(self, batches, n_finalists: int, repeats: int = 1) -> list:
        from quantum_simulations_amd.kernel.device import Cycle, pack_ops
        cycle_repeats = repeats if self.CYCLES and len(batches) == 1 and repeats >= self.LAYOUT_MIN_REPEATS else 0
        own_batches, rewrite = batches, {"ops_in": 0, "ops_out": 0, "need_tile_in": 0, "need_tile_out": 0}
        from quantum_simulations_amd.runner import engine_cost
        costs = engine_cost.table() if self.ENGINE_PRICING else None
        batches = []
        for ops in own_batches:
            stats = {}
            batches.append(planner.rewrite_ops(self.n, ops, stats))
            for key in rewrite:
                rewrite[key] += stats[key]
        priced = None if costs is None else [planner.rewrite_ops(self.n, ops, None, costs) for ops in own_batches]
        own_identity = int(_count_passes(self.n, own_batches, np.arange(self.n, dtype=np.int32)[None, :], 1)[0])
        finalists = choose_plan_layout(self.n, batches, self.LAYOUT_CANDIDATES, n_finalists=n_finalists,
                                       all_finalists=True, beam=self.LAYOUT_BEAM, engine_costs=costs, priced_batches=priced,
                                       cycle_repeats=cycle_repeats)

        def build(l2p, masks, info):
            cyc = info.pop("cycle", None)
            if cyc is not None:
                info.pop("planned", None)
                info.pop("placed", None)
                plan = GpuPlan([pack_ops(cyc["planned"][1])])
                plan.cycle = Cycle(self.n, *zip(cyc["planned"], cyc["tiles"], cyc["placed"]))
                plan.tiles, plan.placed = masks, [cyc["placed"][1]]
                plan.l2p = None if l2p == list(range(self.n)) else l2p
                plan.model_ms = info["model_ms"]
                plan.layout_info = dict(info, passes_identity=own_identity, rewrite=dict(rewrite), cycle_passes=dict(
                    zip(("head", "steady", "tail"), plan.cycle.passes), plain=cyc["plain_passes"]))
                return plan
            planned = info.pop("planned", None) or [[([l2p[q] for q in qs], U) for qs, U in ops] for ops in batches]
            plan = GpuPlan([pack_ops(ops) for ops in planned])
            plan.tiles = masks
            plan.placed = info.pop("placed", None)
            plan.l2p = None if l2p == list(range(self.n)) else l2p
            plan.model_ms = info["model_ms"]
            plan.layout_info = dict(info, passes_identity=own_identity, rewrite=dict(rewrite))
            return plan
        return [build(*f) for f in finalists]

    def _time_on_device(self, plans) -> list:
        timed = []
        for p in plans:
            self.init_zero_state()
            self.execute(p)
            ms = []
            for _ in range(2):
                self.state.time_begin()
                self.execute(p)
                ms.append(self.state.time_end())
            timed.append(min(ms))
        self.init_zero_state()
        return timed

    def _adopt_layout(self, l2p) -> None:
        if l2p == self.l2p or (l2p is None and self.l2p == list(range(self.n))):
            return
        if self._zero:
            self.l2p = l2p
            return
        SW = gate_table.SWAP()
        swaps = [([a, b], SW) for a, b in layout_swaps(self.l2p, l2p, self.n)]
        if swaps:
            self.state.apply_ops(swaps)
        self.l2p = l2p

    def execute(self, plan) -> None:
        self._adopt_layout(getattr(plan, "l2p", None))
        self._zero = False
        self.last_passes = 0
        if getattr(plan, "cycle", None) is not None and self.mode != "per-gate":
            self.last_passes = self.state.apply_cycle(plan.cycle)
            return
        tiles = getattr(plan, "tiles", None) or [None] * len(plan)
        placed = getattr(plan, "placed", None) or [None] * len(plan)
        for ops, masks, place in zip(plan, tiles, placed):
            if masks is not None and place is not None and self.mode != "per-gate":
                self.last_passes += self.state.apply_ops_placed(ops, masks, place)
            elif masks is not None and self.mode != "per-gate":
                self.last_passes += self.state.apply_ops_tiled(ops, masks)
            else:
                self.last_passes += self.state.apply_ops(ops, fused=self.mode != "per-gate")

    def passes_per_step(self, plan: list) -> int:
        return getattr(self, "last_passes", sum(len(ops[0]) for ops in plan))

    def barrier(self) -> None:
        self.state.sync()

    def max_over_ranks(self, value: float) -> float:
        return value

    def profile_begin(self) -> None:
        self.state.profile_begin()

    def profile_end(self) -> list[dict]:
        return self.state.profile_end()

    def sweep_gates(self, n: int, reps: int = 5) -> dict:
        if n == self.n:
            self.l2p, self._zero = None, False
        return measure.sweep_gates(self.state, n, reps)

    def copy_ceiling(self, reps: int = 7) -> dict:
        return measure.copy_ceiling(self.state, reps)

    def stream_ceiling(self, reps: int = 5) -> dict:
        return measure.stream_ceiling(self.state, reps)

    def prefix_parity(self, circuit_dict: dict, n_gates: int, expected: np.ndarray) -> float:
        cd = validate_circuit_dict(circuit_dict)
        prefix = {"number_of_qubits": self.n, "gates": cd["gates"][:n_gates]}
        self.init_zero_state()
        tune, self.tune_on_device = self.tune_on_device, False
        try:
            plan = self.plan(prefix, repeats=self.LAYOUT_MIN_REPEATS)
        finally:
            self.tune_on_device = tune
        self.execute(plan)
        worst = 0.0
        step = 1 << 24
        for off in range(0, 1 << self.n, step):
            cnt = min(step, (1 << self.n) - off)
            got = self.state.download(off, cnt)
            want = expected[off:off + cnt] if self.l2p is None else expected[self.logical_index(off, cnt)]
            worst = max(worst, float(np.max(np.abs(got - want))))
        self.last_parity_layout = None if self.l2p is None else list(self.l2p)
        return worst

    def close(self) -> None:
        if self._work is not None:
            self._work.close()
            self._work = None
        self.state.close()


def _planned_tile_masks(n: int, ops) -> np.ndarray:
    return planner.tile_masks(planner.plan_ops(n, ops)) if len(ops) >= 2 else np.zeros(0, dtype=np.uint64)


def make_engine(n_qubits: int, world: int = 1, rank: int = 0, local_rank: int = 0,
                mode: str = "fused", **kw):
    if world == 1:
        return SingleGpuEngine(n_qubits, device=local_rank, mode=mode, layout=kw.get("layout", "auto"),
                               tune_on_device=kw.get("tune_on_device", False))
    from quantum_simulations_amd.runner.distributed import DistributedEngine
    return DistributedEngine(n_qubits, world, rank, local_rank, mode=mode, **kw)
```

Baseline: 44140.

## Use engine-cost-priced beam search to form gate groups within fused tile passes

Adds a cost-aware group emitter that runs a small beam search over which tile bits each group owns. It prices each gate record by its engine family and predication cost and picks the cheapest grouping. This pricing is wired into plan_balance, cycle creation, plan image generation and a new apply_ops_priced path that the runner uses whenever the plan carries engine costs. The aim is to cut per-pass compute/instruction cost inside fused kernels, at the price of more host-side planning work and reliance on how accurate the cost model is.

Measured after the change: 44410 (median of 6 runs). About the same (+0.6%).

```diff
diff --git a/include/qsim_hip.h b/include/qsim_hip.h
--- a/include/qsim_hip.h
+++ b/include/qsim_hip.h
@@ -59,6 +59,8 @@
 } qsim_cycle_list;
 int qsim_cycle_create(int n_local_qubits, const qsim_cycle_list* head, const qsim_cycle_list* steady, const qsim_cycle_list* tail,
                       int32_t* n_passes, qsim_cycle** out);
+int qsim_cycle_create_priced(int n_local_qubits, const qsim_cycle_list* head, const qsim_cycle_list* steady, const qsim_cycle_list* tail,
+                             const double* engine_costs, int n_engine_costs, int32_t* n_passes, qsim_cycle** out);
 int qsim_cycle_destroy(qsim_cycle* cycle);
 int qsim_apply_cycle(qsim_chunk* c, const qsim_cycle* cycle);
 
@@ -122,6 +124,15 @@
 int qsim_plan_ops_placed(int n_local_qubits, int n_ops, const int32_t* nq, const int32_t* qubits, const double* mats,
                          int n_tiles, const uint64_t* tile_masks, const int32_t* earliest_pass, void* out,
                          uint64_t out_capacity_bytes, int32_t* n_passes);
+int qsim_apply_ops_priced(qsim_chunk* c, int n_ops, const int32_t* nq, const int32_t* qubits, const double* mats,
+                          int n_tiles, const uint64_t* tile_masks, const int32_t* earliest_pass, const double* engine_costs,
+                          int n_engine_costs);
+int qsim_plan_ops_priced(int n_local_qubits, int n_ops, const int32_t* nq, const int32_t* qubits, const double* mats,
+                         int n_tiles, const uint64_t* tile_masks, const int32_t* earliest_pass, const double* engine_costs,
+                         int n_engine_costs, void* out, uint64_t out_capacity_bytes, int32_t* n_passes);
+int qsim_plan_group_prices(int n_local_qubits, int n_ops, const int32_t* nq, const int32_t* qubits, const double* mats,
+                           int n_tiles, const uint64_t* tile_masks, const int32_t* earliest_pass, const double* engine_costs,
+                           int n_engine_costs, double* engine_us_unpriced, double* engine_us_priced);
 int qsim_rewrite_ops_priced(int n_qubits, int n_ops, const int32_t* nq, const int32_t* qubits, const double* mats,
                             int32_t* out_nq, int32_t* out_qubits, double* out_mats, int out_capacity, int32_t* n_out,
                             int32_t* need_tile, const double* engine_costs, int n_engine_costs);
diff --git a/quantum_simulations_amd/_lib.py b/quantum_simulations_amd/_lib.py
--- a/quantum_simulations_amd/_lib.py
+++ b/quantum_simulations_amd/_lib.py
@@ -58,6 +58,7 @@
     "qsim_plan_search_cycle": (C.c_int, [C.c_int, C.c_int, _P, _P, _P, C.c_int, _P, _P, C.c_int, C.c_int, _P, _P, _P, _P, _P, _P,
                                          C.c_uint64]),
     "qsim_cycle_create": (C.c_int, [C.c_int, _P, _P, _P, _P, C.POINTER(_P)]),
+    "qsim_cycle_create_priced": (C.c_int, [C.c_int, _P, _P, _P, _P, C.c_int, _P, C.POINTER(_P)]),
     "qsim_cycle_destroy": (C.c_int, [_P]),
     "qsim_apply_cycle": (C.c_int, [_P, _P]),
     "qsim_rewrite_ops": (C.c_int, [C.c_int, C.c_int, _P, _P, _P, _P, _P, _P, C.c_int, _P, _P]),
@@ -65,6 +66,9 @@
     "qsim_apply_ops_tiled": (C.c_int, [_P, C.c_int, _P, _P, _P, C.c_int, _P]),
     "qsim_apply_ops_placed": (C.c_int, [_P, C.c_int, _P, _P, _P, C.c_int, _P, _P]),
     "qsim_plan_ops_placed": (C.c_int, [C.c_int, C.c_int, _P, _P, _P, C.c_int, _P, _P, _P, C.c_uint64, _P]),
+    "qsim_apply_ops_priced": (C.c_int, [_P, C.c_int, _P, _P, _P, C.c_int, _P, _P, _P, C.c_int]),
+    "qsim_plan_ops_priced": (C.c_int, [C.c_int, C.c_int, _P, _P, _P, C.c_int, _P, _P, _P, C.c_int, _P, C.c_uint64, _P]),
+    "qsim_plan_group_prices": (C.c_int, [C.c_int, C.c_int, _P, _P, _P, C.c_int, _P, _P, _P, C.c_int, _P, _P]),
     "qsim_plan_balance": (C.c_int, [C.c_int, C.c_int, _P, _P, _P, C.c_int, _P, _P, _P, C.c_int, _P, _P, _P]),
     "qsim_choose_layout": (C.c_int, [C.c_int, C.c_int, _P, C.c_int, _P, _P, _P, C.c_uint64, C.c_int, _P, C.POINTER(C.c_double), C.POINTER(C.c_double)]),
     "qsim_plan_count_layouts": (C.c_int, [C.c_int, C.c_int, _P, _P, _P, C.c_int, _P, _P, C.c_int]),
diff --git a/quantum_simulations_amd/csrc/abi_gates.h b/quantum_simulations_amd/csrc/abi_gates.h
--- a/quantum_simulations_amd/csrc/abi_gates.h
+++ b/quantum_simulations_amd/csrc/abi_gates.h
@@ -66,9 +66,13 @@
 }
 
 static int apply_ops_fused(qsim_chunk* c, int n_ops, const int32_t* nq, const int32_t* qubits, const double* mats,
-                           int n_tiles, const uint64_t* tile_masks, const char* what, const int32_t* earliest_pass = nullptr) {
+                           int n_tiles, const uint64_t* tile_masks, const char* what, const int32_t* earliest_pass = nullptr,
+                           const double* engine_costs = nullptr, int n_engine_costs = 0) {
   int rc = validate_ops(c, n_ops, nq, qubits, mats);
   if (rc) return rc;
+  EngineCosts ec;
+  const bool priced = engine_costs_from(engine_costs, n_engine_costs, &ec);
+  if (engine_costs && !priced) return fail(QSIM_ERR_INVALID, "%s: the cost table has %d entries, not %d", what, n_engine_costs, (int)QSIM_ENGINE_COST_COUNT);
   if (n_tiles < 0 || (n_tiles && !tile_masks)) return fail(QSIM_ERR_INVALID, "%s: bad tile list", what);
   if ((rc = require_no_parts(c, what))) return rc;
   if (n_ops < 2 || c->k < kTileMinChunk || c->k > kTileMaxQubits) {
@@ -86,7 +90,7 @@
     hint.earliest = placed.data();
   }
   rc = run_fused(c, ops, RawOps{n_ops, nq, qubits, mats}, n_tiles ? &hint : nullptr, nullptr, &passes,
-                 [&](TileArgs& a, int T, double alg_bytes, bool) { return dispatch_planned(c, a, T, alg_bytes); });
+                 [&](TileArgs& a, int T, double alg_bytes, bool) { return dispatch_planned(c, a, T, alg_bytes); }, priced ? &ec : nullptr);
   c->last_passes = passes;
   return rc;
 }
@@ -101,6 +105,11 @@
 int qsim_apply_ops_placed(qsim_chunk* c, int n_ops, const int32_t* nq, const int32_t* qubits, const double* mats,
                           int n_tiles, const uint64_t* tile_masks, const int32_t* earliest_pass) {
   return apply_ops_fused(c, n_ops, nq, qubits, mats, n_tiles, tile_masks, "qsim_apply_ops_placed", earliest_pass);
+}
+int qsim_apply_ops_priced(qsim_chunk* c, int n_ops, const int32_t* nq, const int32_t* qubits, const double* mats,
+                          int n_tiles, const uint64_t* tile_masks, const int32_t* earliest_pass, const double* engine_costs,
+                          int n_engine_costs) {
+  return apply_ops_fused(c, n_ops, nq, qubits, mats, n_tiles, tile_masks, "qsim_apply_ops_priced", earliest_pass, engine_costs, n_engine_costs);
 }
 
 }
@@ -112,7 +121,7 @@
 };
 static std::atomic<u64> g_cycle_ids{0};
 
-static int cycle_passes(int k, const qsim_cycle_list* l, const char* part, PassList* out) {
+static int cycle_passes(int k, const qsim_cycle_list* l, const char* part, const EngineCosts* costs, PassList* out) {
   if (!l || l->n_ops < 1 || l->n_tiles < 0 || (l->n_tiles && !l->tile_masks))
     return fail(QSIM_ERR_INVALID, "qsim_cycle_create: bad %s list", part);
   int rc = check_op_list(l->n_ops, l->nq, l->qubits, l->mats, k, kQubitOfPlan);
@@ -132,7 +141,7 @@
     lower_unit_real(&a);
     made->push_back(CachedPass{a, T, alg_bytes});
     return (int)QSIM_OK;
-  }, l->n_tiles ? &hint : nullptr);
+  }, l->n_tiles ? &hint : nullptr, nullptr, costs);
   *out = made;
   return rc;
 }
@@ -140,14 +149,24 @@
 extern "C" {
 int qsim_cycle_create(int n_local_qubits, const qsim_cycle_list* head, const qsim_cycle_list* steady, const qsim_cycle_list* tail,
                       int32_t* n_passes, qsim_cycle** out) {
+  return qsim_cycle_create_priced(n_local_qubits, head, steady, tail, nullptr, 0, n_passes, out);
+}
+
+int qsim_cycle_create_priced(int n_local_qubits, const qsim_cycle_list* head, const qsim_cycle_list* steady, const qsim_cycle_list* tail,
+                             const double* engine_costs, int n_engine_costs, int32_t* n_passes, qsim_cycle** out) {
   if (!out) return fail(QSIM_ERR_INVALID, "qsim_cycle_create: out is null");
+  EngineCosts ec;
+  const bool priced = engine_costs_from(engine_costs, n_engine_costs, &ec);
+  if (engine_costs && !priced)
+    return fail(QSIM_ERR_INVALID, "qsim_cycle_create_priced: the cost table has %d entries, not %d", n_engine_costs, (int)QSIM_ENGINE_COST_COUNT);
+  const EngineCosts* costs = priced ? &ec : nullptr;
   if (n_local_qubits < kTileMinChunk || n_local_qubits > kTileMaxQubits)
     return fail(QSIM_ERR_INVALID, "qsim_cycle_create: fused passes need %d..%d local qubits", kTileMinChunk, kTileMaxQubits);
   std::unique_ptr<qsim_cycle> cy(new qsim_cycle());
   cy->k = n_local_qubits;
   cy->id = ++g_cycle_ids;
-  int rc = cycle_passes(n_local_qubits, head, "head", &cy->head);
-  if (rc || (rc = cycle_passes(n_local_qubits, steady, "steady", &cy->steady)) || (rc = cycle_passes(n_local_qubits, tail, "tail", &cy->tail)))
+  int rc = cycle_passes(n_local_qubits, head, "head", costs, &cy->head);
+  if (rc || (rc = cycle_passes(n_local_qubits, steady, "steady", costs, &cy->steady)) || (rc = cycle_passes(n_local_qubits, tail, "tail", costs, &cy->tail)))
     return rc;
   if (n_passes) { n_passes[0] = (int32_t)cy->head->size(); n_passes[1] = (int32_t)cy->steady->size(); n_passes[2] = (int32_t)cy->tail->size(); }
   *out = cy.release();
diff --git a/quantum_simulations_amd/csrc/abi_plan.h b/quantum_simulations_amd/csrc/abi_plan.h
--- a/quantum_simulations_amd/csrc/abi_plan.h
+++ b/quantum_simulations_amd/csrc/abi_plan.h
@@ -10,7 +10,10 @@
 }
 static int plan_ops_images(const char* what, int n_local_qubits, int n_ops, const int32_t* nq, const int32_t* qubits,
                            const double* mats, int n_tiles, const uint64_t* tile_masks, const int32_t* earliest_pass, void* out,
-                           uint64_t out_capacity_bytes, int32_t* n_passes) {
+                           uint64_t out_capacity_bytes, int32_t* n_passes, const double* engine_costs = nullptr, int n_engine_costs = 0) {
+  EngineCosts ec;
+  const bool priced = engine_costs_from(engine_costs, n_engine_costs, &ec);
+  if (engine_costs && !priced) return fail(QSIM_ERR_INVALID, "%s: the cost table has %d entries, not %d", what, n_engine_costs, (int)QSIM_ENGINE_COST_COUNT);
   if (n_tiles < 0 || (n_tiles && !tile_masks)) return fail(QSIM_ERR_INVALID, "%s: bad tile list", what);
   if (!n_passes) return fail(QSIM_ERR_INVALID, "%s: n_passes is null", what);
   if (n_local_qubits < kTileMinChunk || n_local_qubits > kTileMaxQubits)
@@ -35,7 +38,7 @@
     }
     used += sizeof(TileArgs);
     return (int)QSIM_OK;
-  }, n_tiles ? &hint : nullptr);
+  }, n_tiles ? &hint : nullptr, nullptr, priced ? &ec : nullptr);
   *n_passes = passes;
   return rc;
 }
@@ -54,6 +57,12 @@
                          uint64_t out_capacity_bytes, int32_t* n_passes) {
   return plan_ops_images("qsim_plan_ops_placed", n_local_qubits, n_ops, nq, qubits, mats, n_tiles, tile_masks, earliest_pass, out,
                          out_capacity_bytes, n_passes);
+}
+int qsim_plan_ops_priced(int n_local_qubits, int n_ops, const int32_t* nq, const int32_t* qubits, const double* mats,
+                         int n_tiles, const uint64_t* tile_masks, const int32_t* earliest_pass, const double* engine_costs,
+                         int n_engine_costs, void* out, uint64_t out_capacity_bytes, int32_t* n_passes) {
+  return plan_ops_images("qsim_plan_ops_priced", n_local_qubits, n_ops, nq, qubits, mats, n_tiles, tile_masks, earliest_pass, out,
+                         out_capacity_bytes, n_passes, engine_costs, n_engine_costs);
 }
 
 int qsim_lower_pass_images(void* images, int n_images, int32_t* n_rewritten) {
@@ -213,6 +222,28 @@
     if (engine_us_before) engine_us_before[p] = before[(size_t)p];
     if (engine_us_after) engine_us_after[p] = after[(size_t)p];
   }
+  return QSIM_OK;
+}
+
+int qsim_plan_group_prices(int n_local_qubits, int n_ops, const int32_t* nq, const int32_t* qubits, const double* mats,
+                           int n_tiles, const uint64_t* tile_masks, const int32_t* earliest_pass, const double* engine_costs,
+                           int n_engine_costs, double* engine_us_unpriced, double* engine_us_priced) {
+  if (n_tiles < 1 || !tile_masks || !engine_us_unpriced || !engine_us_priced) return fail(QSIM_ERR_INVALID, "qsim_plan_group_prices: bad arguments");
+  if (n_local_qubits < kTileMinChunk || n_local_qubits > kTileMaxQubits)
+    return fail(QSIM_ERR_INVALID, "qsim_plan_group_prices: fused passes need %d..%d local qubits", kTileMinChunk, kTileMaxQubits);
+  EngineCosts ec;
+  if (!engine_costs_from(engine_costs, n_engine_costs, &ec))
+    return fail(QSIM_ERR_INVALID, "qsim_plan_group_prices: the cost table needs %d entries", (int)QSIM_ENGINE_COST_COUNT);
+  int rc = check_op_list(n_ops, nq, qubits, mats, n_local_qubits, kQubitOfPlan);
+  if (rc) return rc;
+  std::vector<FusedOp> ops;
+  std::vector<int32_t> origin, placed;
+  classify_ops(n_ops, nq, qubits, mats, &ops, &origin);
+  if (earliest_pass) for (int32_t i : origin) placed.push_back(earliest_pass[i]);
+  std::vector<double> before, after;
+  if (!plan_group_prices(n_local_qubits, ops, std::vector<u64>(tile_masks, tile_masks + n_tiles), earliest_pass ? placed.data() : nullptr, ec, &before, &after))
+    return fail(QSIM_ERR_INVALID, "qsim_plan_group_prices: the named passes do not finish the list");
+  for (int p = 0; p < n_tiles; ++p) { engine_us_unpriced[p] = before[(size_t)p]; engine_us_priced[p] = after[(size_t)p]; }
   return QSIM_OK;
 }
 
diff --git a/quantum_simulations_amd/csrc/tile_groups.h b/quantum_simulations_amd/csrc/tile_groups.h
--- a/quantum_simulations_amd/csrc/tile_groups.h
+++ b/quantum_simulations_amd/csrc/tile_groups.h
@@ -405,6 +405,213 @@
   }
 };
 
+constexpr int kPricedBeam = 4;
+constexpr int kPricedTriples = 8;
+
+struct GroupTrial {
+  std::vector<TileGroup> groups;
+  std::vector<char> emitted;
+  GroupEmitter e;
+  double key = 0;
+  GroupTrial(const std::vector<FusedOp>& ops, const std::vector<size_t>& members, const std::vector<int>& high, int T)
+      : emitted(members.size(), 0), e(ops, members, high, T, &groups, &emitted) {}
+  GroupTrial(const GroupTrial& o) : groups(o.groups), emitted(o.emitted), e(o.e), key(o.key) {
+    e.out = &groups;
+    e.emitted = &emitted;
+  }
+};
+
+struct PricedGroups {
+  const std::vector<FusedOp>& ops;
+  const std::vector<size_t>& members;
+  const std::vector<int>& high;
+  const int T, k;
+  const EngineCosts& ec;
+  std::vector<double> floor_us;
+  std::vector<unsigned> need, uses;
+
+  PricedGroups(const std::vector<FusedOp>& ops_, const std::vector<size_t>& members_, const std::vector<int>& high_, int T_, int k_,
+               const EngineCosts& ec_)
+      : ops(ops_), members(members_), high(high_), T(T_), k(k_), ec(ec_) {
+    GroupTrial probe(ops, members, high, T);
+    for (size_t mi = 0; mi < members.size(); ++mi) {
+      const FusedOp& o = ops[members[mi]];
+      unsigned n = 0, u = 0;
+      for (int t = 0; t < o.ntargets; ++t) n |= 1u << probe.e.tile_pos(o.target[t]);
+      if (o.kind == TG_PHASE) { for (int b = 0; b < o.nbits; ++b) if (probe.e.tile_pos(o.bits[b]) >= 0) u |= 1u << probe.e.tile_pos(o.bits[b]); }
+      else if (o.control >= 0 && probe.e.tile_pos(o.control) >= 0) u |= 1u << probe.e.tile_pos(o.control);
+      need.push_back(n);
+      uses.push_back(u);
+      floor_us.push_back(record_us(mi, ~0u));
+    }
+  }
+
+  double record_us(size_t mi, unsigned own) const {
+    const FusedOp& o = ops[members[mi]];
+    if (o.kind == TG_DENSE2) return ec.of_family(OPC_DENSE2);
+    if (o.kind == TG_PHASE) {
+      const bool outer = __builtin_popcount(uses[mi]) < o.nbits;
+      return ec.of_family(op_shape(o).family) * ((uses[mi] & ~own) ? ec.v[QSIM_ENGINE_COST_PRED_LANE] : 1.0) * (outer ? ec.v[QSIM_ENGINE_COST_PRED_OUTER] : 1.0);
+    }
+    if (o.control < 0) return ec.of_family(priced_family(o));
+    const double us = ec.of_family(op_shape(o).family);
+    if (!uses[mi]) return us * ec.v[QSIM_ENGINE_COST_PRED_OUTER];
+    return us * ((uses[mi] & ~own) ? ec.v[QSIM_ENGINE_COST_PRED_LANE] : ec.v[QSIM_ENGINE_COST_REG_CTRL]);
+  }
+  static int stream_bytes(const std::vector<TileGroup>& groups) {
+    int bytes = 0;
+    for (const TileGroup& g : groups) {
+      bytes += kGroupRecordBytes;
+      for (const TileDesc& d : g.gates) bytes += d.opcode == OPC_SCALE ? 0 : desc_bytes(d);
+    }
+    return bytes;
+  }
+
+  struct Option { unsigned own; double rank; std::vector<size_t> grp; unsigned claimed; };
+
+  void options(const GroupEmitter& e, std::vector<Option>* out) const {
+    out->clear();
+    std::vector<GroupEmitter::Pending> pend;
+    unsigned cand = 0;
+    for (size_t mi = 0; mi < members.size(); ++mi) {
+      if (e.done[mi] || e.reserved[mi]) continue;
+      pend.push_back(e.pending(mi, (e.merge_on && op_shape(ops[members[mi]]).family == OPC_PHASE) ? 16 : 0));
+      cand |= need[mi] | uses[mi];
+    }
+    if (pend.empty()) return;
+    const double group = ec.v[QSIM_ENGINE_COST_GROUP];
+    auto consider = [&](unsigned own) {
+      Option o;
+      o.own = own;
+      if (!e.select(pend, own, &o.grp, &o.claimed)) return;
+      for (const Option& seen : *out) if (seen.grp == o.grp && seen.claimed == o.claimed) return;
+      unsigned bits_left = 0;
+      std::vector<char> held(members.size(), 0);
+      o.rank = group;
+      for (size_t mi : o.grp) { held[mi] = 1; o.rank += record_us(mi, o.claimed) - floor_us[mi]; }
+      for (size_t mi = 0; mi < members.size(); ++mi) if (!e.done[mi] && !held[mi]) bits_left |= need[mi];
+      o.rank += group * ((__builtin_popcount(bits_left) + kGroupBits - 1) / kGroupBits);
+      if (e.out->empty() && e.direct_ends && !(o.claimed & e.line_bits)) o.rank += ec.v[QSIM_ENGINE_COST_DIRECT_END];
+      out->push_back(std::move(o));
+    };
+    consider(0);
+    {
+      std::vector<size_t> grp;
+      unsigned claimed = 0;
+      e.next_group(&grp, &claimed);
+      if (!grp.empty() && __builtin_popcount(claimed) == kGroupBits) consider(claimed);
+    }
+    const size_t fixed = out->size();
+    if (__builtin_popcount(cand) >= kGroupBits) for_each_triple(cand, consider);
+    std::stable_sort(out->begin() + (long)fixed, out->end(), [](const Option& a, const Option& b) { return a.rank < b.rank; });
+    if (out->size() > fixed + (size_t)kPricedTriples) out->resize(fixed + (size_t)kPricedTriples);
+  }
+
+  bool finish(GroupTrial* t, double* us) const {
+    if (t->e.n_reserved) t->e.write_reserved();
+    if (t->e.left || t->groups.empty()) return false;
+    t->e.move_last_forward();
+    t->e.apply_scale();
+    if (stream_bytes(t->groups) > kTileRecordBudget) return false;
+    *us = ec.of_pass(t->groups, k);
+    return true;
+  }
+
+  void search(std::vector<TileGroup>* groups, double* groups_us) const {
+    double best_us = 1e300;
+    groups->clear();
+    std::vector<std::unique_ptr<GroupTrial>> beam, next;
+    beam.emplace_back(new GroupTrial(ops, members, high, T));
+    if (beam[0]->e.direct_ends && members.size() > 1) {
+      std::unique_ptr<GroupTrial> last(new GroupTrial(ops, members, high, T));
+      last->e.reserve_last();
+      if (last->e.n_reserved) beam.push_back(std::move(last));
+    }
+    std::vector<Option> opts;
+    for (size_t depth = 0; depth <= members.size() && !beam.empty(); ++depth) {
+      next.clear();
+      for (const std::unique_ptr<GroupTrial>& t : beam) {
+        if (t->e.left <= t->e.n_reserved) {
+          GroupTrial closed(*t);
+          double us = 0;
+          if (finish(&closed, &us) && us < best_us) { best_us = us; *groups = closed.groups; }
+          continue;
+        }
+        options(t->e, &opts);
+        for (const Option& o : opts) {
+          std::unique_ptr<GroupTrial> c(new GroupTrial(*t));
+          const size_t before = c->groups.size();
+          if (c->e.write_group(o.grp, o.claimed) || c->groups.size() != before + 1) continue;
+          GroupTrial rest(*c);
+          bool whole = true;
+          while (whole && rest.e.left > rest.e.n_reserved) {
+            std::vector<size_t> grp;
+            unsigned claimed = 0;
+            rest.e.next_group(&grp, &claimed);
+            whole = !grp.empty() && !rest.e.write_group(grp, claimed);
+          }
+          if (!whole || !finish(&rest, &c->key)) continue;
+          if (c->key < best_us) { best_us = c->key; *groups = rest.groups; }
+          next.push_back(std::move(c));
+        }
+      }
+      std::stable_sort(next.begin(), next.end(), [](const std::unique_ptr<GroupTrial>& a, const std::unique_ptr<GroupTrial>& b) { return a->key < b->key; });
+      beam.clear();
+      for (std::unique_ptr<GroupTrial>& c : next) {
+        bool twin = false;
+        for (const std::unique_ptr<GroupTrial>& b : beam)
+          twin = twin || (b->e.done == c->e.done && b->e.reserved == c->e.reserved && b->groups.size() == c->groups.size() &&
+                          std::equal(b->e.regs, b->e.regs + kGroupBits, c->e.regs) &&
+                          (b->groups[0].s[0] >= kTileLow) == (c->groups[0].s[0] >= kTileLow));
+        if (!twin && beam.size() < (size_t)kPricedBeam) beam.push_back(std::move(c));
+      }
+    }
+    *groups_us = best_us;
+  }
+};
+
+struct PricedGroupCache {
+  struct Entry { std::vector<unsigned char> key; std::vector<TileGroup> groups; double us; };
+  static constexpr size_t kEntries = 2048;
+  std::mutex mu;
+  std::map<u64, Entry> map;
+};
+static PricedGroupCache g_priced_groups;
+
+static void regroup_priced(const std::vector<FusedOp>& ops, const std::vector<size_t>& members, const std::vector<int>& high, int T, int k,
+                           const EngineCosts& ec, std::vector<TileGroup>* groups) {
+  if (members.size() < 2 || groups->empty()) return;
+  std::vector<unsigned char> key;
+  auto put = [&](const void* p, size_t n) { const unsigned char* b = (const unsigned char*)p; key.insert(key.end(), b, b + n); };
+  const int32_t head[3] = {T, k, (int32_t)members.size()};
+  put(head, sizeof head);
+  for (int b : high) { const int32_t v = b; put(&v, sizeof v); }
+  put(ec.v, sizeof ec.v);
+  for (size_t i : members) {
+    const FusedOp& o = ops[i];
+    const int32_t f[10] = {o.kind, o.ntargets, o.target[0], o.ntargets > 1 ? o.target[1] : -1, o.control, o.nbits, o.nbits > 0 ? o.bits[0] : -1,
+                           o.nbits > 1 ? o.bits[1] : -1, o.nq, o.nm};
+    put(f, sizeof f);
+    for (int e = 0; e < o.nm; ++e) { put(&o.m[e].x, 8); put(&o.m[e].y, 8); }
+  }
+  const u64 hash = fnv1a(key.data(), key.size());
+  std::vector<TileGroup> found;
+  double found_us = 0;
+  bool known = false;
+  {
+    std::lock_guard<std::mutex> lock(g_priced_groups.mu);
+    auto it = g_priced_groups.map.find(hash);
+    if (it != g_priced_groups.map.end() && it->second.key == key) { found = it->second.groups; found_us = it->second.us; known = true; }
+  }
+  if (!known) {
+    PricedGroups(ops, members, high, T, k, ec).search(&found, &found_us);
+    std::lock_guard<std::mutex> lock(g_priced_groups.mu);
+    if (g_priced_groups.map.size() >= PricedGroupCache::kEntries) g_priced_groups.map.clear();
+    g_priced_groups.map[hash] = PricedGroupCache::Entry{std::move(key), found, found_us};
+  }
+  if (!found.empty() && found_us < ec.of_pass(*groups, k) - 1e-9) groups->swap(found);
+}
+
 static int lower_unit_real(TileArgs* a) {
   if (!tuning().tile_unit || !tuning().tile_special) return 0;
   unsigned char* const base = reinterpret_cast<unsigned char*>(a);
diff --git a/quantum_simulations_amd/csrc/tile_launch.h b/quantum_simulations_amd/csrc/tile_launch.h
--- a/quantum_simulations_amd/csrc/tile_launch.h
+++ b/quantum_simulations_amd/csrc/tile_launch.h
@@ -229,14 +229,15 @@
 
 template <class Sink>
 static int run_fused(qsim_chunk* c, const std::vector<FusedOp>& ops, const RawOps& raw, const TileHint* hint, FusedIo* io,
-                     int* n_passes, Sink&& sink) {
+                     int* n_passes, Sink&& sink, const EngineCosts* costs = nullptr) {
   std::vector<unsigned char> key;
   u64 hash = 0;
   const size_t n_ops = (size_t)raw.n;
   const size_t hint_bytes = hint ? sizeof(uint64_t) * (size_t)hint->n : 0;
   const size_t placed_bytes = hint && hint->earliest ? sizeof(int32_t) * ops.size() : 0;
-  const int32_t hint_tag[2] = {hint ? hint->n : -1, placed_bytes != 0};
-  const size_t key_bytes = n_ops * (sizeof(int32_t) * 3 + sizeof(double) * 32) + sizeof hint_tag + hint_bytes + placed_bytes;
+  const size_t priced_bytes = costs ? sizeof costs->v : 0;
+  const int32_t hint_tag[3] = {hint ? hint->n : -1, placed_bytes != 0, costs != nullptr};
+  const size_t key_bytes = n_ops * (sizeof(int32_t) * 3 + sizeof(double) * 32) + sizeof hint_tag + hint_bytes + placed_bytes + priced_bytes;
   const bool cacheable = raw.nq && raw.qubits && raw.mats && raw.n > 0 && key_bytes <= kPlanCacheMaxKeyBytes && tuning().debug_stats == 0 &&
                          tuning().debug_skip_gates == 0;
   if (cacheable) {
@@ -248,6 +249,7 @@
     std::memcpy(w, hint_tag, sizeof hint_tag); w += sizeof hint_tag;
     if (hint_bytes) std::memcpy(w, hint->masks, hint_bytes);
     if (placed_bytes) std::memcpy(w + hint_bytes, hint->earliest, placed_bytes);
+    if (priced_bytes) std::memcpy(w + hint_bytes + placed_bytes, costs->v, priced_bytes);
     hash = fnv1a(key.data(), key.size(), 1469598103934665603ull ^ (u64)c->k);
     std::vector<CachedPass> hit;
     {
@@ -276,7 +278,7 @@
     if (cacheable) made.push_back(CachedPass{a, T, alg_bytes});
     prepare_planned(c, a, T, first, last, io);
     return sink(a, T, alg_bytes, last);
-  }, hint);
+  }, hint, nullptr, costs);
   if (rc == QSIM_OK && cacheable && !made.empty()) {
     std::lock_guard<std::mutex> lock(g_plan_cache_mu);
     g_plan_cache.emplace_front();
diff --git a/quantum_simulations_amd/csrc/tile_planner.h b/quantum_simulations_amd/csrc/tile_planner.h
--- a/quantum_simulations_amd/csrc/tile_planner.h
+++ b/quantum_simulations_amd/csrc/tile_planner.h
@@ -202,6 +202,15 @@
     }
   }
 
+  void emit_priced(const std::vector<size_t>& members, const std::vector<int>& high, const EngineCosts* costs,
+                   std::vector<TileGroup>* groups, std::vector<char>* emitted) const {
+    emit(members, high, groups, emitted);
+    if (!costs) return;
+    std::vector<size_t> held;
+    for (size_t mi = 0; mi < members.size(); ++mi) if ((*emitted)[mi]) held.push_back(members[mi]);
+    regroup_priced(ops, held, high, T, k, *costs, groups);
+  }
+
   u64 choose_tile(const TileHint* hint, int pass, u64 prev_mask, bool depth2) {
     if (hint && pass < hint->n) {
       const u64 m = hint->masks[pass] & all_qubits & ~((1ull << low) - 1);
@@ -300,7 +309,7 @@
 
 template <class Sink>
 static int plan_fused(int k, const std::vector<FusedOp>& ops_in, int* n_passes, Sink&& sink, const TileHint* hint = nullptr,
-                      PeekPlan* peek = nullptr) {
+                      PeekPlan* peek = nullptr, const EngineCosts* costs = nullptr) {
   const Tuning& tune = tuning();
   const std::vector<FusedOp> ops = planned_ops(ops_in);
   PassBuilder pb(k, ops, peek ? peek->n_total : k);
@@ -341,7 +350,7 @@
     for (size_t j = 0; j < high.size(); ++j) a.h[j] = (uint8_t)high[j];
     std::vector<char> emitted;
     std::vector<TileGroup> groups;
-    pb.emit(members, high, &groups, &emitted);
+    pb.emit_priced(members, high, peek ? nullptr : costs, &groups, &emitted);
     size_t n_emitted = 0;
     const double alg_bytes = pb.account(members, emitted, &n_emitted);
     if (!n_emitted) return fail(QSIM_ERR_INVALID, "internal: fused planner emitted nothing");
diff --git a/quantum_simulations_amd/csrc/tile_search.h b/quantum_simulations_amd/csrc/tile_search.h
--- a/quantum_simulations_amd/csrc/tile_search.h
+++ b/quantum_simulations_amd/csrc/tile_search.h
@@ -358,6 +358,34 @@
   return QSIM_OK;
 }
 
+static bool plan_group_prices(int k, const std::vector<FusedOp>& ops_in, const std::vector<u64>& masks, const int32_t* earliest,
+                              const EngineCosts& ec, std::vector<double>* us_unpriced, std::vector<double>* us_priced) {
+  const std::vector<FusedOp> ops = planned_ops(ops_in);
+  us_unpriced->assign(masks.size(), 0.0);
+  us_priced->assign(masks.size(), 0.0);
+  PassBuilder pb(k, ops, k);
+  std::vector<size_t> members;
+  std::vector<char> emitted;
+  std::vector<TileGroup> groups;
+  for (size_t p = 0; p < masks.size() && pb.remaining; ++p) {
+    pb.begin_pass();
+    pb.pass_no = (int)p;
+    pb.earliest = ops.size() == ops_in.size() ? earliest : nullptr;
+    members.clear();
+    pb.holds(masks[p], &members);
+    if (members.empty()) return false;
+    const std::vector<int> high = pb.filled(pb.bits_of(masks[p]));
+    pb.emit(members, high, &groups, &emitted);
+    (*us_unpriced)[p] = ec.of_pass(groups, k);
+    pb.emit_priced(members, high, &ec, &groups, &emitted);
+    (*us_priced)[p] = ec.of_pass(groups, k);
+    size_t n_emitted = 0;
+    pb.account(members, emitted, &n_emitted);
+    if (!n_emitted) return false;
+  }
+  return pb.remaining == 0;
+}
+
 static int plan_balance(int k, const std::vector<FusedOp>& ops_in, const std::vector<u64>& masks, const double* mem_us,
                         const EngineCosts& ec, bool place, std::vector<int32_t>* earliest, std::vector<double>* eng_before,
                         std::vector<double>* eng_after) {
@@ -381,7 +409,7 @@
       members.clear();
       pb.holds(masks[p], &members);
       if (members.empty()) return false;
-      pb.emit(members, pb.filled(pb.bits_of(masks[p])), &groups, &emitted);
+      pb.emit_priced(members, pb.filled(pb.bits_of(masks[p])), &ec, &groups, &emitted);
       (*eng)[p] = ec.of_pass(groups, k);
       for (size_t mi = 0; mi < members.size(); ++mi) if (emitted[mi]) pass_of[members[mi]] = (int32_t)p;
       size_t n_emitted = 0;
diff --git a/quantum_simulations_amd/kernel/device.py b/quantum_simulations_amd/kernel/device.py
--- a/quantum_simulations_amd/kernel/device.py
+++ b/quantum_simulations_amd/kernel/device.py
@@ -171,6 +171,18 @@
         lib = _lib.load()
         _lib.check(lib.qsim_apply_ops_placed(self._h, len(nq), _lib.ptr(nq), _lib.ptr(qs), _lib.ptr(mats), len(tm), _lib.ptr(tm),
                                              _lib.ptr(place)))
+        return lib.qsim_last_pass_count(self._h)
+
+    def apply_ops_priced(self, ops, tile_masks, earliest, engine_costs) -> int:
+        nq, qs, mats = as_packed(ops)
+        tm = np.ascontiguousarray(tile_masks, dtype=np.uint64)
+        place = None if earliest is None else np.ascontiguousarray(earliest, dtype=np.int32)
+        if place is not None and len(place) != len(nq):
+            raise ValueError("one earliest pass per op expected")
+        costs = np.ascontiguousarray(engine_costs, dtype=np.float64)
+        lib = _lib.load()
+        _lib.check(lib.qsim_apply_ops_priced(self._h, len(nq), _lib.ptr(nq), _lib.ptr(qs), _lib.ptr(mats), len(tm), _lib.ptr(tm),
+                                             _lib.ptr(place), _lib.ptr(costs), len(costs)))
         return lib.qsim_last_pass_count(self._h)
 
     def apply_cycle(self, cycle: "Cycle") -> int:
@@ -443,7 +455,7 @@
 
 class Cycle:
 
-    def __init__(self, k: int, head, steady, tail):
+    def __init__(self, k: int, head, steady, tail, engine_costs=None):
         keep, lists = [], []
         for ops, masks, earliest in (head, steady, tail):
             nq, qs, mats = as_packed(ops)
@@ -456,8 +468,9 @@
                                         _lib.ptr(tm).value if len(tm) else None, None if place is None else _lib.ptr(place).value))
         counts = np.zeros(3, dtype=np.int32)
         self._h = C.c_void_p()
-        _lib.check(_lib.load().qsim_cycle_create(int(k), C.byref(lists[0]), C.byref(lists[1]), C.byref(lists[2]), _lib.ptr(counts),
-                                                 C.byref(self._h)))
+        costs = None if engine_costs is None else np.ascontiguousarray(engine_costs, dtype=np.float64)
+        _lib.check(_lib.load().qsim_cycle_create_priced(int(k), C.byref(lists[0]), C.byref(lists[1]), C.byref(lists[2]), _lib.ptr(costs),
+                                                        0 if costs is None else len(costs), _lib.ptr(counts), C.byref(self._h)))
         self.k = k
         self.passes = tuple(int(x) for x in counts)
 
diff --git a/quantum_simulations_amd/kernel/planner.py b/quantum_simulations_amd/kernel/planner.py
--- a/quantum_simulations_amd/kernel/planner.py
+++ b/quantum_simulations_amd/kernel/planner.py
@@ -27,26 +27,31 @@
     return np.array([sum(1 << b for b in tile_bits(img)) for img in images], dtype=np.uint64)
 
 
-def _plan(n: int, ops, tiles, images, earliest=None) -> tuple:
+def _plan(n: int, ops, tiles, images, earliest=None, engine_costs=None) -> tuple:
     nq, qubits, mats = as_packed(ops)
     lib, count = _lib.load(), C.c_int32()
     head = (n, len(nq), ptr(nq), ptr(qubits), ptr(mats))
     tail = (ptr(images), 0 if images is None else images.nbytes, C.byref(count))
     tm = np.ascontiguousarray(tiles if tiles is not None else [], dtype=np.uint64)
+    place = None
     if len(tm) and earliest is not None:
         place = np.ascontiguousarray(earliest, dtype=np.int32)
         if len(place) != len(nq):
             raise ValueError("one earliest pass per op expected")
+    if engine_costs is not None:
+        costs = np.ascontiguousarray(engine_costs, dtype=np.float64)
+        return lib.qsim_plan_ops_priced(*head, len(tm), ptr(tm), ptr(place), ptr(costs), len(costs), *tail), count.value
+    if place is not None:
         return lib.qsim_plan_ops_placed(*head, len(tm), ptr(tm), ptr(place), *tail), count.value
     rc = lib.qsim_plan_ops_tiled(*head, len(tm), ptr(tm), *tail) if len(tm) else lib.qsim_plan_ops(*head, *tail)
     return rc, count.value
 
 
-def plan_ops(n: int, ops, tiles=None, earliest=None) -> np.ndarray:
+def plan_ops(n: int, ops, tiles=None, earliest=None, engine_costs=None) -> np.ndarray:
     room = _FIRST_BUFFER
     while True:
         images = np.zeros(room, dtype=PASS_IMAGE)
-        rc, count = _plan(n, ops, tiles, images, earliest)
+        rc, count = _plan(n, ops, tiles, images, earliest, engine_costs)
         if rc != _lib.QSIM_ERR_INVALID or count < room:
             _lib.check(rc)
             return images[:count]
@@ -78,6 +83,19 @@
     _lib.check(_lib.load().qsim_plan_balance(n, len(nq), ptr(nq), ptr(qubits), ptr(mats), len(tm), ptr(tm), ptr(mem), ptr(costs),
                                              len(costs), ptr(earliest), ptr(before), ptr(after)))
     return earliest, before, after
+
+
+def group_prices(n: int, ops, tiles, engine_costs, earliest=None) -> tuple:
+    nq, qubits, mats = as_packed(ops)
+    tm = np.ascontiguousarray(tiles, dtype=np.uint64)
+    costs = np.ascontiguousarray(engine_costs, dtype=np.float64)
+    place = None if earliest is None else np.ascontiguousarray(earliest, dtype=np.int32)
+    if place is not None and len(place) != len(nq):
+        raise ValueError("one earliest pass per op expected")
+    before, after = np.zeros(len(tm)), np.zeros(len(tm))
+    _lib.check(_lib.load().qsim_plan_group_prices(n, len(nq), ptr(nq), ptr(qubits), ptr(mats), len(tm), ptr(tm), ptr(place), ptr(costs),
+                                                  len(costs), ptr(before), ptr(after)))
+    return before, after
 
 
 def tiles_per_workgroup(n: int, tile_bits: int, fixed_bits: int = 0) -> int:
diff --git a/quantum_simulations_amd/runner/engine.py b/quantum_simulations_amd/runner/engine.py
--- a/quantum_simulations_amd/runner/engine.py
+++ b/quantum_simulations_amd/runner/engine.py
@@ -23,6 +23,7 @@
     placed: list | None = None
     l2p: list | None = None
     model_ms: tuple | None = None
+    engine_costs = None
     cycle = None
 
 
@@ -140,7 +141,7 @@
                 info.pop("planned", None)
                 info.pop("placed", None)
                 plan = GpuPlan([pack_ops(cyc["planned"][1])])
-                plan.cycle = Cycle(self.n, *zip(cyc["planned"], cyc["tiles"], cyc["placed"]))
+                plan.cycle = Cycle(self.n, *zip(cyc["planned"], cyc["tiles"], cyc["placed"]), engine_costs=costs)
                 plan.tiles, plan.placed = masks, [cyc["placed"][1]]
                 plan.l2p = None if l2p == list(range(self.n)) else l2p
                 plan.model_ms = info["model_ms"]
@@ -151,6 +152,7 @@
             plan = GpuPlan([pack_ops(ops) for ops in planned])
             plan.tiles = masks
             plan.placed = info.pop("placed", None)
+            plan.engine_costs = costs
             plan.l2p = None if l2p == list(range(self.n)) else l2p
             plan.model_ms = info["model_ms"]
             plan.layout_info = dict(info, passes_identity=own_identity, rewrite=dict(rewrite))
@@ -192,8 +194,11 @@
             return
         tiles = getattr(plan, "tiles", None) or [None] * len(plan)
         placed = getattr(plan, "placed", None) or [None] * len(plan)
+        costs = getattr(plan, "engine_costs", None)
         for ops, masks, place in zip(plan, tiles, placed):
-            if masks is not None and place is not None and self.mode != "per-gate":
+            if masks is not None and costs is not None and len(masks) and self.mode != "per-gate":
+                self.last_passes += self.state.apply_ops_priced(ops, masks, place, costs)
+            elif masks is not None and place is not None and self.mode != "per-gate":
                 self.last_passes += self.state.apply_ops_placed(ops, masks, place)
             elif masks is not None and self.mode != "per-gate":
                 self.last_passes += self.state.apply_ops_tiled(ops, masks)
```
